# shaderko/velocity-asr

Hardware: NVIDIA B200
Metric: rtfx (higher is better)
Workload: dtype f32

## Files before the change

velocity-asr_b200/csrc/engine.cu:

```cuda
#include <cmath>
#include <cstdio>
#include <cstdlib>
#include <cstring>
#include <string>
#include <unordered_map>
#include <vector>

#include "../../include/vasr.h"
#include "common.cuh"
#include "kernels.cuh"

using namespace vasr;

namespace {

thread_local std::string g_err;

int fail(int code, const std::string& msg) {
  g_err = msg;
  return code;
}

#define CK(expr)                                                                               \
  do {                                                                                         \
    cudaError_t e_ = (expr);                                                                   \
    if (e_ != cudaSuccess)                                                                     \
      return fail(VASR_ERR_CUDA, std::string(#expr) + ": " + cudaGetErrorString(e_) + " (" +   \
                                     __FILE__ + ":" + std::to_string(__LINE__) + ")");         \
  } while (0)

#define RET(expr)            \
  do {                       \
    int r_ = (expr);         \
    if (r_ != VASR_OK) return r_; \
  } while (0)

constexpr int N_FFT = 400, HOP = 160, N_FREQ = 201, PAD = 200;

struct BlockW {
  float *ln1_g, *ln1_b, *ln2_g, *ln2_b, *conv_w, *conv_b, *A, *D;
  float *w_in, *w_xdt, *b_xdt, *w_out, *w_f1, *b_f1, *w_f2, *b_f2;
  float* s_f1;
  int N = 0;
  int di = 0, ks = 0;
  int structured = 0;
};

struct QSite {
  float *qs = nullptr, *qz = nullptr;
  int N = 0;
  int nmod = 0;
  const char* name[3] = {nullptr, nullptr, nullptr};
  int c0[3] = {0, 0, 0}, nc[3] = {0, 0, 0};
};
enum { Q_TB = 0, Q_P1, Q_P2, Q_Q, Q_KV, Q_O, Q_F3, Q_FO, Q_CTC, Q_SITES };

struct Arena {
  char* base = nullptr;
  size_t bytes = 0;
  size_t used = 0;
  void reset() { used = 0; }
  template <typename T>
  T* take(int64_t n) {
    size_t off = (used + 255) & ~size_t(255);
    used = off + (size_t)(n > 0 ? n : 0) * sizeof(T);
    return reinterpret_cast<T*>(base + off);
  }
};

}

struct vasr_handle {
  vasr_config cfg{};
  int device = 0;
  std::unordered_map<std::string, std::vector<float>> staged;
  bool committed = false;
  std::vector<void*> weight_allocs;
  std::vector<void*> frontend_allocs;
  std::vector<void*>* alloc_list = &weight_allocs;
  int quant = 0;
  int quant_active = 0;
  int calibrating = 0;
  QSite qsite[Q_SITES];
  static constexpr int RAG_RING = 4;
  int32_t* rag_pin[RAG_RING] = {};
  cudaEvent_t rag_ev[RAG_RING] = {};
  int64_t rag_pin_cap = 0;
  int rag_next = 0;
  float* q_mm = nullptr;
  std::unordered_map<const float*, float*> w_split;

  std::vector<BlockW> local, global;
  float *tb_w = nullptr, *tb_b = nullptr, *pe_time = nullptr, *pe_freq = nullptr, *tb_g = nullptr, *tb_bt = nullptr;
  int64_t pe_rows = 0;
  float *loc_g = nullptr, *loc_b = nullptr, *glo_g = nullptr, *glo_b = nullptr;
  float *p1_w = nullptr, *p1_b = nullptr, *p2_w = nullptr, *p2_b = nullptr;
  float *n1_g = nullptr, *n1_b = nullptr, *n2_g = nullptr, *n2_b = nullptr;
  float *w_q = nullptr, *b_q = nullptr, *w_kv = nullptr, *b_kv = nullptr, *w_o = nullptr, *b_o = nullptr;
  float *w_f3 = nullptr, *b_f3 = nullptr, *w_fo = nullptr, *b_fo = nullptr;
  float *ctc_g = nullptr, *ctc_b = nullptr, *w_ctc = nullptr, *b_ctc = nullptr;
  float *w_q_ln = nullptr, *b_q_ln = nullptr, *s_q = nullptr, *w_kv_ln = nullptr, *b_kv_ln = nullptr, *s_kv = nullptr;
  float *w_ctc_ln = nullptr, *b_ctc_ln = nullptr, *s_ctc = nullptr, *w_f3p = nullptr, *b_f3p = nullptr;
  float* win = nullptr;
  float* tw400 = nullptr;
  int *fb_lo = nullptr, *fb_off = nullptr;
  float* fb_w = nullptr;

  int num_sms = 148;
  int64_t tc_launches = 0;

  Arena ws;
  cudaStream_t own_stream = nullptr;
  static constexpr int HOST_SLICES = 8;
  cudaStream_t copy_stream = nullptr;
  cudaEvent_t slice_ev[HOST_SLICES] = {};
  cudaEvent_t copy_gate = nullptr;
  int64_t launches = 0;
  cudaEvent_t call_done = nullptr;
  cudaStream_t call_stream = nullptr;
  bool call_pending = false;

  int prof = 0;
  struct ProfEntry { std::string tag; cudaEvent_t e0, e1; };
  std::vector<ProfEntry> prof_ev;
  bool timing = false;
  std::vector<cudaEvent_t> ev;
  int ev_used = 0;
  cudaEvent_t ev_t0 = nullptr, ev_t1 = nullptr;
  bool ev_total = false;
};

namespace {

struct Dims {
  int64_t B, S, T, L, M, K1, K2, Mg, M2, Tp;
  int d, di, n_mels, V, att;
};

constexpr int GLOBAL_EXPAND = 2, GLOBAL_KS = 4;

Dims make_dims(const vasr_handle* h, int64_t B, int64_t S, int64_t T) {
  Dims q{};
  q.B = B;
  q.S = S;
  q.T = T;
  q.L = (T + 1) / 2;
  q.M = B * q.L;
  int64_t k1 = q.L / 8 > 64 ? q.L / 8 : 64;
  q.K1 = k1 < q.L ? k1 : q.L;
  int64_t k2 = q.K1 / 4 > 16 ? q.K1 / 4 : 16;
  k2 = k2 < 64 ? k2 : 64;
  q.K2 = k2 < q.K1 ? k2 : q.K1;
  q.Mg = B * q.K1;
  q.M2 = B * q.K2;
  q.Tp = T + 2 + ((T + 2) & 1);
  q.d = h->cfg.d_model;
  q.di = h->cfg.d_model * (h->cfg.ssm_expand_ratio > GLOBAL_EXPAND ? h->cfg.ssm_expand_ratio : GLOBAL_EXPAND);
  q.n_mels = h->cfg.mel_bins;
  q.V = h->cfg.vocab_size;
  q.att = h->cfg.attention_dim;
  return q;
}

struct Work {
  float *raw, *melpad;
  double* part;
  float* qscratch;
  float *xa, *xb, *u, *xz, *bcdt, *yg, *hbuf, *cat, *f3, *fm, *fused, *qb, *ob;
  float *ga, *gb, *g2, *g2n, *kv;
  float* logits;
  float* lnstat;
  float* amax_val;
  int32_t* amax_idx;
  int32_t* pred;
  float* pcm_stage;
  int32_t *tok_stage, *len_stage;
  int32_t* ragbuf;
  const int32_t* rag;
};

size_t carve(vasr_handle* h, const Dims& q, bool need_mel, bool need_logits, Work* w, bool need_stage = false) {
  Arena a = h->ws;
  a.reset();
  Work t{};
  const int nmax = h->cfg.ssm_state_dim > h->cfg.global_ssm_state_dim ? h->cfg.ssm_state_dim
                                                                      : h->cfg.global_ssm_state_dim;
  if (need_mel) {
    t.part = a.take<double>(q.B * mel_fft_blocks(q.T) * q.n_mels * 2);
    t.raw = a.take<float>(q.B * q.T * q.n_mels);
  }
  t.melpad = a.take<float>(q.B * q.Tp * q.n_mels);
  t.xa = a.take<float>(q.M * q.d);
  t.xb = a.take<float>(q.M * q.d);
  t.u = a.take<float>(q.M * q.d);
  t.xz = a.take<float>(q.M * 2 * q.di);
  t.bcdt = a.take<float>(q.M * (2 * nmax + q.di));
  t.yg = a.take<float>(q.M * q.di);
  t.hbuf = a.take<float>(q.M * q.di);
  t.cat = a.take<float>(q.M * 2 * q.d);
  if (!h->w_f3p) t.f3 = a.take<float>(q.M * 3 * q.d);
  t.fm = a.take<float>(q.M * q.d);
  t.fused = a.take<float>(q.M * q.d);
  t.qb = a.take<float>(q.M * q.att);
  t.ob = a.take<float>(q.M * q.att);
  t.ga = a.take<float>(q.Mg * q.d);
  t.gb = a.take<float>(q.Mg * q.d);
  t.g2 = a.take<float>(q.M2 * q.d);
  t.g2n = a.take<float>(q.M2 * q.d);
  t.kv = a.take<float>(q.M2 * 2 * q.att);
  if (need_logits) t.logits = a.take<float>(q.M * q.V);
  t.lnstat = a.take<float>(q.M * 2);
  t.amax_val = a.take<float>(q.M * argmax_slots(q.V));
  t.amax_idx = a.take<int32_t>(q.M * argmax_slots(q.V));
  if (h->quant_active) t.qscratch = a.take<float>(q.M * (q.V > 3 * q.d ? q.V : 3 * q.d));
  t.pred = a.take<int32_t>(q.M);
  t.ragbuf = a.take<int32_t>(q.B * RAG_STRIDE);
  if (need_stage) {
    t.pcm_stage = a.take<float>(q.B * q.S);
    t.tok_stage = a.take<int32_t>(q.M);
    t.len_stage = a.take<int32_t>(q.B);
  }
  if (w) *w = t;
  return a.used + 256;
}

int ensure_workspace(vasr_handle* h, const Dims& q, bool need_mel, bool need_logits, Work* w,
                     bool need_stage = false) {
  const size_t need = carve(h, q, need_mel, need_logits, nullptr, need_stage);
  if (need > h->ws.bytes) {
    CK(cudaDeviceSynchronize());
    if (h->ws.base) CK(cudaFree(h->ws.base));
    h->ws.base = nullptr;
    h->ws.bytes = 0;
    void* p = nullptr;
    CK(cudaMalloc(&p, need));
    h->ws.base = static_cast<char*>(p);
    h->ws.bytes = need;
  }
  carve(h, q, need_mel, need_logits, w, need_stage);
  return VASR_OK;
}

const std::vector<float>* find(vasr_handle* h, const std::string& k) {
  auto it = h->staged.find(k);
  return it == h->staged.end() ? nullptr : &it->second;
}

int need(vasr_handle* h, const std::string& k, int64_t numel, const std::vector<float>** out) {
  const std::vector<float>* v = find(h, k);
  if (!v) return fail(VASR_ERR_STATE, "missing weight: " + k);
  if (numel >= 0 && (int64_t)v->size() != numel)
    return fail(VASR_ERR_SHAPE, "weight " + k + " has " + std::to_string(v->size()) + " elements, expected " +
                                    std::to_string(numel));
  *out = v;
  return VASR_OK;
}

template <typename T>
int upload(vasr_handle* h, const T* src, size_t n, T** dst) {
  void* p = nullptr;
  CK(cudaMalloc(&p, (n ? n : 1) * sizeof(T)));
  h->alloc_list->push_back(p);
  if (n) CK(cudaMemcpy(p, src, n * sizeof(T), cudaMemcpyHostToDevice));
  *dst = static_cast<T*>(p);
  return VASR_OK;
}

int up(vasr_handle* h, const std::string& k, int64_t numel, float** dst) {
  const std::vector<float>* v;
  RET(need(h, k, numel, &v));
  return upload(h, v->data(), v->size(), dst);
}

void fake_quant_rows(std::vector<float>& w, int64_t rows) {
  const int64_t cols = rows > 0 ? (int64_t)w.size() / rows : 0;
  for (int64_t r = 0; r < rows; ++r) {
    float* x = w.data() + r * cols;
    float lo = x[0], hi = x[0];
    for (int64_t c = 1; c < cols; ++c) { lo = fminf(lo, x[c]); hi = fmaxf(hi, x[c]); }
    float scale = fmaxf(fabsf(lo), fabsf(hi)) / 127.0f;
    if (scale < 1e-10f) scale = 1e-10f;
    for (int64_t c = 0; c < cols; ++c) {
      volatile float t = x[c] / scale;
      float q = nearbyintf(t + 0.0f);
      q = fminf(fmaxf(q, -128.f), 127.f);
      volatile float dq = (q - 0.0f) * scale;
      volatile float diff = dq - x[c];
      x[c] = x[c] + diff;
    }
  }
}

int get_w(vasr_handle* h, const std::string& k, int64_t numel, int64_t rows, std::vector<float>* out) {
  const std::vector<float>* v;
  RET(need(h, k, numel, &v));
  *out = *v;
  if (h->quant) fake_quant_rows(*out, rows);
  return VASR_OK;
}
int up_w(vasr_handle* h, const std::string& k, int64_t numel, int64_t rows, float** dst) {
  std::vector<float> w;
  RET(get_w(h, k, numel, rows, &w));
  return upload(h, w.data(), w.size(), dst);
}

void fold_ln(const std::vector<float>& W, int64_t N, int64_t K, const float* bias, const float* gamma,
             const float* beta, std::vector<float>* Wf, std::vector<float>* bf, std::vector<float>* sf) {
  Wf->resize((size_t)N * K);
  bf->resize((size_t)N);
  sf->resize((size_t)N);
  for (int64_t n = 0; n < N; ++n) {
    double sb = bias ? (double)bias[n] : 0.0, ss = 0.0;
    for (int64_t k = 0; k < K; ++k) {
      const float w = W[(size_t)n * K + k];
      const float wf = w * gamma[k];
      (*Wf)[(size_t)n * K + k] = wf;
      sb += (double)w * (double)beta[k];
      ss += (double)wf;
    }
    (*bf)[(size_t)n] = (float)sb;
    (*sf)[(size_t)n] = (float)ss;
  }
}
bool can_fold_ln(int d) { return d % 32 == 0 && d / 32 > 4; }
int upload_folded(vasr_handle* h, const std::vector<float>& W, int64_t N, int64_t K, const float* bias,
                  const std::string& gk, const std::string& bk, float** Wd, float** bd, float** sd) {
  const std::vector<float>*g, *b;
  RET(need(h, gk, K, &g));
  RET(need(h, bk, K, &b));
  std::vector<float> Wf, bf, sf;
  fold_ln(W, N, K, bias, g->data(), b->data(), &Wf, &bf, &sf);
  RET(upload(h, Wf.data(), Wf.size(), Wd));
  RET(upload(h, bf.data(), bf.size(), bd));
  return upload(h, sf.data(), sf.size(), sd);
}

int gate_perm_row(int rp, int C) {
  const int t = rp / 192, a = (rp % 192) / 96, j = (rp % 96) / 32, i = rp % 32;
  return j * C + 64 * t + 32 * a + i;
}

int pack_block(vasr_handle* h, const std::string& p, int N, int expand, int ks, BlockW* w) {
  const int d = h->cfg.d_model, di = d * expand;
  w->N = N;
  w->di = di;
  w->ks = ks;
  RET(up(h, p + "norm1.weight", d, &w->ln1_g));
  RET(up(h, p + "norm1.bias", d, &w->ln1_b));
  RET(up(h, p + "norm2.weight", d, &w->ln2_g));
  RET(up(h, p + "norm2.bias", d, &w->ln2_b));
  RET(up(h, p + "conv.weight", (int64_t)d * ks, &w->conv_w));
  RET(up(h, p + "conv.bias", d, &w->conv_b));
  const std::vector<float>*alog, *xw, *dw, *db;
  RET(need(h, p + "ssm.A_log", N, &alog));
  std::vector<float> A(N);
  int structured = 1;
  for (int n = 0; n < N; ++n) {
    A[n] = -expf((*alog)[n]);
    if (fabsf((*alog)[n] - logf((float)(n + 1))) > 1e-6f) structured = 0;
  }
  w->structured = structured;
  RET(upload(h, A.data(), A.size(), &w->A));
  RET(up(h, p + "ssm.D", di, &w->D));
  RET(up(h, p + "ssm.in_proj.weight", (int64_t)2 * di * d, &w->w_in));
  RET(need(h, p + "ssm.x_proj.weight", (int64_t)2 * N * di, &xw));
  RET(need(h, p + "ssm.dt_proj.weight", (int64_t)di * di, &dw));
  RET(need(h, p + "ssm.dt_proj.bias", di, &db));
  std::vector<float> wx((size_t)(2 * N + di) * di), bx((size_t)2 * N + di, 0.f);
  memcpy(wx.data(), xw->data(), xw->size() * sizeof(float));
  memcpy(wx.data() + xw->size(), dw->data(), dw->size() * sizeof(float));
  memcpy(bx.data() + 2 * N, db->data(), db->size() * sizeof(float));
  RET(upload(h, wx.data(), wx.size(), &w->w_xdt));
  RET(upload(h, bx.data(), bx.size(), &w->b_xdt));
  RET(up(h, p + "ssm.out_proj.weight", (int64_t)d * di, &w->w_out));
  const std::vector<float>*f1w, *f1b;
  RET(need(h, p + "ffn.0.weight", (int64_t)di * d, &f1w));
  RET(need(h, p + "ffn.0.bias", di, &f1b));
  w->s_f1 = nullptr;
  if (can_fold_ln(d) && (di % 192 == 0 || di % 192 >= 128)) {
    RET(upload_folded(h, *f1w, di, d, f1b->data(), p + "norm2.weight", p + "norm2.bias", &w->w_f1, &w->b_f1, &w->s_f1));
  } else {
    RET(upload(h, f1w->data(), f1w->size(), &w->w_f1));
    RET(upload(h, f1b->data(), f1b->size(), &w->b_f1));
  }
  RET(up(h, p + "ffn.3.weight", (int64_t)d * di, &w->w_f2));
  RET(up(h, p + "ffn.3.bias", d, &w->b_f2));
  return VASR_OK;
}

void default_window(std::vector<float>& w) {
  w.resize(N_FFT);
  for (int i = 0; i < N_FFT; ++i) w[i] = (float)(0.5 - 0.5 * cos(2.0 * M_PI * i / N_FFT));
}
void default_filterbank(int n_mels, std::vector<float>& fb) {
  fb.assign((size_t)n_mels * N_FREQ, 0.f);
  auto lin = [](float a, float b, int steps, int i) {
    float step = (b - a) / (float)(steps - 1);
    return i < steps / 2 ? a + step * (float)i : b - step * (float)(steps - 1 - i);
  };
  const float mel_max = 2595.f * log10f(1.f + 8000.f / 700.f);
  std::vector<float> hz(n_mels + 2);
  for (int i = 0; i < n_mels + 2; ++i) hz[i] = 700.f * (powf(10.f, lin(0.f, mel_max, n_mels + 2, i) / 2595.f) - 1.f);
  for (int j = 0; j < n_mels; ++j)
    for (int k = 0; k < N_FREQ; ++k) {
      const float f = lin(0.f, 8000.f, N_FREQ, k);
      const float up_ = (f - hz[j]) / (hz[j + 1] - hz[j] + 1e-10f);
      const float dn = (hz[j + 2] - f) / (hz[j + 2] - hz[j + 1] + 1e-10f);
      const float v = up_ < dn ? up_ : dn;
      fb[(size_t)j * N_FREQ + k] = v > 0.f ? v : 0.f;
    }
}

int pack_frontend_impl(vasr_handle* h);
int setup_qsites(vasr_handle* h);
void free_splits(vasr_handle* h);
int pack_frontend(vasr_handle* h) {
  CK(cudaDeviceSynchronize());
  free_splits(h);
  for (void* p : h->frontend_allocs) cudaFree(p);
  h->frontend_allocs.clear();
  h->alloc_list = &h->frontend_allocs;
  const int r = pack_frontend_impl(h);
  h->alloc_list = &h->weight_allocs;
  return r;
}
int pack_frontend_impl(vasr_handle* h) {
  const int n_mels = h->cfg.mel_bins;
  std::vector<float> win, fb;
  if (const std::vector<float>* v = find(h, "frontend.window")) {
    if ((int)v->size() != N_FFT) return fail(VASR_ERR_SHAPE, "frontend.window must have 400 elements");
    win = *v;
  } else {
    default_window(win);
  }
  if (const std::vector<float>* v = find(h, "frontend.mel_filterbank")) {
    if ((int64_t)v->size() != (int64_t)n_mels * N_FREQ)
      return fail(VASR_ERR_SHAPE, "frontend.mel_filterbank must be n_mels x 201");
    fb = *v;
  } else {
    default_filterbank(n_mels, fb);
  }
  RET(upload(h, win.data(), win.size(), &h->win));
  std::vector<float> tw((size_t)2 * N_FFT);
  for (int m = 0; m < N_FFT; ++m) {
    const double ang = 2.0 * M_PI * (double)m / (double)N_FFT;
    tw[2 * m] = (float)cos(ang);
    tw[2 * m + 1] = (float)(-sin(ang));
  }
  RET(upload(h, tw.data(), tw.size(), &h->tw400));
  std::vector<int> lo(n_mels), off(n_mels + 1, 0);
  std::vector<float> wts;
  for (int j = 0; j < n_mels; ++j) {
    int a = -1, b = -1;
    for (int k = 0; k < N_FREQ; ++k)
      if (fb[(size_t)j * N_FREQ + k] != 0.f) {
        if (a < 0) a = k;
        b = k;
      }
    lo[j] = a < 0 ? 0 : a;
    if (a >= 0)
      for (int k = a; k <= b; ++k) wts.push_back(fb[(size_t)j * N_FREQ + k]);
    off[j + 1] = (int)wts.size();
  }
  RET(upload(h, lo.data(), lo.size(), &h->fb_lo));
  RET(upload(h, off.data(), off.size(), &h->fb_off));
  RET(upload(h, wts.data(), wts.size(), &h->fb_w));
  return VASR_OK;
}

void free_splits(vasr_handle* h) {
  for (auto& kv : h->w_split) cudaFree(kv.second);
  h->w_split.clear();
}

void free_weights(vasr_handle* h) {
  free_splits(h);
  for (void* p : h->weight_allocs) cudaFree(p);
  h->weight_allocs.clear();
  h->local.clear();
  h->global.clear();
  h->committed = false;
}

#define KL(expr)                                                                            \
  do {                                                                                      \
    cudaError_t e_ = (expr);                                                                \
    if (e_ != cudaSuccess)                                                                  \
      return fail(e_ == cudaErrorInvalidValue ? VASR_ERR_UNSUPPORTED : VASR_ERR_CUDA,       \
                  std::string(#expr) + ": " + cudaGetErrorString(e_));                      \
  } while (0)

int split_of(vasr_handle* h, const float* W, int64_t numel, cudaStream_t s, const float** out) {
  auto it = h->w_split.find(W);
  if (it == h->w_split.end()) {
    void* p = nullptr;
    CK(cudaMalloc(&p, (size_t)2 * numel * sizeof(float)));
    KL(launch_split_tf32(W, static_cast<float*>(p), numel, s));
    it = h->w_split.emplace(W, static_cast<float*>(p)).first;
  }
  *out = it->second;
  return VASR_OK;
}

int gemm(vasr_handle* h, GemmArgs& g, cudaStream_t s);
int calibrate_site(vasr_handle* h, const GemmArgs& g, const QSite& q, float* scratch, cudaStream_t s) {
  GemmArgs p = g;
  p.C = scratch; p.ldc = g.N;
  p.q_scale = p.q_zp = nullptr;
  p.act = ACT_NONE; p.act_from = 0;
  p.resid = nullptr; p.pe_time = p.pe_freq = nullptr;
  RET(gemm(h, p, s));
  for (int i = 0; i < q.nmod; ++i) {
    KL(launch_minmax(scratch, g.N, g.M, q.c0[i], q.nc[i], h->q_mm, s, &h->launches));
    KL(launch_set_qparams(h->q_mm, q.qs, q.qz, q.c0[i], q.nc[i], s, &h->launches));
  }
  return VASR_OK;
}

int gemm_impl(vasr_handle* h, GemmArgs& g, cudaStream_t s);
int gemm(vasr_handle* h, GemmArgs& g, cudaStream_t s) {
  if (!h->prof) return gemm_impl(h, g, s);
  vasr_handle::ProfEntry pe;
  pe.tag = "M" + std::to_string(g.M) + " K" + std::to_string(g.K) + " N" + std::to_string(g.N) + " act" +
           std::to_string(g.act) + (g.resid ? " resid" : "") + (g.pe_time ? " pe" : "") + (g.q_scale ? " quant" : "");
  CK(cudaEventCreate(&pe.e0));
  CK(cudaEventCreate(&pe.e1));
  CK(cudaEventRecord(pe.e0, s));
  const int r = gemm_impl(h, g, s);
  CK(cudaEventRecord(pe.e1, s));
  h->prof_ev.push_back(pe);
  return r;
}

int gemm_impl(vasr_handle* h, GemmArgs& g, cudaStream_t s) {
  RET(split_of(h, g.W, g.N * g.K, s, &g.W_split));
  const cudaError_t e = launch_gemm_tc(g, h->num_sms, s, &h->launches);
  if (e == cudaErrorNotSupported) {
    (void)cudaGetLastError();
    return fail(VASR_ERR_UNSUPPORTED, "projection " + std::to_string(g.M) + " x " + std::to_string(g.K) + " -> " +
                                          std::to_string(g.N) + ": view not supported by the tensor-core kernel "
                                          "(16-byte alignment of rows, K % 4, N % 4)");
  }
  if (e != cudaSuccess) return fail(VASR_ERR_CUDA, std::string("launch_gemm_tc: ") + cudaGetErrorString(e));
  ++h->tc_launches;
  return VASR_OK;
}

int gemm_q(vasr_handle* h, GemmArgs& g, int site, float* qscratch, cudaStream_t s) {
  if (site >= 0 && h->quant_active) {
    const QSite& q = h->qsite[site];
    g.q_scale = q.qs;
    g.q_zp = q.qz;
    if (h->calibrating) RET(calibrate_site(h, g, q, qscratch, s));
  }
  return gemm(h, g, s);
}

int linear(vasr_handle* h, const float* A, int64_t lda, const float* W, const float* bias, float* C, int64_t ldc,
           int64_t M, int64_t K, int64_t N, int act, int act_from, const float* resid, int64_t ldr,
           cudaStream_t s, int site = -1, float* qscratch = nullptr) {
  GemmArgs g;
  g.A = A; g.lda = lda; g.W = W; g.bias = bias; g.C = C; g.ldc = ldc;
  g.M = M; g.N = N; g.K = K; g.act = act; g.act_from = act_from; g.resid = resid; g.ldr = ldr;
  return gemm_q(h, g, site, qscratch, s);
}
int linear_ln(vasr_handle* h, const Work& k, const float* A, int64_t lda, const float* W, const float* bias,
              const float* colsum, float* C, int64_t ldc, int64_t M, int64_t K, int64_t N, int act, cudaStream_t s) {
  GemmArgs g;
  g.A = A; g.lda = lda; g.W = W; g.bias = bias; g.C = C; g.ldc = ldc;
  g.M = M; g.N = N; g.K = K; g.act = act; g.act_from = 0;
  g.ln_s = colsum; g.ln_stats = k.lnstat;
  return gemm(h, g, s);
}


int run_scan(vasr_handle* h, const BlockW& w, const Work& k, int64_t B, int64_t L, int quirk, cudaStream_t s) {
  const int di = w.di;
  const int64_t ld = 2 * w.N + di;
  ScanArgs a;
  a.x = k.xz; a.ldx = 2 * di;
  a.z = k.xz + di; a.ldz = 2 * di;
  a.Bm = k.bcdt; a.ldb = ld;
  a.Cm = k.bcdt + w.N; a.ldc = ld;
  a.dt = k.bcdt + 2 * w.N; a.lddt = ld;
  a.A = w.A; a.D = w.D;
  a.y = k.yg; a.ldy = di;
  a.B = B; a.L = L; a.Di = di; a.N = w.N;
  a.parallel_quirk = quirk;
  a.structured_a = w.structured;
  a.num_sms = h->num_sms;
  const bool t = h->timing && h->ev_used + 2 <= (int)h->ev.size();
  if (t) cudaEventRecord(h->ev[h->ev_used], s);
  KL(launch_selective_scan(a, s, &h->launches));
  if (t) {
    cudaEventRecord(h->ev[h->ev_used + 1], s);
    h->ev_used += 2;
  }
  return VASR_OK;
}

int run_block(vasr_handle* h, const BlockW& w, const Work& k, float* x, float* x1, int64_t B, int64_t L, int quirk,
              cudaStream_t s) {
  const int d = h->cfg.d_model, di = w.di;
  const int64_t M = B * L;
  KL(launch_ln_dwconv(x, k.u, w.ln1_g, w.ln1_b, w.conv_w, w.conv_b, B, L, d, w.ks, s, &h->launches));
  RET(linear(h, k.u, d, w.w_in, nullptr, k.xz, 2 * di, M, d, 2 * di, ACT_NONE, 0, nullptr, 0, s));
  RET(linear(h, k.xz, 2 * di, w.w_xdt, w.b_xdt, k.bcdt, 2 * w.N + di, M, di, 2 * w.N + di, ACT_SOFTPLUS, 2 * w.N,
             nullptr, 0, s));
  RET(run_scan(h, w, k, B, L, quirk, s));
  RET(linear(h, k.yg, di, w.w_out, nullptr, x1, d, M, di, d, ACT_NONE, 0, x, d, s));
  if (w.s_f1) {
    RET(linear_ln(h, k, x1, d, w.w_f1, w.b_f1, w.s_f1, k.hbuf, di, M, d, di, ACT_GELU, s));
  } else {
    KL(launch_layer_norm(x1, d, k.u, d, w.ln2_g, w.ln2_b, M, d, s, &h->launches));
    RET(linear(h, k.u, d, w.w_f1, w.b_f1, k.hbuf, di, M, d, di, ACT_GELU, 0, nullptr, 0, s));
  }
  RET(linear(h, k.hbuf, di, w.w_f2, w.b_f2, x, d, M, di, d, ACT_NONE, 0, x1, d, s));
  return VASR_OK;
}

int quirk_for(const vasr_handle* h, int stack, int scan_mode) {
  if (scan_mode < 0) scan_mode = stack == 0 ? h->cfg.scan_mode : VASR_SCAN_PARALLEL;
  return scan_mode == VASR_SCAN_PARALLEL ? 1 : 0;
}

int run_global_context(vasr_handle* h, const Dims& q, const Work& k, cudaStream_t s) {
  const int d = q.d, att = q.att;
  KL(launch_adaptive_pool(k.cat, 2 * d, k.gb, q.B, q.L, q.K1, d, s, &h->launches, k.rag, RAG_L, RAG_K1));
  RET(linear(h, k.gb, d, h->p1_w, h->p1_b, k.ga, d, q.Mg, d, d, ACT_NONE, 0, nullptr, 0, s, Q_P1, k.qscratch));
  for (size_t i = 0; i < h->global.size(); ++i)
    RET(run_block(h, h->global[i], k, k.ga, k.gb, q.B, q.K1, quirk_for(h, 1, -1), s));
  KL(launch_layer_norm(k.ga, d, k.ga, d, h->glo_g, h->glo_b, q.Mg, d, s, &h->launches));
  KL(launch_adaptive_pool(k.ga, d, k.g2, q.B, q.K1, q.K2, d, s, &h->launches, k.rag, RAG_K1, RAG_K2));
  RET(linear(h, k.g2, d, h->p2_w, h->p2_b, k.g2n, d, q.M2, d, d, ACT_NONE, 0, nullptr, 0, s, Q_P2, k.qscratch));
  if (h->w_kv_ln) {
    RET(linear_ln(h, k, k.g2n, d, h->w_kv_ln, h->b_kv_ln, h->s_kv, k.kv, 2 * att, q.M2, d, 2 * att, ACT_NONE, s));
    RET(linear_ln(h, k, k.cat, 2 * d, h->w_q_ln, h->b_q_ln, h->s_q, k.qb, att, q.M, d, att, ACT_NONE, s));
  } else {
    KL(launch_layer_norm(k.g2n, d, k.g2n, d, h->n1_g, h->n1_b, q.M2, d, s, &h->launches));
    RET(linear(h, k.g2n, d, h->w_kv, h->b_kv, k.kv, 2 * att, q.M2, d, 2 * att, ACT_NONE, 0, nullptr, 0, s, Q_KV, k.qscratch));
    KL(launch_layer_norm(k.cat, 2 * d, k.u, d, h->n2_g, h->n2_b, q.M, d, s, &h->launches));
    RET(linear(h, k.u, d, h->w_q, h->b_q, k.qb, att, q.M, d, att, ACT_NONE, 0, nullptr, 0, s, Q_Q, k.qscratch));
  }
  KL(launch_attention(k.qb, att, k.kv, k.ob, att, q.B, q.L, q.K2, h->cfg.attention_heads,
                      att / h->cfg.attention_heads, s, &h->launches, k.rag));
  RET(linear(h, k.ob, att, h->w_o, h->b_o, k.cat + d, 2 * d, q.M, att, d, ACT_NONE, 0, nullptr, 0, s, Q_O, k.qscratch));
  if (h->w_f3p) {
    GemmArgs g;
    g.A = k.cat; g.lda = 2 * d; g.W = h->w_f3p; g.bias = h->b_f3p; g.C = k.fm; g.ldc = d;
    g.M = q.M; g.N = 3 * d; g.K = 2 * d; g.gate = 1;
    RET(gemm(h, g, s));
  } else {
    RET(linear(h, k.cat, 2 * d, h->w_f3, h->b_f3, k.f3, 3 * d, q.M, 2 * d, 3 * d, ACT_NONE, 0, nullptr, 0, s, Q_F3, k.qscratch));
    KL(launch_gate_mix(k.f3, k.fm, q.M, d, s, &h->launches));
  }
  RET(linear(h, k.fm, d, h->w_fo, h->b_fo, k.fused, d, q.M, d, d, ACT_NONE, 0, nullptr, 0, s, Q_FO, k.qscratch));
  return VASR_OK;
}

int run_ctc_head(vasr_handle* h, const Dims& q, const Work& k, const float* x, float* logits, cudaStream_t s) {
  if (h->w_ctc_ln) {
    GemmArgs g;
    g.A = x; g.lda = q.d; g.W = h->w_ctc_ln; g.bias = h->b_ctc_ln; g.C = logits; g.ldc = q.V;
    g.M = q.M; g.N = q.V; g.K = q.d;
    g.ln_s = h->s_ctc; g.ln_stats = k.lnstat;
    if (!logits) { g.amax_val = k.amax_val; g.amax_idx = k.amax_idx; }
    return gemm(h, g, s);
  }
  if (!logits) return fail(VASR_ERR_STATE, "the FakeQuantize model decodes from its logits");
  KL(launch_layer_norm(x, q.d, k.u, q.d, h->ctc_g, h->ctc_b, q.M, q.d, s, &h->launches));
  RET(linear(h, k.u, q.d, h->w_ctc, h->b_ctc, logits, q.V, q.M, q.d, q.V, ACT_NONE, 0, nullptr, 0, s, Q_CTC, k.qscratch));
  return VASR_OK;
}

int run_model(vasr_handle* h, const Dims& q, const Work& k, float* logits, float* f_tb, float* f_local,
              float* f_fused, cudaStream_t s) {
  const int d = q.d;
  if (q.L > h->pe_rows)
    return fail(VASR_ERR_SHAPE, "sequence of " + std::to_string(q.L) + " tokens exceeds the positional table (" +
                                    std::to_string(h->pe_rows) + " rows, model.py:87,125)");
  GemmArgs g;
  g.A = k.melpad; g.lda = 2 * q.n_mels; g.rows_per_batch = q.L; g.batch_stride = q.Tp * q.n_mels;
  g.W = h->tb_w; g.bias = h->tb_b; g.C = k.xa; g.ldc = d;
  g.M = q.M; g.N = d; g.K = 3 * q.n_mels;
  g.act = ACT_GELU; g.act_from = 0;
  g.pe_time = h->pe_time; g.pe_freq = h->pe_freq; g.pe_half = d / 2; g.pe_rows = q.L;
  RET(gemm_q(h, g, Q_TB, k.qscratch, s));
  KL(launch_layer_norm(k.xa, d, k.xa, d, h->tb_g, h->tb_bt, q.M, d, s, &h->launches));
  if (f_tb) CK(cudaMemcpyAsync(f_tb, k.xa, (size_t)q.M * d * sizeof(float), cudaMemcpyDeviceToDevice, s));
  for (size_t i = 0; i < h->local.size(); ++i)
    RET(run_block(h, h->local[i], k, k.xa, k.xb, q.B, q.L, quirk_for(h, 0, -1), s));
  KL(launch_layer_norm(k.xa, d, k.cat, 2 * d, h->loc_g, h->loc_b, q.M, d, s, &h->launches));
  if (f_local)
    CK(cudaMemcpy2DAsync(f_local, (size_t)d * sizeof(float), k.cat, (size_t)2 * d * sizeof(float),
                         (size_t)d * sizeof(float), (size_t)q.M, cudaMemcpyDeviceToDevice, s));
  RET(run_global_context(h, q, k, s));
  if (f_fused) CK(cudaMemcpyAsync(f_fused, k.fused, (size_t)q.M * d * sizeof(float), cudaMemcpyDeviceToDevice, s));
  RET(run_ctc_head(h, q, k, k.fused, logits, s));
  return VASR_OK;
}

int run_mel(vasr_handle* h, const Dims& q, const Work& k, const float* pcm, int normalize, cudaStream_t s) {
  KL(launch_mel_fft(pcm, k.raw, normalize ? k.part : nullptr, q.B, q.S, q.T, q.n_mels, h->fb_lo, h->fb_off, h->fb_w,
                    h->win, h->tw400, s, &h->launches, k.rag));
  return VASR_OK;
}

int run_mel_from_host(vasr_handle* h, const Dims& q, const Work& k, const float* pcm_host, cudaStream_t s) {
  const int64_t per = (q.B + vasr_handle::HOST_SLICES - 1) / vasr_handle::HOST_SLICES;
  const int64_t nblk = mel_fft_blocks(q.T);
  CK(cudaEventRecord(h->copy_gate, s));
  CK(cudaStreamWaitEvent(h->copy_stream, h->copy_gate, 0));
  int i = 0;
  for (int64_t b0 = 0; b0 < q.B; b0 += per, ++i) {
    const int64_t nb = q.B - b0 < per ? q.B - b0 : per;
    CK(cudaMemcpyAsync(k.pcm_stage + b0 * q.S, pcm_host + b0 * q.S, (size_t)nb * q.S * sizeof(float),
                       cudaMemcpyHostToDevice, h->copy_stream));
    CK(cudaEventRecord(h->slice_ev[i], h->copy_stream));
    CK(cudaStreamWaitEvent(s, h->slice_ev[i], 0));
    KL(launch_mel_fft(k.pcm_stage + b0 * q.S, k.raw + b0 * q.T * q.n_mels, k.part + b0 * nblk * q.n_mels * 2, nb, q.S,
                      q.T, q.n_mels, h->fb_lo, h->fb_off, h->fb_w, h->win, h->tw400, s, &h->launches,
                      k.rag ? k.rag + b0 * RAG_STRIDE : nullptr));
  }
  return VASR_OK;
}

int check_ready(const vasr_handle* h) {
  if (!h) return fail(VASR_ERR_INVALID, "null handle");
  if (!h->committed) return fail(VASR_ERR_STATE, "weights not committed (call vasr_commit_weights)");
  return VASR_OK;
}

struct DeviceGuard {
  int prev = -1;
  explicit DeviceGuard(int dev) {
    if (cudaGetDevice(&prev) != cudaSuccess || prev == dev) prev = -1;
    cudaSetDevice(dev);
  }
  ~DeviceGuard() {
    if (prev >= 0) cudaSetDevice(prev);
  }
  DeviceGuard(const DeviceGuard&) = delete;
  DeviceGuard& operator=(const DeviceGuard&) = delete;
};

struct CallOrder {
  vasr_handle* h;
  cudaStream_t s;
  CallOrder(vasr_handle* h_, cudaStream_t s_) : h(h_), s(s_) {
    if (h->call_pending && h->call_stream != s) cudaStreamWaitEvent(s, h->call_done, 0);
  }
  ~CallOrder() {
    if (cudaEventRecord(h->call_done, s) == cudaSuccess) {
      h->call_stream = s;
      h->call_pending = true;
    }
  }
  CallOrder(const CallOrder&) = delete;
  CallOrder& operator=(const CallOrder&) = delete;
};

void timing_begin(vasr_handle* h, cudaStream_t s) {
  h->ev_used = 0;
  h->ev_total = false;
  if (h->timing) {
    cudaEventRecord(h->ev_t0, s);
    h->ev_total = true;
  }
}
void timing_end(vasr_handle* h, cudaStream_t s) {
  if (h->timing) cudaEventRecord(h->ev_t1, s);
}

int setup_qsites(vasr_handle* h) {
  const int d = h->cfg.d_model, att = h->cfg.attention_dim, V = h->cfg.vocab_size;
  auto site = [&](int id, int N, std::initializer_list<const char*> names, std::initializer_list<int> widths) {
    QSite& q = h->qsite[id];
    q.N = N;
    q.nmod = 0;
    int c = 0;
    auto w = widths.begin();
    for (const char* nm : names) {
      q.name[q.nmod] = nm; q.c0[q.nmod] = c; q.nc[q.nmod] = *w;
      c += *w; ++w; ++q.nmod;
    }
  };
  site(Q_TB, d, {"temporal_binding.conv"}, {d});
  site(Q_P1, d, {"global_context.pool1.pool_proj"}, {d});
  site(Q_P2, d, {"global_context.pool2.pool_proj"}, {d});
  site(Q_Q, att, {"global_context.cross_attention.q_proj"}, {att});
  site(Q_KV, 2 * att, {"global_context.cross_attention.k_proj", "global_context.cross_attention.v_proj"}, {att, att});
  site(Q_O, d, {"global_context.cross_attention.out_proj"}, {d});
  site(Q_F3, 3 * d, {"global_context.fusion.gate_proj.0", "global_context.fusion.local_proj",
                     "global_context.fusion.global_proj"}, {d, d, d});
  site(Q_FO, d, {"global_context.fusion.out_proj"}, {d});
  site(Q_CTC, V, {"ctc_head.proj.2"}, {V});
  for (int i = 0; i < Q_SITES; ++i) {
    QSite& q = h->qsite[i];
    std::vector<float> zeros((size_t)q.N, 0.f);
    RET(upload(h, zeros.data(), zeros.size(), &q.qs));
    RET(upload(h, zeros.data(), zeros.size(), &q.qz));
  }
  if (!h->q_mm) {
    void* p = nullptr;
    CK(cudaMalloc(&p, 2 * sizeof(float)));
    h->q_mm = static_cast<float*>(p);
  }
  return VASR_OK;
}

QSite* find_module(vasr_handle* h, const char* module, int* idx) {
  for (int i = 0; i < Q_SITES; ++i)
    for (int j = 0; j < h->qsite[i].nmod; ++j)
      if (strcmp(h->qsite[i].name[j], module) == 0) {
        *idx = j;
        return &h->qsite[i];
      }
  return nullptr;
}

}

extern "C" {

const char* vasr_last_error(void) { return g_err.c_str(); }
const char* vasr_version(void) { return "libvasr 0.1 (sm_100a)"; }

int64_t vasr_num_frames(int64_t samples) { return 1 + samples / HOP; }
int64_t vasr_num_tokens(int64_t frames) { return (frames + 1) / 2; }

int vasr_create(const vasr_config* cfg, int device, vasr_handle** out) {
  if (!cfg || !out) return fail(VASR_ERR_INVALID, "null argument");
  *out = nullptr;
  const vasr_config& c = *cfg;
  if (c.scan_mode < 0 || c.scan_mode > 2) return fail(VASR_ERR_INVALID, "Unknown scan_mode");
  if (c.d_model <= 0 || c.d_model > 192 || (c.d_model % 16) != 0)
    return fail(VASR_ERR_UNSUPPORTED, "d_model must be a multiple of 16, at most 192");
  if ((c.mel_bins * 3) % 16 != 0 || c.mel_bins * 8 > 1024)
    return fail(VASR_ERR_UNSUPPORTED, "mel_bins must make 3*mel_bins a multiple of 16 (and be <= 128)");
  auto n_ok = [](int n) { return n == 16 || n == 32 || n == 64; };
  if (!n_ok(c.ssm_state_dim) || !n_ok(c.global_ssm_state_dim))
    return fail(VASR_ERR_UNSUPPORTED, "ssm state_dim must be 16, 32 or 64");
  const int di = c.d_model * c.ssm_expand_ratio;
  if (c.ssm_expand_ratio < 1 || (di % 64) != 0 || (c.d_model * GLOBAL_EXPAND) % 64 != 0)
    return fail(VASR_ERR_UNSUPPORTED, "d_model*expand_ratio (and 2*d_model for the global stack) must be multiples of 64");
  if (c.ssm_kernel_size < 1 || c.ssm_kernel_size > 8) return fail(VASR_ERR_UNSUPPORTED, "ssm_kernel_size must be in [1, 8]");
  if (c.attention_heads < 1 || c.attention_dim % c.attention_heads != 0 || c.attention_dim / c.attention_heads > 16 ||
      c.attention_dim % 16 != 0 || c.attention_heads > 4)
    return fail(VASR_ERR_UNSUPPORTED, "attention_dim must be a multiple of 16 with head_dim <= 16 and at most 4 heads "
                                      "(the attention kernel runs 64 threads per head in a 256-thread CTA)");
  if (c.vocab_size < 1 || c.ssm_layers < 0 || c.global_ssm_layers < 0) return fail(VASR_ERR_INVALID, "bad sizes");
  int ndev = 0;
  if (cudaGetDeviceCount(&ndev) != cudaSuccess || ndev <= 0)
    return fail(VASR_ERR_CUDA, "no CUDA device: libvasr has no CPU path");
  if (device < 0 || device >= ndev) return fail(VASR_ERR_INVALID, "bad device index");
  cudaDeviceProp prop;
  CK(cudaGetDeviceProperties(&prop, device));
  if (prop.major != 10) return fail(VASR_ERR_CUDA, std::string("libvasr is built for sm_100a only; device is ") + prop.name);
  DeviceGuard dev_guard(device);
  vasr_handle* h = new vasr_handle();
  h->cfg = c;
  h->device = device;
  h->num_sms = prop.multiProcessorCount;
  h->prof = debug_env_int("VASR_PROF", 0);
  CK(cudaStreamCreateWithFlags(&h->own_stream, cudaStreamNonBlocking));
  CK(cudaStreamCreateWithFlags(&h->copy_stream, cudaStreamNonBlocking));
  for (auto& e : h->slice_ev) CK(cudaEventCreateWithFlags(&e, cudaEventDisableTiming));
  CK(cudaEventCreateWithFlags(&h->copy_gate, cudaEventDisableTiming));
  CK(cudaEventCreateWithFlags(&h->call_done, cudaEventDisableTiming));
  h->ev.resize(64);
  for (auto& e : h->ev) CK(cudaEventCreate(&e));
  CK(cudaEventCreate(&h->ev_t0));
  CK(cudaEventCreate(&h->ev_t1));
  RET(pack_frontend(h));
  *out = h;
  return VASR_OK;
}

void vasr_destroy(vasr_handle* h) {
  if (!h) return;
  DeviceGuard dev_guard(h->device);
  cudaDeviceSynchronize();
  free_weights(h);
  for (void* p : h->frontend_allocs) cudaFree(p);
  if (h->ws.base) cudaFree(h->ws.base);
  if (h->q_mm) cudaFree(h->q_mm);
  for (auto& e : h->ev) cudaEventDestroy(e);
  if (h->ev_t0) cudaEventDestroy(h->ev_t0);
  if (h->ev_t1) cudaEventDestroy(h->ev_t1);
  if (h->own_stream) cudaStreamDestroy(h->own_stream);
  if (h->copy_stream) cudaStreamDestroy(h->copy_stream);
  for (auto& e : h->slice_ev)
    if (e) cudaEventDestroy(e);
  if (h->copy_gate) cudaEventDestroy(h->copy_gate);
  if (h->call_done) cudaEventDestroy(h->call_done);
  for (int i = 0; i < vasr_handle::RAG_RING; ++i) {
    if (h->rag_pin[i]) cudaFreeHost(h->rag_pin[i]);
    if (h->rag_ev[i]) cudaEventDestroy(h->rag_ev[i]);
  }
  delete h;
}

int vasr_set_weight(vasr_handle* h, const char* name, const float* host, int64_t numel) {
  if (!h || !name || (!host && numel > 0) || numel < 0) return fail(VASR_ERR_INVALID, "null argument");
  const std::string k(name);
  static const char* prefixes[] = {"temporal_binding.", "local_ssm.", "global_context.", "ctc_head.", "frontend."};
  bool ok = false;
  for (const char* p : prefixes) ok = ok || k.rfind(p, 0) == 0;
  if (!ok) return fail(VASR_ERR_INVALID, "unknown weight name: " + k);
  h->staged[k].assign(host, host + numel);
  if (k.rfind("frontend.", 0) == 0) {
    DeviceGuard dev_guard(h->device);
    return pack_frontend(h);
  }
  h->committed = false;
  return VASR_OK;
}

int vasr_commit_weights(vasr_handle* h) {
  if (!h) return fail(VASR_ERR_INVALID, "null handle");
  DeviceGuard dev_guard(h->device);
  CK(cudaDeviceSynchronize());
  free_weights(h);
  h->w_q_ln = h->b_q_ln = h->s_q = h->w_kv_ln = h->b_kv_ln = h->s_kv = nullptr;
  h->w_ctc_ln = h->b_ctc_ln = h->s_ctc = h->w_f3p = h->b_f3p = nullptr;
  const vasr_config& c = h->cfg;
  const int d = c.d_model, nm = c.mel_bins, att = c.attention_dim;
  std::vector<float> cwv;
  RET(get_w(h, "temporal_binding.conv.weight", (int64_t)d * nm * 3, d, &cwv));
  const std::vector<float>* cw = &cwv;
  std::vector<float> tbw((size_t)d * 3 * nm);
  for (int o = 0; o < d; ++o)
    for (int ch = 0; ch < nm; ++ch)
      for (int j = 0; j < 3; ++j) tbw[(size_t)o * 3 * nm + j * nm + ch] = (*cw)[((size_t)o * nm + ch) * 3 + j];
  RET(upload(h, tbw.data(), tbw.size(), &h->tb_w));
  RET(up(h, "temporal_binding.conv.bias", d, &h->tb_b));
  const std::vector<float>* pt;
  RET(need(h, "temporal_binding.pos_encoding.pe_time", -1, &pt));
  if (pt->size() % (size_t)(d / 2) != 0) return fail(VASR_ERR_SHAPE, "pe_time must be (rows, d_model/2)");
  h->pe_rows = (int64_t)pt->size() / (d / 2);
  RET(upload(h, pt->data(), pt->size(), &h->pe_time));
  RET(up(h, "temporal_binding.pos_encoding.pe_freq", d - d / 2, &h->pe_freq));
  RET(up(h, "temporal_binding.norm.weight", d, &h->tb_g));
  RET(up(h, "temporal_binding.norm.bias", d, &h->tb_bt));
  h->local.resize(c.ssm_layers);
  for (int i = 0; i < c.ssm_layers; ++i)
    RET(pack_block(h, "local_ssm.layers." + std::to_string(i) + ".", c.ssm_state_dim, c.ssm_expand_ratio,
                   c.ssm_kernel_size, &h->local[i]));
  RET(up(h, "local_ssm.norm.weight", d, &h->loc_g));
  RET(up(h, "local_ssm.norm.bias", d, &h->loc_b));
  const std::string gc = "global_context.";
  h->global.resize(c.global_ssm_layers);
  for (int i = 0; i < c.global_ssm_layers; ++i)
    RET(pack_block(h, gc + "global_ssm.layers." + std::to_string(i) + ".", c.global_ssm_state_dim, GLOBAL_EXPAND,
                   GLOBAL_KS, &h->global[i]));
  RET(up(h, gc + "global_ssm.norm.weight", d, &h->glo_g));
  RET(up(h, gc + "global_ssm.norm.bias", d, &h->glo_b));
  RET(up_w(h, gc + "pool1.pool_proj.weight", (int64_t)d * d, d, &h->p1_w));
  RET(up(h, gc + "pool1.pool_proj.bias", d, &h->p1_b));
  RET(up_w(h, gc + "pool2.pool_proj.weight", (int64_t)d * d, d, &h->p2_w));
  RET(up(h, gc + "pool2.pool_proj.bias", d, &h->p2_b));
  RET(up(h, gc + "norm1.weight", d, &h->n1_g));
  RET(up(h, gc + "norm1.bias", d, &h->n1_b));
  RET(up(h, gc + "norm2.weight", d, &h->n2_g));
  RET(up(h, gc + "norm2.bias", d, &h->n2_b));
  RET(up_w(h, gc + "cross_attention.q_proj.weight", (int64_t)att * d, att, &h->w_q));
  RET(up(h, gc + "cross_attention.q_proj.bias", att, &h->b_q));
  const std::vector<float>*kb, *vb;
  std::vector<float> kwv, vwv;
  RET(get_w(h, gc + "cross_attention.k_proj.weight", (int64_t)att * d, att, &kwv));
  RET(need(h, gc + "cross_attention.k_proj.bias", att, &kb));
  RET(get_w(h, gc + "cross_attention.v_proj.weight", (int64_t)att * d, att, &vwv));
  RET(need(h, gc + "cross_attention.v_proj.bias", att, &vb));
  const std::vector<float>*kw = &kwv, *vw = &vwv;
  std::vector<float> wkv(*kw), bkv(*kb);
  wkv.insert(wkv.end(), vw->begin(), vw->end());
  bkv.insert(bkv.end(), vb->begin(), vb->end());
  RET(upload(h, wkv.data(), wkv.size(), &h->w_kv));
  RET(upload(h, bkv.data(), bkv.size(), &h->b_kv));
  if (!h->quant && can_fold_ln(d)) {
    const std::vector<float>*qw, *qb;
    RET(need(h, gc + "cross_attention.q_proj.weight", (int64_t)att * d, &qw));
    RET(need(h, gc + "cross_attention.q_proj.bias", att, &qb));
    RET(upload_folded(h, *qw, att, d, qb->data(), gc + "norm2.weight", gc + "norm2.bias", &h->w_q_ln, &h->b_q_ln, &h->s_q));
    RET(upload_folded(h, wkv, 2 * att, d, bkv.data(), gc + "norm1.weight", gc + "norm1.bias", &h->w_kv_ln, &h->b_kv_ln,
                      &h->s_kv));
  }
  RET(up_w(h, gc + "cross_attention.out_proj.weight", (int64_t)d * att, d, &h->w_o));
  RET(up(h, gc + "cross_attention.out_proj.bias", d, &h->b_o));
  const std::vector<float>*gb, *lb, *cb2;
  std::vector<float> gwv, lwv, cwv2;
  RET(get_w(h, gc + "fusion.gate_proj.0.weight", (int64_t)d * 2 * d, d, &gwv));
  RET(need(h, gc + "fusion.gate_proj.0.bias", d, &gb));
  RET(get_w(h, gc + "fusion.local_proj.weight", (int64_t)d * d, d, &lwv));
  RET(need(h, gc + "fusion.local_proj.bias", d, &lb));
  RET(get_w(h, gc + "fusion.global_proj.weight", (int64_t)d * d, d, &cwv2));
  RET(need(h, gc + "fusion.global_proj.bias", d, &cb2));
  const std::vector<float>*gw = &gwv, *lw = &lwv, *cw2 = &cwv2;
  std::vector<float> wf3((size_t)3 * d * 2 * d, 0.f), bf3;
  memcpy(wf3.data(), gw->data(), gw->size() * sizeof(float));
  for (int o = 0; o < d; ++o) {
    memcpy(&wf3[(size_t)(d + o) * 2 * d], &(*lw)[(size_t)o * d], d * sizeof(float));
    memcpy(&wf3[(size_t)(2 * d + o) * 2 * d + d], &(*cw2)[(size_t)o * d], d * sizeof(float));
  }
  bf3 = *gb;
  bf3.insert(bf3.end(), lb->begin(), lb->end());
  bf3.insert(bf3.end(), cb2->begin(), cb2->end());
  RET(upload(h, wf3.data(), wf3.size(), &h->w_f3));
  RET(upload(h, bf3.data(), bf3.size(), &h->b_f3));
  h->w_f3p = h->b_f3p = nullptr;
  if (!h->quant && d % 64 == 0) {
    std::vector<float> wp(wf3.size()), bp(bf3.size());
    for (int rp = 0; rp < 3 * d; ++rp) {
      const int r = gate_perm_row(rp, d);
      memcpy(&wp[(size_t)rp * 2 * d], &wf3[(size_t)r * 2 * d], (size_t)2 * d * sizeof(float));
      bp[(size_t)rp] = bf3[(size_t)r];
    }
    RET(upload(h, wp.data(), wp.size(), &h->w_f3p));
    RET(upload(h, bp.data(), bp.size(), &h->b_f3p));
  }
  RET(up_w(h, gc + "fusion.out_proj.weight", (int64_t)d * d, d, &h->w_fo));
  RET(up(h, gc + "fusion.out_proj.bias", d, &h->b_fo));
  RET(up(h, "ctc_head.proj.0.weight", d, &h->ctc_g));
  RET(up(h, "ctc_head.proj.0.bias", d, &h->ctc_b));
  RET(up_w(h, "ctc_head.proj.2.weight", (int64_t)c.vocab_size * d, c.vocab_size, &h->w_ctc));
  RET(up(h, "ctc_head.proj.2.bias", c.vocab_size, &h->b_ctc));
  if (!h->quant && can_fold_ln(d)) {
    const std::vector<float>*hw, *hb;
    RET(need(h, "ctc_head.proj.2.weight", (int64_t)c.vocab_size * d, &hw));
    RET(need(h, "ctc_head.proj.2.bias", c.vocab_size, &hb));
    RET(upload_folded(h, *hw, c.vocab_size, d, hb->data(), "ctc_head.proj.0.weight", "ctc_head.proj.0.bias", &h->w_ctc_ln,
                      &h->b_ctc_ln, &h->s_ctc));
  }
  h->quant_active = h->quant;
  if (h->quant_active) RET(setup_qsites(h));
  h->committed = true;
  return VASR_OK;
}

int vasr_log_mel(vasr_handle* h, const float* pcm_dev, int64_t B, int64_t S, int normalize, float* mel_dev,
                 void* stream) {
  if (!h) return fail(VASR_ERR_INVALID, "null handle");
  if (B < 0 || !pcm_dev || !mel_dev) return fail(VASR_ERR_INVALID, "null argument");
  if (S <= PAD) return fail(VASR_ERR_SHAPE, "reflect padding needs more than 200 samples (audio.py:100-101)");
  DeviceGuard dev_guard(h->device);
  cudaStream_t s = static_cast<cudaStream_t>(stream);
  CallOrder call_order(h, s);
  const Dims q = make_dims(h, B, S, vasr_num_frames(S));
  Work k;
  RET(ensure_workspace(h, q, true, false, &k));
  RET(run_mel(h, q, k, pcm_dev, normalize, s));
  KL(launch_mel_finish(k.raw, nullptr, nullptr, mel_dev, q.B, q.T, q.n_mels, q.T, 0, s, &h->launches, nullptr,
                       normalize ? k.part : nullptr));
  return VASR_OK;
}

int vasr_forward(vasr_handle* h, const float* mel_dev, int64_t B, int64_t T, float* logits_dev, float* feat_tb_dev,
                 float* feat_local_dev, float* feat_fused_dev, void* stream) {
  RET(check_ready(h));
  if (B < 0 || T < 1 || !mel_dev || !logits_dev) return fail(VASR_ERR_INVALID, "null argument");
  DeviceGuard dev_guard(h->device);
  cudaStream_t s = static_cast<cudaStream_t>(stream);
  CallOrder call_order(h, s);
  const Dims q = make_dims(h, B, 0, T);
  Work k;
  RET(ensure_workspace(h, q, false, false, &k));
  timing_begin(h, s);
  KL(launch_mel_finish(mel_dev, nullptr, nullptr, k.melpad, q.B, q.T, q.n_mels, q.Tp, 1, s, &h->launches));
  RET(run_model(h, q, k, logits_dev, feat_tb_dev, feat_local_dev, feat_fused_dev, s));
  timing_end(h, s);
  return VASR_OK;
}

int vasr_ssm_block(vasr_handle* h, int stack, int layer, int scan_mode, const float* x_dev, int64_t B, int64_t L,
                   float* out_dev, void* stream) {
  RET(check_ready(h));
  if (stack < 0 || stack > 1) return fail(VASR_ERR_INVALID, "stack must be 0 (local) or 1 (global)");
  const std::vector<BlockW>& blocks = stack == 0 ? h->local : h->global;
  if (layer < 0 || layer >= (int)blocks.size()) return fail(VASR_ERR_INVALID, "layer out of range");
  if (scan_mode > 2) return fail(VASR_ERR_INVALID, "Unknown scan_mode");
  DeviceGuard dev_guard(h->device);
  cudaStream_t s = static_cast<cudaStream_t>(stream);
  CallOrder call_order(h, s);
  Dims q = make_dims(h, B, 0, 2 * L - 1);
  Work k;
  RET(ensure_workspace(h, q, false, false, &k));
  const size_t bytes = (size_t)B * L * q.d * sizeof(float);
  CK(cudaMemcpyAsync(k.xa, x_dev, bytes, cudaMemcpyDeviceToDevice, s));
  RET(run_block(h, blocks[layer], k, k.xa, k.xb, B, L, quirk_for(h, stack, scan_mode), s));
  CK(cudaMemcpyAsync(out_dev, k.xa, bytes, cudaMemcpyDeviceToDevice, s));
  return VASR_OK;
}

int vasr_global_context(vasr_handle* h, const float* local_dev, int64_t B, int64_t L, float* out_dev, void* stream) {
  RET(check_ready(h));
  DeviceGuard dev_guard(h->device);
  cudaStream_t s = static_cast<cudaStream_t>(stream);
  CallOrder call_order(h, s);
  Dims q = make_dims(h, B, 0, 2 * L - 1);
  Work k;
  RET(ensure_workspace(h, q, false, false, &k));
  const size_t row = (size_t)q.d * sizeof(float);
  CK(cudaMemcpy2DAsync(k.cat, 2 * row, local_dev, row, row, (size_t)q.M, cudaMemcpyDeviceToDevice, s));
  RET(run_global_context(h, q, k, s));
  CK(cudaMemcpyAsync(out_dev, k.fused, (size_t)q.M * row, cudaMemcpyDeviceToDevice, s));
  return VASR_OK;
}

int vasr_ctc_head(vasr_handle* h, const float* x_dev, int64_t B, int64_t L, float* logits_dev, void* stream) {
  RET(check_ready(h));
  DeviceGuard dev_guard(h->device);
  cudaStream_t s = static_cast<cudaStream_t>(stream);
  CallOrder call_order(h, s);
  Dims q = make_dims(h, B, 0, 2 * L - 1);
  Work k;
  RET(ensure_workspace(h, q, false, false, &k));
  RET(run_ctc_head(h, q, k, x_dev, logits_dev, s));
  return VASR_OK;
}

int vasr_selective_scan(const float* x, int64_t ldx, const float* dt, int64_t lddt, const float* A, const float* Bm,
                        int64_t ldb, const float* Cm, int64_t ldc, const float* D, const float* z, int64_t ldz,
                        float* y, int64_t ldy, int64_t B, int64_t L, int64_t Di, int64_t N, int scan_mode,
                        void* stream) {
  if (!x || !dt || !A || !Bm || !Cm || !y) return fail(VASR_ERR_INVALID, "null argument");
  if (scan_mode < 0 || scan_mode > 2) return fail(VASR_ERR_INVALID, "Unknown scan_mode");
  if (N != 16 && N != 32 && N != 64) return fail(VASR_ERR_UNSUPPORTED, "state_dim must be 16, 32 or 64");
  float ah[64];
  CK(cudaMemcpy(ah, A, (size_t)N * sizeof(float), cudaMemcpyDeviceToHost));
  int structured = 1;
  for (int n = 0; n < N; ++n)
    if (fabsf(ah[n] + (float)(n + 1)) > 2e-6f * (float)(n + 1)) structured = 0;
  ScanArgs a;
  a.x = x; a.ldx = ldx; a.dt = dt; a.lddt = lddt; a.z = z; a.ldz = ldz;
  a.Bm = Bm; a.ldb = ldb; a.Cm = Cm; a.ldc = ldc; a.A = A; a.D = D; a.y = y; a.ldy = ldy;
  a.B = B; a.L = L; a.Di = (int)Di; a.N = (int)N;
  a.parallel_quirk = scan_mode == VASR_SCAN_PARALLEL;
  a.structured_a = structured;
  cudaStream_t s = static_cast<cudaStream_t>(stream);
  int dev = 0;
  CK(cudaGetDevice(&dev));
  CK(cudaDeviceGetAttribute(&a.num_sms, cudaDevAttrMultiProcessorCount, dev));
  KL(launch_selective_scan(a, s, nullptr));
  return VASR_OK;
}

int vasr_ctc_greedy(const float* logits_dev, int64_t B, int64_t L, int64_t V, int blank, int collapse,
                    int32_t* tokens_dev, int32_t* lens_dev, void* stream) {
  if (!tokens_dev || !lens_dev || (!logits_dev && B * L > 0)) return fail(VASR_ERR_INVALID, "null argument");
  if (B <= 0) return VASR_OK;
  cudaStream_t s = static_cast<cudaStream_t>(stream);
  int32_t* pred = nullptr;
  CK(cudaMallocAsync(reinterpret_cast<void**>(&pred), (size_t)(B * L > 0 ? B * L : 1) * sizeof(int32_t), s));
  KL(launch_argmax(logits_dev, pred, B * L, (int)V, s, nullptr));
  KL(launch_ctc_collapse(pred, tokens_dev, lens_dev, B, L, blank, collapse, s, nullptr));
  CK(cudaFreeAsync(pred, s));
  return VASR_OK;
}

int vasr_ctc_greedy_timestamps(const float* logits_dev, int64_t B, int64_t L, int64_t V, int blank,
                               int32_t* tokens_dev, int32_t* starts_dev, int32_t* ends_dev, int32_t* lens_dev,
                               void* stream) {
  if (!tokens_dev || !starts_dev || !ends_dev || !lens_dev || (!logits_dev && B * L > 0))
    return fail(VASR_ERR_INVALID, "null argument");
  if (B <= 0) return VASR_OK;
  cudaStream_t s = static_cast<cudaStream_t>(stream);
  int32_t* pred = nullptr;
  CK(cudaMallocAsync(reinterpret_cast<void**>(&pred), (size_t)(B * L > 0 ? B * L : 1) * sizeof(int32_t), s));
  KL(launch_argmax(logits_dev, pred, B * L, (int)V, s, nullptr));
  KL(launch_ctc_runs(pred, tokens_dev, starts_dev, ends_dev, lens_dev, B, L, blank, s, nullptr));
  CK(cudaFreeAsync(pred, s));
  return VASR_OK;
}

int vasr_ctc_beam_search(const float* logits_dev, int64_t B, int64_t L, int64_t V, int beam_width, int blank,
                         int32_t* tokens_dev, int32_t* lens_dev, double* scores_dev, void* stream) {
  if (!tokens_dev && B * beam_width * L > 0) return fail(VASR_ERR_INVALID, "null argument");
  if (!lens_dev || !scores_dev || (!logits_dev && B * L > 0)) return fail(VASR_ERR_INVALID, "null argument");
  if (beam_width < 1 || beam_width > 32) return fail(VASR_ERR_INVALID, "beam_width must be in [1, 32]");
  if (V < 1 || blank < 0 || blank >= V) return fail(VASR_ERR_INVALID, "blank token outside the vocabulary");
  if (B <= 0) return VASR_OK;
  cudaStream_t s = static_cast<cudaStream_t>(stream);
  const int W = beam_width;
  const int K = (int)(V - 1 < W + 1 ? V - 1 : W + 1) > 0 ? (int)(V - 1 < W + 1 ? V - 1 : W + 1) : 1;
  const int64_t M = B * L, cap = 1 + L * W;
  float2* stats = nullptr;
  int32_t *top = nullptr, *trie = nullptr;
  CK(cudaMallocAsync(reinterpret_cast<void**>(&stats), (size_t)(M > 0 ? M : 1) * sizeof(float2), s));
  CK(cudaMallocAsync(reinterpret_cast<void**>(&top), (size_t)(M > 0 ? M : 1) * K * sizeof(int32_t), s));
  CK(cudaMallocAsync(reinterpret_cast<void**>(&trie), (size_t)3 * B * cap * sizeof(int32_t), s));
  KL(launch_beam_rows(logits_dev, stats, top, M, (int)V, K, blank, s, nullptr));
  KL(launch_beam_search(logits_dev, stats, top, K, B, L, (int)V, W, blank, trie, cap, tokens_dev, lens_dev,
                        scores_dev, s, nullptr));
  CK(cudaFreeAsync(stats, s));
  CK(cudaFreeAsync(top, s));
  CK(cudaFreeAsync(trie, s));
  return VASR_OK;
}

static int upload_ragged(vasr_handle* h, const Dims& q, Work& k, const int32_t* lens, bool from_samples,
                         cudaStream_t s) {
  const int64_t count = q.B * RAG_STRIDE;
  if (count > h->rag_pin_cap) {
    CK(cudaDeviceSynchronize());
    for (int i = 0; i < vasr_handle::RAG_RING; ++i) {
      if (h->rag_pin[i]) CK(cudaFreeHost(h->rag_pin[i]));
      h->rag_pin[i] = nullptr;
      CK(cudaHostAlloc(reinterpret_cast<void**>(&h->rag_pin[i]), (size_t)count * sizeof(int32_t), cudaHostAllocDefault));
      if (!h->rag_ev[i]) CK(cudaEventCreateWithFlags(&h->rag_ev[i], cudaEventDisableTiming));
    }
    h->rag_pin_cap = count;
  }
  const int slot = h->rag_next;
  h->rag_next = (slot + 1) % vasr_handle::RAG_RING;
  CK(cudaEventSynchronize(h->rag_ev[slot]));
  int32_t* host = h->rag_pin[slot];
  for (int64_t i = 0; i < count; ++i) host[i] = 0;
  for (int64_t b = 0; b < q.B; ++b) {
    const int64_t n = lens[b];
    if (from_samples) {
      if (n <= PAD || n > q.S)
        return fail(VASR_ERR_SHAPE, "ragged batch: every utterance needs more than 200 and at most S samples");
    } else if (n < 1 || n > q.T) {
      return fail(VASR_ERR_SHAPE, "ragged batch: every utterance needs between 1 and T frames");
    }
    const Dims u = make_dims(h, 1, from_samples ? n : 0, from_samples ? vasr_num_frames(n) : n);
    int32_t* r = host + b * RAG_STRIDE;
    r[RAG_S] = (int32_t)(from_samples ? n : 0);
    r[RAG_T] = (int32_t)u.T;
    r[RAG_L] = (int32_t)u.L;
    r[RAG_K1] = (int32_t)u.K1;
    r[RAG_K2] = (int32_t)u.K2;
  }
  CK(cudaMemcpyAsync(k.ragbuf, host, (size_t)count * sizeof(int32_t), cudaMemcpyHostToDevice, s));
  CK(cudaEventRecord(h->rag_ev[slot], s));
  k.rag = k.ragbuf;
  return VASR_OK;
}

static int transcribe_impl(vasr_handle* h, const float* pcm_dev, const float* pcm_host, int64_t B, int64_t S,
                           int32_t* tokens_dev, int32_t* lens_dev, int32_t* tokens_host, int32_t* lens_host,
                           cudaStream_t s, const int32_t* sample_lens = nullptr) {
  const bool host = pcm_host != nullptr;
  CallOrder call_order(h, s);
  const Dims q = make_dims(h, B, S, vasr_num_frames(S));
  Work k;
  const bool from_parts = h->w_ctc_ln != nullptr;
  RET(ensure_workspace(h, q, true, !from_parts, &k, host));
  if (sample_lens) RET(upload_ragged(h, q, k, sample_lens, true, s));
  if (host) {
    tokens_dev = k.tok_stage;
    lens_dev = k.len_stage;
  }
  timing_begin(h, s);
  if (host) RET(run_mel_from_host(h, q, k, pcm_host, s));
  else RET(run_mel(h, q, k, pcm_dev, 1, s));
  KL(launch_mel_finish(k.raw, nullptr, nullptr, k.melpad, q.B, q.T, q.n_mels, q.Tp, 1, s, &h->launches, k.rag, k.part));
  RET(run_model(h, q, k, from_parts ? nullptr : k.logits, nullptr, nullptr, nullptr, s));
  if (from_parts) {
    KL(launch_ctc_collapse(k.pred, tokens_dev, lens_dev, q.B, q.L, 0, 1, s, &h->launches, k.rag, k.amax_val, k.amax_idx,
                           argmax_slots(q.V)));
  } else {
    KL(launch_argmax(k.logits, k.pred, q.M, q.V, s, &h->launches));
    KL(launch_ctc_collapse(k.pred, tokens_dev, lens_dev, q.B, q.L, 0, 1, s, &h->launches, k.rag));
  }
  timing_end(h, s);
  if (host) {
    CK(cudaMemcpyAsync(tokens_host, tokens_dev, (size_t)q.M * sizeof(int32_t), cudaMemcpyDeviceToHost, s));
    CK(cudaMemcpyAsync(lens_host, lens_dev, (size_t)B * sizeof(int32_t), cudaMemcpyDeviceToHost, s));
    CK(cudaStreamSynchronize(s));
  }
  return VASR_OK;
}

int vasr_transcribe(vasr_handle* h, const float* pcm_dev, int64_t B, int64_t S, int32_t* tokens_dev,
                    int32_t* lens_dev, void* stream) {
  RET(check_ready(h));
  if (B < 0 || !pcm_dev || !tokens_dev || !lens_dev) return fail(VASR_ERR_INVALID, "null argument");
  if (S <= PAD) return fail(VASR_ERR_SHAPE, "reflect padding needs more than 200 samples (audio.py:100-101)");
  DeviceGuard dev_guard(h->device);
  return transcribe_impl(h, pcm_dev, nullptr, B, S, tokens_dev, lens_dev, nullptr, nullptr,
                         static_cast<cudaStream_t>(stream));
}

int vasr_transcribe_host(vasr_handle* h, const float* pcm_host, int64_t B, int64_t S, int32_t* tokens_host,
                         int32_t* lens_host) {
  RET(check_ready(h));
  if (B <= 0 || !pcm_host || !tokens_host || !lens_host) return fail(VASR_ERR_INVALID, "null argument");
  if (S <= PAD) return fail(VASR_ERR_SHAPE, "reflect padding needs more than 200 samples (audio.py:100-101)");
  DeviceGuard dev_guard(h->device);
  return transcribe_impl(h, nullptr, pcm_host, B, S, nullptr, nullptr, tokens_host, lens_host, h->own_stream);
}

int vasr_transcribe_ragged(vasr_handle* h, const float* pcm_dev, const int32_t* sample_lens_host, int64_t B,
                           int64_t S, int32_t* tokens_dev, int32_t* lens_dev, void* stream) {
  RET(check_ready(h));
  if (B < 0 || !pcm_dev || !tokens_dev || !lens_dev || !sample_lens_host)
    return fail(VASR_ERR_INVALID, "null argument");
  if (S <= PAD) return fail(VASR_ERR_SHAPE, "reflect padding needs more than 200 samples (audio.py:100-101)");
  DeviceGuard dev_guard(h->device);
  return transcribe_impl(h, pcm_dev, nullptr, B, S, tokens_dev, lens_dev, nullptr, nullptr,
                         static_cast<cudaStream_t>(stream), sample_lens_host);
}

int vasr_transcribe_ragged_host(vasr_handle* h, const float* pcm_host, const int32_t* sample_lens_host, int64_t B,
                                int64_t S, int32_t* tokens_host, int32_t* lens_host) {
  RET(check_ready(h));
  if (B <= 0 || !pcm_host || !tokens_host || !lens_host || !sample_lens_host)
    return fail(VASR_ERR_INVALID, "null argument");
  if (S <= PAD) return fail(VASR_ERR_SHAPE, "reflect padding needs more than 200 samples (audio.py:100-101)");
  DeviceGuard dev_guard(h->device);
  return transcribe_impl(h, nullptr, pcm_host, B, S, nullptr, nullptr, tokens_host, lens_host, h->own_stream,
                         sample_lens_host);
}

int vasr_forward_ragged(vasr_handle* h, const float* mel_dev, const int32_t* frame_lens_host, int64_t B, int64_t T,
                        float* logits_dev, void* stream) {
  RET(check_ready(h));
  if (B < 0 || T < 1 || !mel_dev || !logits_dev || !frame_lens_host) return fail(VASR_ERR_INVALID, "null argument");
  DeviceGuard dev_guard(h->device);
  cudaStream_t s = static_cast<cudaStream_t>(stream);
  CallOrder call_order(h, s);
  const Dims q = make_dims(h, B, 0, T);
  Work k;
  RET(ensure_workspace(h, q, false, false, &k));
  RET(upload_ragged(h, q, k, frame_lens_host, false, s));
  timing_begin(h, s);
  KL(launch_mel_finish(mel_dev, nullptr, nullptr, k.melpad, q.B, q.T, q.n_mels, q.Tp, 1, s, &h->launches, k.rag));
  RET(run_model(h, q, k, logits_dev, nullptr, nullptr, nullptr, s));
  timing_end(h, s);
  return VASR_OK;
}

int vasr_linear(const float* x_dev, int64_t ldx, const float* w_dev, const float* bias_dev, float* out_dev,
                int64_t ldo, int64_t M, int64_t K, int64_t N, int act, void* stream) {
  if (!x_dev || !w_dev || !out_dev) return fail(VASR_ERR_INVALID, "null argument");
  if (act < 0 || act > 3) return fail(VASR_ERR_INVALID, "unknown activation");
  GemmArgs g;
  g.A = x_dev; g.lda = ldx; g.W = w_dev; g.bias = bias_dev; g.C = out_dev; g.ldc = ldo;
  g.M = M; g.N = N; g.K = K; g.act = act; g.act_from = 0;
  KL(launch_gemm(g, static_cast<cudaStream_t>(stream), nullptr));
  return VASR_OK;
}

int vasr_set_quantization(vasr_handle* h, int enabled) {
  if (!h) return fail(VASR_ERR_INVALID, "null handle");
  if ((enabled != 0) != (h->quant != 0)) {
    h->quant = enabled != 0;
    h->committed = false;
  }
  return VASR_OK;
}

int vasr_calibrate(vasr_handle* h, const float* mel_dev, int64_t B, int64_t T, void* stream) {
  RET(check_ready(h));
  if (!h->quant_active) return fail(VASR_ERR_STATE, "quantisation is not enabled (vasr_set_quantization + commit)");
  if (B <= 0 || T < 1 || !mel_dev) return fail(VASR_ERR_INVALID, "null argument");
  DeviceGuard dev_guard(h->device);
  cudaStream_t s = static_cast<cudaStream_t>(stream);
  CallOrder call_order(h, s);
  const Dims q = make_dims(h, B, 0, T);
  Work k;
  RET(ensure_workspace(h, q, false, true, &k));
  KL(launch_mel_finish(mel_dev, nullptr, nullptr, k.melpad, q.B, q.T, q.n_mels, q.Tp, 1, s, &h->launches));
  h->calibrating = 1;
  const int r = run_model(h, q, k, k.logits, nullptr, nullptr, nullptr, s);
  h->calibrating = 0;
  return r;
}

int vasr_get_quant_params(vasr_handle* h, const char* module, float* scale, float* zero_point) {
  if (!h || !module || !scale || !zero_point) return fail(VASR_ERR_INVALID, "null argument");
  if (!h->quant_active) return fail(VASR_ERR_STATE, "quantisation is not enabled");
  int j = 0;
  QSite* q = find_module(h, module, &j);
  if (!q) return fail(VASR_ERR_INVALID, std::string("not a quantised module: ") + module);
  DeviceGuard dev_guard(h->device);
  CK(cudaDeviceSynchronize());
  CK(cudaMemcpy(scale, q->qs + q->c0[j], sizeof(float), cudaMemcpyDeviceToHost));
  CK(cudaMemcpy(zero_point, q->qz + q->c0[j], sizeof(float), cudaMemcpyDeviceToHost));
  return VASR_OK;
}

int vasr_set_quant_params(vasr_handle* h, const char* module, float scale, float zero_point) {
  if (!h || !module) return fail(VASR_ERR_INVALID, "null argument");
  if (!h->quant_active) return fail(VASR_ERR_STATE, "quantisation is not enabled");
  int j = 0;
  QSite* q = find_module(h, module, &j);
  if (!q) return fail(VASR_ERR_INVALID, std::string("not a quantised module: ") + module);
  DeviceGuard dev_guard(h->device);
  CK(cudaDeviceSynchronize());
  std::vector<float> sv((size_t)q->nc[j], scale), zv((size_t)q->nc[j], zero_point);
  CK(cudaMemcpy(q->qs + q->c0[j], sv.data(), sv.size() * sizeof(float), cudaMemcpyHostToDevice));
  CK(cudaMemcpy(q->qz + q->c0[j], zv.data(), zv.size() * sizeof(float), cudaMemcpyHostToDevice));
  return VASR_OK;
}

int vasr_quant_site(vasr_handle* h, const char* module, const float* x_dev, int64_t B, int64_t R, float* out_dev,
                    int32_t* n_out, int32_t* col0, int32_t* ncol, void* stream) {
  RET(check_ready(h));
  if (!module) return fail(VASR_ERR_INVALID, "null argument");
  if (!h->quant_active) return fail(VASR_ERR_STATE, "quantisation is not enabled (vasr_set_quantization + commit)");
  int j = 0;
  QSite* q = find_module(h, module, &j);
  if (!q) return fail(VASR_ERR_INVALID, std::string("not a quantised module: ") + module);
  const int site = (int)(q - h->qsite);
  if (n_out) *n_out = q->N;
  if (col0) *col0 = q->c0[j];
  if (ncol) *ncol = q->nc[j];
  if (!x_dev || !out_dev) return B * R > 0 ? fail(VASR_ERR_INVALID, "null argument") : VASR_OK;
  if (B <= 0 || R <= 0) return VASR_OK;
  DeviceGuard dev_guard(h->device);
  cudaStream_t s = static_cast<cudaStream_t>(stream);
  CallOrder call_order(h, s);
  const int d = h->cfg.d_model, att = h->cfg.attention_dim;
  GemmArgs g;
  g.act = ACT_NONE;
  g.C = out_dev; g.ldc = q->N; g.N = q->N;
  if (site == Q_TB) {
    const Dims dm = make_dims(h, B, 0, R);
    Work k;
    RET(ensure_workspace(h, dm, false, false, &k));
    KL(launch_mel_finish(x_dev, nullptr, nullptr, k.melpad, dm.B, dm.T, dm.n_mels, dm.Tp, 1, s, &h->launches));
    g.A = k.melpad; g.lda = 2 * dm.n_mels; g.rows_per_batch = dm.L; g.batch_stride = dm.Tp * dm.n_mels;
    g.W = h->tb_w; g.bias = h->tb_b; g.M = dm.M; g.K = 3 * dm.n_mels;
  } else {
    struct { const float* w; const float* b; int K; } tab[Q_SITES] = {
        {nullptr, nullptr, 0}, {h->p1_w, h->p1_b, d}, {h->p2_w, h->p2_b, d}, {h->w_q, h->b_q, d},
        {h->w_kv, h->b_kv, d}, {h->w_o, h->b_o, att}, {h->w_f3, h->b_f3, 2 * d}, {h->w_fo, h->b_fo, d},
        {h->w_ctc, h->b_ctc, d}};
    g.A = x_dev; g.lda = tab[site].K; g.W = tab[site].w; g.bias = tab[site].b; g.M = B * R; g.K = tab[site].K;
  }
  g.q_scale = q->qs;
  g.q_zp = q->qz;
  return gemm(h, g, s);
}

int vasr_split_tf32(const float* w_dev, float* split_dev, int64_t numel, void* stream) {
  if (!w_dev || !split_dev || numel < 0) return fail(VASR_ERR_INVALID, "null argument");
  KL(launch_split_tf32(w_dev, split_dev, numel, static_cast<cudaStream_t>(stream)));
  return VASR_OK;
}

int vasr_linear_tc(const float* x_dev, int64_t ldx, const float* w_dev, const float* w_split_dev,
                   const float* bias_dev, const float* resid_dev, int64_t ldr, float* out_dev, int64_t ldo, int64_t M,
                   int64_t K, int64_t N, int act, void* stream) {
  if (!x_dev || (!w_dev && !w_split_dev) || !out_dev) return fail(VASR_ERR_INVALID, "null argument");
  if (act < 0 || act > 3) return fail(VASR_ERR_INVALID, "unknown activation");
  cudaStream_t s = static_cast<cudaStream_t>(stream);
  int dev = 0, sms = 148;
  CK(cudaGetDevice(&dev));
  CK(cudaDeviceGetAttribute(&sms, cudaDevAttrMultiProcessorCount, dev));
  GemmArgs g;
  g.A = x_dev; g.lda = ldx; g.W = w_dev; g.bias = bias_dev; g.C = out_dev; g.ldc = ldo;
  g.M = M; g.N = N; g.K = K; g.act = act; g.act_from = 0;
  g.resid = resid_dev; g.ldr = ldr;
  float* hl = nullptr;
  if (!w_split_dev) {
    CK(cudaMallocAsync(reinterpret_cast<void**>(&hl), (size_t)2 * N * K * sizeof(float), s));
    KL(launch_split_tf32(w_dev, hl, N * K, s));
    w_split_dev = hl;
  }
  g.W_split = w_split_dev;
  cudaError_t e = launch_gemm_tc(g, sms, s, nullptr);
  if (hl) CK(cudaFreeAsync(hl, s));
  if (e == cudaErrorNotSupported) return fail(VASR_ERR_UNSUPPORTED, "tensor map could not be encoded for this view");
  if (e != cudaSuccess) return fail(VASR_ERR_CUDA, std::string("launch_gemm_tc: ") + cudaGetErrorString(e));
  return VASR_OK;
}

int vasr_debug_gemm_trace(long long* dev_buf) {
  g_trace = dev_buf;
  return VASR_OK;
}

int vasr_debug_dump_profile(vasr_handle* h) {
  if (!h) return fail(VASR_ERR_INVALID, "null handle");
  CK(cudaDeviceSynchronize());
  std::unordered_map<std::string, std::pair<int, float>> agg;
  float total = 0.f;
  for (auto& pe : h->prof_ev) {
    float ms = 0.f;
    cudaEventElapsedTime(&ms, pe.e0, pe.e1);
    auto& a = agg[pe.tag];
    a.first += 1;
    a.second += ms;
    total += ms;
    cudaEventDestroy(pe.e0);
    cudaEventDestroy(pe.e1);
  }
  h->prof_ev.clear();
  for (auto& kv : agg)
    printf("%-44s x%3d  total %8.3f ms  avg %7.1f us\n", kv.first.c_str(), kv.second.first, kv.second.second,
           1e3f * kv.second.second / kv.second.first);
  printf("projections total %.3f ms\n", total);
  fflush(stdout);
  return VASR_OK;
}

int64_t vasr_tc_launches(const vasr_handle* h) { return h ? h->tc_launches : 0; }
int64_t vasr_kernel_launches(const vasr_handle* h) { return h ? h->launches : 0; }
int64_t vasr_workspace_bytes(const vasr_handle* h) { return h ? (int64_t)h->ws.bytes : 0; }

int vasr_set_timing(vasr_handle* h, int enabled) {
  if (!h) return fail(VASR_ERR_INVALID, "null handle");
  h->timing = enabled != 0;
  return VASR_OK;
}

int vasr_last_timing(const vasr_handle* h, float* scan_ms, int32_t* scan_launches, float* total_ms) {
  if (!h) return fail(VASR_ERR_INVALID, "null handle");
  if (!h->ev_total) return fail(VASR_ERR_STATE, "timing was not enabled for the last call");
  CK(cudaEventSynchronize(h->ev_t1));
  float tot = 0.f, sc = 0.f;
  CK(cudaEventElapsedTime(&tot, h->ev_t0, h->ev_t1));
  for (int i = 0; i + 1 < h->ev_used; i += 2) {
    float ms = 0.f;
    CK(cudaEventElapsedTime(&ms, h->ev[i], h->ev[i + 1]));
    sc += ms;
  }
  if (scan_ms) *scan_ms = sc;
  if (scan_launches) *scan_launches = h->ev_used / 2;
  if (total_ms) *total_ms = tot;
  return VASR_OK;
}

}
```

velocity-asr_b200/csrc/gemm_tc.cu:

```cuda
#include <cuda.h>

#include <cstdlib>
#include <cstring>

#include "common.cuh"
#include "kernels.cuh"

namespace vasr {

namespace {

constexpr int TBM = 128, TBN = 128, TBK = 32, STAGES = 4;
constexpr int TILE_BYTES = TBM * TBK * 4;
constexpr int STAGE_BYTES = 3 * TILE_BYTES;
constexpr int EPI_WARPS = 8;
constexpr int EPI_STAGE_BYTES = 32 * 128;
constexpr int BAR_OFFSET = STAGES * STAGE_BYTES + EPI_WARPS * EPI_STAGE_BYTES;
constexpr int SMEM_BYTES = BAR_OFFSET + 256 + 1024;
constexpr int TC_THREADS = 448;
constexpr uint32_t TMEM_COLS = 512;
constexpr uint32_t TMEM_A0 = 256;
static_assert(SMEM_BYTES <= 232448, "exceeds the 227 KB of dynamic shared memory per CTA");

constexpr int B_FULL = 0, B_CONV = STAGES, B_EMPTY = 2 * STAGES, B_TFULL = 3 * STAGES, B_TEMPTY = 3 * STAGES + 2;
constexpr int N_BARS = 3 * STAGES + 4;

__device__ __forceinline__ uint32_t make_idesc(uint32_t n) {
  return (1u << 4) | (2u << 7) | (2u << 10) | ((n >> 3) << 17) | ((uint32_t)(TBM >> 4) << 24);
}

__device__ __forceinline__ uint32_t smem_u32(const void* p) { return (uint32_t)__cvta_generic_to_shared(p); }

__device__ __forceinline__ void mbar_init(uint32_t bar, uint32_t count) {
  asm volatile("mbarrier.init.shared::cta.b64 [%0], %1;" ::"r"(bar), "r"(count));
}
__device__ __forceinline__ void mbar_arrive(uint32_t bar) {
  asm volatile("mbarrier.arrive.shared::cta.b64 _, [%0];" ::"r"(bar) : "memory");
}
__device__ __forceinline__ void mbar_expect_tx(uint32_t bar, uint32_t bytes) {
  asm volatile("mbarrier.arrive.expect_tx.shared::cta.b64 _, [%0], %1;" ::"r"(bar), "r"(bytes) : "memory");
}
__device__ __forceinline__ bool mbar_try(uint32_t bar, uint32_t parity) {
  uint32_t done;
  asm volatile(
      "{\n\t.reg .pred p;\n\t"
      "mbarrier.try_wait.parity.shared::cta.b64 p, [%1], %2;\n\t"
      "selp.u32 %0, 1, 0, p;\n\t}"
      : "=r"(done)
      : "r"(bar), "r"(parity)
      : "memory");
  return done != 0;
}
__device__ __noinline__ void mbar_wait_slow(uint32_t bar, uint32_t parity) {
  const long long t0 = clock64();
  while (!mbar_try(bar, parity))
    if (clock64() - t0 > 4000000000LL) __trap();
}
__device__ __forceinline__ void mbar_wait(uint32_t bar, uint32_t parity) {
  if (!mbar_try(bar, parity)) mbar_wait_slow(bar, parity);
}

__device__ __forceinline__ void tma_load_3d(uint32_t dst, const CUtensorMap* map, int c0, int c1, int c2,
                                            uint32_t bar) {
  asm volatile(
      "cp.async.bulk.tensor.3d.shared::cluster.global.mbarrier::complete_tx::bytes [%0], [%1, {%3, %4, %5}], [%2];"
      ::"r"(dst), "l"(map), "r"(bar), "r"(c0), "r"(c1), "r"(c2)
      : "memory");
}
__device__ __forceinline__ void tma_prefetch_3d(const CUtensorMap* map, int c0, int c1, int c2) {
  asm volatile("cp.async.bulk.prefetch.tensor.3d.L2.global [%0, {%1, %2, %3}];" ::"l"(map), "r"(c0), "r"(c1), "r"(c2)
               : "memory");
}
__device__ __forceinline__ void tma_load_2d(uint32_t dst, const CUtensorMap* map, int c0, int c1, uint32_t bar) {
  asm volatile(
      "cp.async.bulk.tensor.2d.shared::cluster.global.mbarrier::complete_tx::bytes [%0], [%1, {%3, %4}], [%2];"
      ::"r"(dst), "l"(map), "r"(bar), "r"(c0), "r"(c1)
      : "memory");
}

__device__ __forceinline__ uint64_t umma_desc(uint32_t smem_addr) {
  return (uint64_t)((smem_addr & 0x3FFFF) >> 4) | (1ull << 16) | (64ull << 32) | (1ull << 46) | (2ull << 61);
}
__device__ __forceinline__ void umma_tf32_ts(uint32_t tmem_d, uint32_t tmem_a, uint64_t db, uint32_t idesc,
                                             uint32_t accumulate) {
  asm volatile(
      "{\n\t.reg .pred p;\n\t"
      "setp.ne.b32 p, %4, 0;\n\t"
      "tcgen05.mma.cta_group::1.kind::tf32 [%0], [%1], %2, %3, p;\n\t}"
      ::"r"(tmem_d), "r"(tmem_a), "l"(db), "r"(idesc), "r"(accumulate)
      : "memory");
}
__device__ __forceinline__ void umma_commit(uint32_t bar) {
  asm volatile("tcgen05.commit.cta_group::1.mbarrier::arrive::one.shared::cluster.b64 [%0];" ::"r"(bar) : "memory");
}
__device__ __forceinline__ bool elect_one() {
  uint32_t pred;
  asm volatile("{\n\t.reg .pred p;\n\telect.sync _|p, 0xffffffff;\n\tselp.u32 %0, 1, 0, p;\n\t}" : "=r"(pred));
  return pred != 0;
}
__device__ __forceinline__ void tc_fence_before() { asm volatile("tcgen05.fence::before_thread_sync;" ::: "memory"); }
__device__ __forceinline__ void tc_fence_after() { asm volatile("tcgen05.fence::after_thread_sync;" ::: "memory"); }

__device__ __forceinline__ void tmem_ld32(uint32_t taddr, uint32_t (&v)[32]) {
  asm volatile(
      "tcgen05.ld.sync.aligned.32x32b.x32.b32 "
      "{%0, %1, %2, %3, %4, %5, %6, %7, %8, %9, %10, %11, %12, %13, %14, %15, "
      "%16, %17, %18, %19, %20, %21, %22, %23, %24, %25, %26, %27, %28, %29, %30, %31}, [%32];"
      : "=r"(v[0]), "=r"(v[1]), "=r"(v[2]), "=r"(v[3]), "=r"(v[4]), "=r"(v[5]), "=r"(v[6]), "=r"(v[7]),
        "=r"(v[8]), "=r"(v[9]), "=r"(v[10]), "=r"(v[11]), "=r"(v[12]), "=r"(v[13]), "=r"(v[14]), "=r"(v[15]),
        "=r"(v[16]), "=r"(v[17]), "=r"(v[18]), "=r"(v[19]), "=r"(v[20]), "=r"(v[21]), "=r"(v[22]), "=r"(v[23]),
        "=r"(v[24]), "=r"(v[25]), "=r"(v[26]), "=r"(v[27]), "=r"(v[28]), "=r"(v[29]), "=r"(v[30]), "=r"(v[31])
      : "r"(taddr));
  asm volatile("tcgen05.wait::ld.sync.aligned;" ::: "memory");
}
__device__ __forceinline__ void tmem_ld32_issue(uint32_t taddr, uint32_t (&v)[32]) {
  asm volatile(
      "tcgen05.ld.sync.aligned.32x32b.x32.b32 "
      "{%0, %1, %2, %3, %4, %5, %6, %7, %8, %9, %10, %11, %12, %13, %14, %15, "
      "%16, %17, %18, %19, %20, %21, %22, %23, %24, %25, %26, %27, %28, %29, %30, %31}, [%32];"
      : "=r"(v[0]), "=r"(v[1]), "=r"(v[2]), "=r"(v[3]), "=r"(v[4]), "=r"(v[5]), "=r"(v[6]), "=r"(v[7]),
        "=r"(v[8]), "=r"(v[9]), "=r"(v[10]), "=r"(v[11]), "=r"(v[12]), "=r"(v[13]), "=r"(v[14]), "=r"(v[15]),
        "=r"(v[16]), "=r"(v[17]), "=r"(v[18]), "=r"(v[19]), "=r"(v[20]), "=r"(v[21]), "=r"(v[22]), "=r"(v[23]),
        "=r"(v[24]), "=r"(v[25]), "=r"(v[26]), "=r"(v[27]), "=r"(v[28]), "=r"(v[29]), "=r"(v[30]), "=r"(v[31])
      : "r"(taddr));
}
__device__ __forceinline__ void tmem_ld_wait() { asm volatile("tcgen05.wait::ld.sync.aligned;" ::: "memory"); }
__device__ __forceinline__ void tmem_st32(uint32_t taddr, const uint32_t (&v)[32]) {
  asm volatile(
      "tcgen05.st.sync.aligned.32x32b.x32.b32 [%0], "
      "{%1, %2, %3, %4, %5, %6, %7, %8, %9, %10, %11, %12, %13, %14, %15, %16, "
      "%17, %18, %19, %20, %21, %22, %23, %24, %25, %26, %27, %28, %29, %30, %31, %32};"
      ::"r"(taddr), "r"(v[0]), "r"(v[1]), "r"(v[2]), "r"(v[3]), "r"(v[4]), "r"(v[5]), "r"(v[6]), "r"(v[7]),
        "r"(v[8]), "r"(v[9]), "r"(v[10]), "r"(v[11]), "r"(v[12]), "r"(v[13]), "r"(v[14]), "r"(v[15]),
        "r"(v[16]), "r"(v[17]), "r"(v[18]), "r"(v[19]), "r"(v[20]), "r"(v[21]), "r"(v[22]), "r"(v[23]),
        "r"(v[24]), "r"(v[25]), "r"(v[26]), "r"(v[27]), "r"(v[28]), "r"(v[29]), "r"(v[30]), "r"(v[31])
      : "memory");
}

__device__ __forceinline__ uint32_t rna_tf32(float x) {
  uint32_t r;
  asm("cvt.rna.tf32.f32 %0, %1;" : "=r"(r) : "f"(x));
  return r;
}

template <int ACT>
__device__ __forceinline__ float apply_act_t(float v) {
  if (ACT == ACT_GELU) return gelu_poly(v);
  if (ACT == ACT_SOFTPLUS) return softplus_t20(v);
  if (ACT == ACT_SIGMOID) return sigmoid_f(v);
  return v;
}

struct TcArgs {
  int64_t M, N, K;
  int64_t rows_per_batch;
  int64_t n_batches;
  int m_tiles_per_batch;
  int n_tiles;
  float* C;
  int64_t ldc;
  const float* bias;
  const float* q_scale;
  const float* q_zp;
  int act_from;
  const float* resid;
  int64_t ldr;
  const float* pe_time;
  const float* pe_freq;
  int pe_half;
  int prefetch;
  int dbg;
  int rotate_n;
  int wres;
  long long* trace;
  const float* ln_s;
  float2* ln_stats;
  float ln_eps;
  float* amax_val;
  int32_t* amax_idx;
};
constexpr int EPI_LNA = 1, EPI_AMAX = 2, EPI_GATE = 4;
__device__ __forceinline__ void tile_coords(const TcArgs& g, int64_t tile64, int64_t units, int64_t* mt, int* nt) {
  const uint32_t tile = (uint32_t)tile64, n_tiles = (uint32_t)g.n_tiles;
  const uint32_t m = tile / n_tiles;
  const uint32_t per = (uint32_t)units / n_tiles > 0 ? (uint32_t)units / n_tiles : 1u;
  *mt = m;
  *nt = (int)((tile - m * n_tiles + (g.rotate_n ? m / per : 0u)) % n_tiles);
}
#ifdef VASR_TC_TRACE_MMA
#define MMA_TRACE(x) x
#else
#define MMA_TRACE(x)
#endif
constexpr int TRACE_SLOTS = 128;
constexpr int TRACE_ROLES = 16;
constexpr int TRACE_CTA = 8;
__device__ __forceinline__ void trace_cta(const TcArgs& g, int slot) {
  if (g.trace) {
    unsigned long long t;
    asm volatile("mov.u64 %0, %%globaltimer;" : "=l"(t));
    g.trace[TRACE_ROLES * TRACE_SLOTS + TRACE_CTA * blockIdx.x + slot] = (long long)t;
  }
}
__device__ __forceinline__ void trace_ev(const TcArgs& g, int role, int idx) {
  if (g.trace && blockIdx.x == 0 && idx < TRACE_SLOTS) g.trace[role * TRACE_SLOTS + idx] = clock64();
}

template <int ACT, bool PE, bool RESID, bool QUANT, bool PAIR, int EPI = 0>
__device__ __forceinline__ void epilogue_loop(const TcArgs& g, uint8_t* stg, int warp, int lane, uint32_t first_tile,
                                              uint32_t tile_stride, uint32_t total_tiles32, uint32_t units, uint32_t rank,
                                              uint32_t bar_tfull0, uint32_t bar_tempty0_local,
                                              const float2* sstats = nullptr) {
  constexpr uint32_t tmem_base = 0u;
  constexpr uint32_t TM = PAIR ? 2 * TBM : TBM;
  auto BARF = [&](uint32_t acc) { return bar_tfull0 + 8u * acc; };
  auto arrive_empty = [&](uint32_t acc) {
    if (PAIR) {
      __syncwarp();
      if (lane == 0) {
        uint32_t r;
        asm volatile("mapa.shared::cluster.u32 %0, %1, %2;" : "=r"(r) : "r"(bar_tempty0_local + 8u * acc), "r"(0u));
        asm volatile("mbarrier.arrive.shared::cluster.b64 _, [%0];" ::"r"(r) : "memory");
      }
    } else {
      mbar_arrive(bar_tempty0_local + 8u * acc);
    }
  };
  const int q = warp & 3;
  const int chalf = (warp - 6) >> 2;
    const int cc = lane & 7, rsub = lane >> 3;
  const uint32_t n_tiles = (uint32_t)g.n_tiles, mtpb = (uint32_t)g.m_tiles_per_batch;
  const uint32_t per = units / n_tiles > 0 ? units / n_tiles : 1u;
  const uint32_t rpb = (uint32_t)g.rows_per_batch;
  uint32_t it = 0;
  for (uint32_t tile = first_tile; tile < total_tiles32; tile += tile_stride, ++it) {
    if (tile + tile_stride >= total_tiles32) pdl_trigger();
    const uint32_t mt = tile / n_tiles;
    const uint32_t nt = (tile % n_tiles + (g.rotate_n ? mt / per : 0u)) % n_tiles;
    const uint32_t batch = mt / mtpb;
    const uint32_t mi0 = (mt % mtpb) * TM + rank * TBM + q * 32;
    const uint32_t ncol0 = nt * TBN;
    const uint32_t nrem = (uint32_t)g.N - ncol0;
    const int nchunks = nrem >= (uint32_t)TBN ? 4 : (int)((nrem + 31) >> 5);
    const uint32_t acc = it & 1u;
    const int c_begin = 2 * chalf, c_end = (2 * chalf + 2 < nchunks) ? 2 * chalf + 2 : nchunks;
    const uint32_t n0 = ncol0 + c_begin * 32 + 4 * cc;
    const int64_t mrow0 = (int64_t)batch * rpb + mi0;
    float* crow = g.C + mrow0 * g.ldc + n0;
    const float* rrow = RESID ? g.resid + mrow0 * g.ldr + n0 : nullptr;
    if constexpr ((EPI & EPI_AMAX) != 0) {
      static_assert(!PE && !RESID && !QUANT && ACT == ACT_NONE, "argmax epilogue: plain projection only");
      const uint32_t r = mi0 + lane;
      const int64_t grow = (int64_t)batch * rpb + r;
      const int64_t slot = ((int64_t)nt * 2 + chalf) * g.M + grow;
      mbar_wait(BARF(acc), (it >> 1) & 1u);
      tc_fence_after();
      if (c_begin >= c_end) {
        tc_fence_before();
        arrive_empty(acc);
        if (r < rpb) { g.amax_val[slot] = -INFINITY; g.amax_idx[slot] = -1; }
        continue;
      }
      uint32_t v0[32], v1[32];
      const uint32_t taddr = tmem_base + ((uint32_t)(q * 32) << 16) + acc * TBN + c_begin * 32;
      tmem_ld32_issue(taddr, v0);
      if (c_begin + 1 < c_end) tmem_ld32_issue(taddr + 32, v1);
      float rs = 1.f, ms = 0.f;
      if (EPI & EPI_LNA) {
        const float2 t = sstats[(it & 1u) * TBM + q * 32 + lane];
        rs = t.x; ms = t.y;
      }
      tmem_ld_wait();
      tc_fence_before();
      arrive_empty(acc);
      float best = -INFINITY;
      int bi = -1;
#pragma unroll
      for (int j = 0; j < 2; ++j) {
        if (c_begin + j >= c_end) break;
        const uint32_t nb = ncol0 + (c_begin + j) * 32;
#pragma unroll
        for (int k4 = 0; k4 < 8; ++k4) {
          const uint32_t n = nb + 4 * k4;
          if (n >= (uint32_t)g.N) break;
          const float4 b = g.bias ? __ldg(reinterpret_cast<const float4*>(g.bias + n)) : make_float4(0.f, 0.f, 0.f, 0.f);
          float4 t = b;
          if (EPI & EPI_LNA) {
            const float4 sc = __ldg(reinterpret_cast<const float4*>(g.ln_s + n));
            t.x = fmaf(ms, sc.x, b.x); t.y = fmaf(ms, sc.y, b.y); t.z = fmaf(ms, sc.z, b.z); t.w = fmaf(ms, sc.w, b.w);
          }
          const float a0 = __uint_as_float(j == 0 ? v0[4 * k4] : v1[4 * k4]);
          const float a1 = __uint_as_float(j == 0 ? v0[4 * k4 + 1] : v1[4 * k4 + 1]);
          const float a2 = __uint_as_float(j == 0 ? v0[4 * k4 + 2] : v1[4 * k4 + 2]);
          const float a3 = __uint_as_float(j == 0 ? v0[4 * k4 + 3] : v1[4 * k4 + 3]);
          const float x0 = (EPI & EPI_LNA) ? fmaf(rs, a0, t.x) : a0 + t.x;
          const float x1 = (EPI & EPI_LNA) ? fmaf(rs, a1, t.y) : a1 + t.y;
          const float x2 = (EPI & EPI_LNA) ? fmaf(rs, a2, t.z) : a2 + t.z;
          const float x3 = (EPI & EPI_LNA) ? fmaf(rs, a3, t.w) : a3 + t.w;
          if (x0 > best || bi < 0) { best = x0; bi = (int)n; }
          if (x1 > best) { best = x1; bi = (int)n + 1; }
          if (x2 > best) { best = x2; bi = (int)n + 2; }
          if (x3 > best) { best = x3; bi = (int)n + 3; }
        }
      }
      if (r < rpb) { g.amax_val[slot] = best; g.amax_idx[slot] = bi; }
      continue;
    }
    float4 b4[2], qs4[2], qz4[2], pf4[2];
    bool col_ok[2];
#pragma unroll
    for (int j = 0; j < 2; ++j) {
      const uint32_t n = n0 + 32 * j;
      col_ok[j] = (c_begin + j < c_end) && n < (uint32_t)g.N;
      b4[j] = qs4[j] = qz4[j] = pf4[j] = make_float4(0.f, 0.f, 0.f, 0.f);
      if (!(EPI & EPI_LNA) && col_ok[j] && g.bias) b4[j] = __ldg(reinterpret_cast<const float4*>(g.bias + n));
      if (QUANT && col_ok[j]) {
        qs4[j] = __ldg(reinterpret_cast<const float4*>(g.q_scale + n));
        qz4[j] = __ldg(reinterpret_cast<const float4*>(g.q_zp + n));
      }
      if (PE && col_ok[j] && n >= (uint32_t)g.pe_half)
        pf4[j] = __ldg(reinterpret_cast<const float4*>(g.pe_freq + (n - g.pe_half)));
    }
    float4 r4[8];
    auto load_resid = [&](int j) {
#pragma unroll
      for (int i = 0; i < 8; ++i) {
        const uint32_t rr = 4 * i + rsub;
        r4[i] = make_float4(0.f, 0.f, 0.f, 0.f);
        if (RESID && col_ok[j] && mi0 + rr < rpb)
          r4[i] = __ldg(reinterpret_cast<const float4*>(rrow + (int64_t)rr * g.ldr + 32 * j));
      }
    };
    if (RESID) load_resid(0);
    if (threadIdx.x == 192) trace_ev(g, 5, (int)it);
    mbar_wait(BARF(acc), (it >> 1) & 1u);
    if (threadIdx.x == 192) trace_ev(g, 6, (int)it);
    tc_fence_after();
    if (c_begin >= c_end) {
      tc_fence_before();
      arrive_empty(acc);
      continue;
    }
    uint32_t v0[32], v1[32];
    const uint32_t taddr = tmem_base + ((uint32_t)(q * 32) << 16) + acc * TBN + c_begin * 32;
    if (!(g.dbg & 1)) {
      tmem_ld32_issue(taddr, v0);
      if (c_begin + 1 < c_end) tmem_ld32_issue(taddr + 32, v1);
      float2 own = make_float2(1.f, 0.f);
      if constexpr ((EPI & EPI_LNA) != 0) {
        if (mi0 + lane < rpb) own = __ldcg(g.ln_stats + mrow0 + lane);
      }
      tmem_ld_wait();
      if constexpr ((EPI & EPI_LNA) != 0) {
        const u64 rs2 = pack2(own.x, own.x), ms2 = pack2(own.y, own.y);
#pragma unroll
        for (int j = 0; j < 2; ++j) {
          if (c_begin + j >= c_end) break;
          const uint32_t nb = ncol0 + (c_begin + j) * 32;
#pragma unroll
          for (int k4 = 0; k4 < 8; ++k4) {
            if (nb + 4 * k4 >= (uint32_t)g.N) break;
            const float4 sc = __ldg(reinterpret_cast<const float4*>(g.ln_s + nb + 4 * k4));
            const float4 bc = g.bias ? __ldg(reinterpret_cast<const float4*>(g.bias + nb + 4 * k4)) : make_float4(0.f, 0.f, 0.f, 0.f);
            uint32_t* v = j == 0 ? v0 : v1;
            u64 a = pack2(__uint_as_float(v[4 * k4]), __uint_as_float(v[4 * k4 + 1]));
            u64 b = pack2(__uint_as_float(v[4 * k4 + 2]), __uint_as_float(v[4 * k4 + 3]));
            a = fma2(rs2, a, fma2(ms2, pack2(sc.x, sc.y), pack2(bc.x, bc.y)));
            b = fma2(rs2, b, fma2(ms2, pack2(sc.z, sc.w), pack2(bc.z, bc.w)));
            float f0, f1, f2, f3;
            unpack2(a, f0, f1); unpack2(b, f2, f3);
            v[4 * k4] = __float_as_uint(f0); v[4 * k4 + 1] = __float_as_uint(f1);
            v[4 * k4 + 2] = __float_as_uint(f2); v[4 * k4 + 3] = __float_as_uint(f3);
          }
        }
      }
    } else {
#pragma unroll
      for (int k = 0; k < 32; ++k) v0[k] = v1[k] = 0u;
    }
    tc_fence_before();
    arrive_empty(acc);
    if (threadIdx.x == 192) trace_ev(g, 7, (int)it);
    if (g.dbg & 2) continue;
#pragma unroll
    for (int j = 0; j < 2; ++j) {
      if (c_begin + j >= c_end) break;
      {
        uint8_t* srow = stg + lane * 128;
#pragma unroll
        for (int k = 0; k < 8; ++k)
          *reinterpret_cast<uint4*>(srow + ((k ^ (lane & 7)) << 4)) =
              j == 0 ? make_uint4(v0[4 * k], v0[4 * k + 1], v0[4 * k + 2], v0[4 * k + 3])
                     : make_uint4(v1[4 * k], v1[4 * k + 1], v1[4 * k + 2], v1[4 * k + 3]);
      }
      __syncwarp();
      if (threadIdx.x == 192 && j == 0) trace_ev(g, 8, (int)it);
      const uint32_t n = n0 + 32 * j;
      const bool act_on = ACT != ACT_NONE && n >= (uint32_t)g.act_from;
#pragma unroll
      for (int i = 0; i < 8; ++i) {
        const uint32_t rr = 4 * i + rsub;
        float4 x = *reinterpret_cast<const float4*>(stg + rr * 128 + ((cc ^ (rr & 7)) << 4));
        if constexpr ((EPI & EPI_LNA) == 0) { x.x += b4[j].x; x.y += b4[j].y; x.z += b4[j].z; x.w += b4[j].w; }
        if (QUANT) {
          x.x = fake_quant_u8(x.x, qs4[j].x, qz4[j].x); x.y = fake_quant_u8(x.y, qs4[j].y, qz4[j].y);
          x.z = fake_quant_u8(x.z, qs4[j].z, qz4[j].z); x.w = fake_quant_u8(x.w, qs4[j].w, qz4[j].w);
        }
        if (act_on) {
          if (ACT == ACT_GELU) {
            gelu_poly2(x.x, x.y);
            gelu_poly2(x.z, x.w);
          } else {
            x.x = apply_act_t<ACT>(x.x); x.y = apply_act_t<ACT>(x.y);
            x.z = apply_act_t<ACT>(x.z); x.w = apply_act_t<ACT>(x.w);
          }
        }
        if (PE) {
          float4 p4 = pf4[j];
          if (n < (uint32_t)g.pe_half && col_ok[j] && mi0 + rr < rpb)
            p4 = __ldg(reinterpret_cast<const float4*>(g.pe_time + (int64_t)(mi0 + rr) * g.pe_half + n));
          x.x += p4.x; x.y += p4.y; x.z += p4.z; x.w += p4.w;
        }
        if (RESID) { x.x += r4[i].x; x.y += r4[i].y; x.z += r4[i].z; x.w += r4[i].w; }
        if (col_ok[j] && mi0 + rr < rpb) *reinterpret_cast<float4*>(crow + (int64_t)rr * g.ldc + 32 * j) = x;
      }
      __syncwarp();
      if (RESID && j == 0 && c_begin + 1 < c_end) load_resid(1);
      if (threadIdx.x == 192 && j == 0) trace_ev(g, 9, (int)it);
    }
  }
}

template <int ACT, bool RESID, int EPI = 0>
__device__ __forceinline__ void epilogue_loop192(const TcArgs& g, uint8_t* stg, float2* rowfac, const float2* sstats, int warp, int lane, uint32_t first_tile,
                                                 uint32_t tile_stride, uint32_t total_tiles32, uint32_t rank,
                                                 uint32_t bar_tfull0, uint32_t bar_tempty0_local) {
  constexpr uint32_t tmem_base = 0u;
  constexpr uint32_t TN = 192, TM = 2 * TBM;
  auto arrive_empty = [&](uint32_t acc) {
    __syncwarp();
    if (lane == 0) {
      uint32_t r;
      asm volatile("mapa.shared::cluster.u32 %0, %1, %2;" : "=r"(r) : "r"(bar_tempty0_local + 8u * acc), "r"(0u));
      asm volatile("mbarrier.arrive.shared::cluster.b64 _, [%0];" ::"r"(r) : "memory");
    }
  };
  const int q = warp & 3;
  const int chalf = (warp - 6) >> 2;
  const int cc = lane & 7, rsub = lane >> 3;
  const uint32_t n_tiles = (uint32_t)g.n_tiles, mtpb = (uint32_t)g.m_tiles_per_batch;
  const uint32_t rpb = (uint32_t)g.rows_per_batch;
  uint32_t it = 0;
  for (uint32_t tile = first_tile; tile < total_tiles32; tile += tile_stride, ++it) {
    if (tile + tile_stride >= total_tiles32) pdl_trigger();
    const uint32_t mt = tile / n_tiles, nt = tile - mt * n_tiles;
    const uint32_t batch = mt / mtpb;
    const uint32_t mi0 = (mt % mtpb) * TM + rank * TBM + q * 32;
    const uint32_t ncol0 = nt * TN;
    const uint32_t nrem = (uint32_t)g.N - ncol0;
    const int nchunks = nrem >= TN ? 6 : (int)((nrem + 31) >> 5);
    const uint32_t acc = it & 1u;
    const int c_begin = 3 * chalf, c_end = (c_begin + 3 < nchunks) ? c_begin + 3 : nchunks;
    const uint32_t n0 = ncol0 + c_begin * 32 + 4 * cc;
    const int64_t mrow0 = (int64_t)batch * rpb + mi0;
    float* crow = g.C + mrow0 * g.ldc + n0;
    const float* rrow = RESID ? g.resid + mrow0 * g.ldr + n0 : nullptr;
    float4 b4[3];
    bool col_ok[3];
#pragma unroll
    for (int j = 0; j < 3; ++j) {
      const uint32_t n = n0 + 32 * j;
      col_ok[j] = (c_begin + j < c_end) && n < (uint32_t)g.N;
      b4[j] = make_float4(0.f, 0.f, 0.f, 0.f);
      if (col_ok[j] && g.bias) b4[j] = __ldg(reinterpret_cast<const float4*>(g.bias + n));
    }
    if constexpr ((EPI & EPI_GATE) != 0) {
      static_assert(!RESID && ACT == ACT_NONE && !(EPI & EPI_LNA), "gate epilogue: plain stacked projection");
      float* orow = g.C + mrow0 * g.ldc + nt * 64 + chalf * 32 + 4 * cc;
      mbar_wait(bar_tfull0 + 8u * acc, (it >> 1) & 1u);
      tc_fence_after();
      uint32_t v0[32], v1[32];
      const uint32_t taddr = tmem_base + ((uint32_t)(q * 32) << 16) + acc * TN + c_begin * 32;
      tmem_ld32_issue(taddr, v0);
      tmem_ld32_issue(taddr + 32, v1);
      tmem_ld_wait();
      float4 gx[8], lx[8];
      auto take = [&](const uint32_t (&v)[32], int j, float4 (&o)[8]) {
        uint8_t* srow = stg + lane * 128;
#pragma unroll
        for (int k = 0; k < 8; ++k)
          *reinterpret_cast<uint4*>(srow + ((k ^ (lane & 7)) << 4)) = make_uint4(v[4 * k], v[4 * k + 1], v[4 * k + 2], v[4 * k + 3]);
        __syncwarp();
#pragma unroll
        for (int i = 0; i < 8; ++i) {
          const uint32_t rr = 4 * i + rsub;
          float4 x = *reinterpret_cast<const float4*>(stg + rr * 128 + ((cc ^ (rr & 7)) << 4));
          x.x += b4[j].x; x.y += b4[j].y; x.z += b4[j].z; x.w += b4[j].w;
          o[i] = x;
        }
        __syncwarp();
      };
      take(v0, 0, gx);
      tmem_ld32_issue(taddr + 64, v0);
      tmem_ld_wait();
      tc_fence_before();
      arrive_empty(acc);
      take(v1, 1, lx);
#pragma unroll
      for (int i = 0; i < 8; ++i) {
        gx[i].x = sigmoid_f(gx[i].x); gx[i].y = sigmoid_f(gx[i].y); gx[i].z = sigmoid_f(gx[i].z); gx[i].w = sigmoid_f(gx[i].w);
      }
      {
        uint8_t* srow = stg + lane * 128;
#pragma unroll
        for (int k = 0; k < 8; ++k)
          *reinterpret_cast<uint4*>(srow + ((k ^ (lane & 7)) << 4)) = make_uint4(v0[4 * k], v0[4 * k + 1], v0[4 * k + 2], v0[4 * k + 3]);
        __syncwarp();
#pragma unroll
        for (int i = 0; i < 8; ++i) {
          const uint32_t rr = 4 * i + rsub;
          float4 t = *reinterpret_cast<const float4*>(stg + rr * 128 + ((cc ^ (rr & 7)) << 4));
          t.x += b4[2].x; t.y += b4[2].y; t.z += b4[2].z; t.w += b4[2].w;
          float4 o;
          o.x = gx[i].x * lx[i].x + (1.0f - gx[i].x) * t.x;
          o.y = gx[i].y * lx[i].y + (1.0f - gx[i].y) * t.y;
          o.z = gx[i].z * lx[i].z + (1.0f - gx[i].z) * t.z;
          o.w = gx[i].w * lx[i].w + (1.0f - gx[i].w) * t.w;
          if (mi0 + rr < rpb) *reinterpret_cast<float4*>(orow + (int64_t)rr * g.ldc) = o;
        }
        __syncwarp();
      }
      continue;
    }
    float4 r4[8];
    auto load_resid = [&](int j) {
#pragma unroll
      for (int i = 0; i < 8; ++i) {
        const uint32_t rr = 4 * i + rsub;
        r4[i] = make_float4(0.f, 0.f, 0.f, 0.f);
        if (RESID && col_ok[j] && mi0 + rr < rpb)
          r4[i] = __ldg(reinterpret_cast<const float4*>(rrow + (int64_t)rr * g.ldr + 32 * j));
      }
    };
    if (RESID) {
      load_resid(0);
      if (cc == 0) {
#pragma unroll
        for (int j = 1; j < 3; ++j)
#pragma unroll
          for (int i = 0; i < 8; ++i) {
            const uint32_t rr = 4 * i + rsub;
            if (col_ok[j] && mi0 + rr < rpb)
              asm volatile("prefetch.global.L2 [%0];" ::"l"(rrow + (int64_t)rr * g.ldr + 32 * j));
          }
      }
    }
    mbar_wait(bar_tfull0 + 8u * acc, (it >> 1) & 1u);
    if (warp == 6 && lane == 0) { if (it == 0) trace_cta(g, 2); trace_cta(g, 4); }
    tc_fence_after();
    if (c_begin >= c_end) {
      tc_fence_before();
      arrive_empty(acc);
      continue;
    }
    uint32_t v0[32], v1[32];
    const uint32_t taddr = tmem_base + ((uint32_t)(q * 32) << 16) + acc * TN + c_begin * 32;
    tmem_ld32_issue(taddr, v0);
    if (c_begin + 1 < c_end) tmem_ld32_issue(taddr + 32, v1);
    float4 s4[3];
    if constexpr ((EPI & EPI_LNA) != 0) {
      rowfac[lane] = sstats[(it & 1u) * TBM + q * 32 + lane];
#pragma unroll
      for (int j = 0; j < 3; ++j)
        s4[j] = col_ok[j] ? __ldg(reinterpret_cast<const float4*>(g.ln_s + n0 + 32 * j)) : make_float4(0.f, 0.f, 0.f, 0.f);
    }
    tmem_ld_wait();
    auto emit = [&](const uint32_t (&v)[32], int j) {
      uint8_t* srow = stg + lane * 128;
#pragma unroll
      for (int k = 0; k < 8; ++k)
        *reinterpret_cast<uint4*>(srow + ((k ^ (lane & 7)) << 4)) = make_uint4(v[4 * k], v[4 * k + 1], v[4 * k + 2], v[4 * k + 3]);
      __syncwarp();
#pragma unroll
      for (int i = 0; i < 8; ++i) {
        const uint32_t rr = 4 * i + rsub;
        float4 x = *reinterpret_cast<const float4*>(stg + rr * 128 + ((cc ^ (rr & 7)) << 4));
        if constexpr ((EPI & EPI_LNA) != 0) {
          const float2 f = rowfac[rr];
          const u64 rs2 = pack2(f.x, f.x), ms2 = pack2(f.y, f.y);
          const u64 lo = fma2(rs2, pack2(x.x, x.y), fma2(ms2, pack2(s4[j].x, s4[j].y), pack2(b4[j].x, b4[j].y)));
          const u64 hi = fma2(rs2, pack2(x.z, x.w), fma2(ms2, pack2(s4[j].z, s4[j].w), pack2(b4[j].z, b4[j].w)));
          unpack2(lo, x.x, x.y);
          unpack2(hi, x.z, x.w);
        } else {
          const u64 lo = add2(pack2(x.x, x.y), pack2(b4[j].x, b4[j].y)), hi = add2(pack2(x.z, x.w), pack2(b4[j].z, b4[j].w));
          unpack2(lo, x.x, x.y);
          unpack2(hi, x.z, x.w);
        }
        if (ACT != ACT_NONE && n0 + 32 * j >= (uint32_t)g.act_from) {
          if (ACT == ACT_GELU) {
            gelu_poly2(x.x, x.y);
            gelu_poly2(x.z, x.w);
          } else {
            x.x = apply_act_t<ACT>(x.x); x.y = apply_act_t<ACT>(x.y);
            x.z = apply_act_t<ACT>(x.z); x.w = apply_act_t<ACT>(x.w);
          }
        }
        if (RESID) { x.x += r4[i].x; x.y += r4[i].y; x.z += r4[i].z; x.w += r4[i].w; }
        if (col_ok[j] && mi0 + rr < rpb) *reinterpret_cast<float4*>(crow + (int64_t)rr * g.ldc + 32 * j) = x;
      }
      __syncwarp();
    };
    emit(v0, 0);
    const bool has2 = c_begin + 2 < c_end;
    if (has2) {
      tmem_ld32_issue(taddr + 64, v0);
      tmem_ld_wait();
    }
    tc_fence_before();
    arrive_empty(acc);
    if (c_begin + 1 < c_end) {
      if (RESID) load_resid(1);
      emit(v1, 1);
    }
    if (has2) {
      if (RESID) load_resid(2);
      emit(v0, 2);
    }
    if (warp == 6 && lane == 0 && it == 0) trace_cta(g, 3);
  }
}

template <int ACT, bool PE, bool RESID, bool QUANT>
__global__ void __launch_bounds__(TC_THREADS, 1)
gemm_tc_kernel(const __grid_constant__ CUtensorMap tmA, const __grid_constant__ CUtensorMap tmWh,
               const __grid_constant__ CUtensorMap tmWl, const TcArgs g) {
  extern __shared__ uint8_t smem_raw[];
  uint8_t* smem = smem_raw + ((1024u - (smem_u32(smem_raw) & 1023u)) & 1023u);
  uint64_t* bars = reinterpret_cast<uint64_t*>(smem + BAR_OFFSET);
  uint32_t* tmem_slot = reinterpret_cast<uint32_t*>(bars + N_BARS);

  const int warp = threadIdx.x >> 5, lane = threadIdx.x & 31;
  const uint32_t bar0 = smem_u32(bars);
  auto BAR = [&](int i) { return bar0 + 8u * (uint32_t)i; };
  const uint32_t stage0 = smem_u32(smem);

  if (threadIdx.x == 0) {
    for (int s = 0; s < STAGES; ++s) {
      mbar_init(BAR(B_FULL + s), 1);
      mbar_init(BAR(B_CONV + s), 128);
      mbar_init(BAR(B_EMPTY + s), 1);
    }
    for (int a = 0; a < 2; ++a) {
      mbar_init(BAR(B_TFULL + a), 1);
      mbar_init(BAR(B_TEMPTY + a), EPI_WARPS * 32);
    }
    asm volatile("fence.mbarrier_init.release.cluster;" ::: "memory");
  }
  if (warp == 1) {
    asm volatile("tcgen05.alloc.cta_group::1.sync.aligned.shared::cta.b32 [%0], %1;" ::"r"(smem_u32(tmem_slot)),
                 "r"(TMEM_COLS));
    asm volatile("tcgen05.relinquish_alloc_permit.cta_group::1.sync.aligned;");
  }
  tc_fence_before();
  __syncthreads();
  tc_fence_after();
  if (*tmem_slot != 0u) __trap();
  constexpr uint32_t tmem_base = 0u;
  pdl_wait();

  const int nkb = (int)((g.K + TBK - 1) / TBK);
  const int64_t total_tiles = (int64_t)g.n_tiles * g.m_tiles_per_batch * g.n_batches;
  const int64_t UNITS = gridDim.x;
  if (threadIdx.x == 0) trace_cta(g, 0);

  if (warp == 0) {
    uint32_t stage = 0, phase = 0;
    int tr_i = 0;
    for (int64_t tile = blockIdx.x; tile < total_tiles; tile += gridDim.x) {
      int nt;
      int64_t mt;
      tile_coords(g, tile, UNITS, &mt, &nt);
      const int batch = (int)((uint32_t)mt / (uint32_t)g.m_tiles_per_batch);
      const int mi0 = (int)((uint32_t)mt % (uint32_t)g.m_tiles_per_batch) * TBM;
      if (g.prefetch && tile + gridDim.x < total_tiles) {
        int nnt;
        int64_t nmt;
        tile_coords(g, tile + gridDim.x, UNITS, &nmt, &nnt);
        const int nbatch = (int)((uint32_t)nmt / (uint32_t)g.m_tiles_per_batch);
        const int nmi0 = (int)((uint32_t)nmt % (uint32_t)g.m_tiles_per_batch) * TBM;
        if (elect_one())
          for (int kb = 0; kb < nkb; ++kb) tma_prefetch_3d(&tmA, kb * TBK, nmi0, nbatch);
        __syncwarp();
      }
      for (int kb = 0; kb < nkb; ++kb) {
        mbar_wait(BAR(B_EMPTY + stage), phase ^ 1);
        if (lane == 0) trace_ev(g, 0, tr_i);
        ++tr_i;
        const uint32_t sb = stage0 + stage * STAGE_BYTES;
        if (elect_one()) {
          mbar_expect_tx(BAR(B_FULL + stage), 3 * TILE_BYTES);
          tma_load_3d(sb, &tmA, kb * TBK, mi0, batch, BAR(B_FULL + stage));
          tma_load_2d(sb + TILE_BYTES, &tmWh, kb * TBK, nt * TBN, BAR(B_FULL + stage));
          tma_load_2d(sb + 2 * TILE_BYTES, &tmWl, kb * TBK, nt * TBN, BAR(B_FULL + stage));
        }
        __syncwarp();
        if (++stage == STAGES) { stage = 0; phase ^= 1; }
      }
    }
  } else if (warp == 1) {
    uint32_t stage = 0, phase = 0;
    int64_t it = 0;
    int tr_i = 0;
    for (int64_t tile = blockIdx.x; tile < total_tiles; tile += gridDim.x, ++it) {
      int nt;
      int64_t mt_unused;
      tile_coords(g, tile, UNITS, &mt_unused, &nt);
      int64_t nrem = g.N - (int64_t)nt * TBN;
      const uint32_t n_mma = nrem >= TBN ? (uint32_t)TBN : (uint32_t)((nrem + 15) & ~15LL);
      const uint32_t idesc = make_idesc(n_mma);
      const uint32_t acc = (uint32_t)(it & 1);
      mbar_wait(BAR(B_TEMPTY + acc), (uint32_t)((it >> 1) & 1) ^ 1);
      tc_fence_after();
      const uint32_t tmem_d = tmem_base + acc * TBN;
      for (int kb = 0; kb < nkb; ++kb) {
        mbar_wait(BAR(B_FULL + stage), phase);
        mbar_wait(BAR(B_CONV + stage), phase);
        tc_fence_after();
        if (lane == 0) trace_ev(g, 3, tr_i);
        const uint32_t sb = stage0 + stage * STAGE_BYTES;
        const uint64_t db_hi = umma_desc(sb + TILE_BYTES), db_lo = umma_desc(sb + 2 * TILE_BYTES);
        const uint32_t a_hi = tmem_base + TMEM_A0 + stage * 64, a_lo = a_hi + 32;
        if (elect_one()) {
#pragma unroll
          for (int k4 = 0; k4 < TBK / 8; ++k4) {
            const uint64_t adv = (uint64_t)(k4 * 2);
            umma_tf32_ts(tmem_d, a_lo + 8 * k4, db_hi + adv, idesc, (kb | k4) != 0);
            umma_tf32_ts(tmem_d, a_hi + 8 * k4, db_lo + adv, idesc, 1);
            umma_tf32_ts(tmem_d, a_hi + 8 * k4, db_hi + adv, idesc, 1);
          }
          umma_commit(BAR(B_EMPTY + stage));
          if (kb == nkb - 1) umma_commit(BAR(B_TFULL + acc));
          trace_ev(g, 4, tr_i);
        }
        ++tr_i;
        __syncwarp();
        if (++stage == STAGES) { stage = 0; phase ^= 1; }
      }
    }
  } else if (warp < 6) {
    const int quad = warp & 3;
    const int row = quad * 32 + lane;
    const uint32_t lane_addr = tmem_base + ((uint32_t)(quad * 32) << 16) + TMEM_A0;
    uint32_t stage = 0, phase = 0;
    int tr_i = 0;
    for (int64_t tile = blockIdx.x; tile < total_tiles; tile += gridDim.x) {
      for (int kb = 0; kb < nkb; ++kb) {
        mbar_wait(BAR(B_FULL + stage), phase);
        if (threadIdx.x == 64) trace_ev(g, 1, tr_i);
        const uint8_t* arow = smem + stage * STAGE_BYTES + row * 128;
        uint32_t hi[32], lo[32];
#pragma unroll
        for (int c = 0; c < 8; ++c) {
          const float4 v = *reinterpret_cast<const float4*>(arow + ((c ^ (row & 7)) << 4));
          hi[4 * c + 0] = rna_tf32(v.x); lo[4 * c + 0] = rna_tf32(v.x - __uint_as_float(hi[4 * c + 0]));
          hi[4 * c + 1] = rna_tf32(v.y); lo[4 * c + 1] = rna_tf32(v.y - __uint_as_float(hi[4 * c + 1]));
          hi[4 * c + 2] = rna_tf32(v.z); lo[4 * c + 2] = rna_tf32(v.z - __uint_as_float(hi[4 * c + 2]));
          hi[4 * c + 3] = rna_tf32(v.w); lo[4 * c + 3] = rna_tf32(v.w - __uint_as_float(hi[4 * c + 3]));
        }
        tc_fence_after();
        tmem_st32(lane_addr + stage * 64, hi);
        tmem_st32(lane_addr + stage * 64 + 32, lo);
        asm volatile("tcgen05.wait::st.sync.aligned;" ::: "memory");
        tc_fence_before();
        mbar_arrive(BAR(B_CONV + stage));
        if (threadIdx.x == 64) trace_ev(g, 2, tr_i);
        ++tr_i;
        if (++stage == STAGES) { stage = 0; phase ^= 1; }
      }
    }
  } else {
    epilogue_loop<ACT, PE, RESID, QUANT, false>(g, smem + STAGES * STAGE_BYTES + (warp - 6) * EPI_STAGE_BYTES, warp, lane,
                                                blockIdx.x, gridDim.x, (uint32_t)total_tiles, (uint32_t)UNITS, 0u,
                                                BAR(B_TFULL), BAR(B_TEMPTY));
  }

  tc_fence_before();
  __syncthreads();
  if (threadIdx.x == 0) trace_cta(g, 7);
  if (warp == 1) {
    tc_fence_after();
    asm volatile("tcgen05.dealloc.cta_group::1.sync.aligned.b32 %0, %1;" ::"r"(tmem_base), "r"(TMEM_COLS));
  }
}

constexpr int P_STAGE_BYTES = 2 * TILE_BYTES;
constexpr int P_STAGES = 6;
constexpr int P_ASLOTS = 4;
constexpr int P_BAR_OFFSET = P_STAGES * P_STAGE_BYTES + EPI_WARPS * EPI_STAGE_BYTES;
constexpr int P_SMEM_BYTES = P_BAR_OFFSET + 512 + 1024;
static_assert(P_SMEM_BYTES <= 232448, "exceeds the 227 KB of dynamic shared memory per CTA");
constexpr int PB_AFULL = 0, PB_WFULL = P_STAGES, PB_CONV = 2 * P_STAGES, PB_EMPTY = 3 * P_STAGES,
              PB_TFULL = 4 * P_STAGES, PB_TEMPTY = 4 * P_STAGES + 2, PB_AFREE = 4 * P_STAGES + 4;
constexpr int P_NBARS = 4 * P_STAGES + 4 + P_ASLOTS;

template <int TN>
struct PairCfg {
  static constexpr int W_HALF_BYTES = (TN / 2) * TBK * 4;
  static constexpr int STAGE_BYTES = TILE_BYTES + 2 * W_HALF_BYTES;
  static constexpr int STAGES = TN == 128 ? 6 : 4;
  static constexpr int ASLOTS = TN == 128 ? 4 : 2;
  static constexpr uint32_t A0 = 2 * TN;
  static constexpr int BAR_OFFSET = STAGES * STAGE_BYTES + EPI_WARPS * EPI_STAGE_BYTES;
  static constexpr int ROWFAC_OFFSET = BAR_OFFSET + 512;
  static constexpr int SMEM_BYTES = BAR_OFFSET + 512 + (TN == 192 ? EPI_WARPS * 256 + 2 * TBM * 8 : 0) + 1024;
  static constexpr int AFULL = 0, WFULL = STAGES, CONV = 2 * STAGES, EMPTY = 3 * STAGES, TFULL = 4 * STAGES,
                       TEMPTY = 4 * STAGES + 2, AFREE = 4 * STAGES + 4, NBARS = 4 * STAGES + 4 + ASLOTS;
  static_assert(SMEM_BYTES <= 232448, "exceeds the 227 KB of dynamic shared memory per CTA");
  static_assert(A0 + ASLOTS * 64 <= 512, "tensor memory");
};
static_assert(PairCfg<128>::STAGE_BYTES == P_STAGE_BYTES && PairCfg<128>::SMEM_BYTES == P_SMEM_BYTES, "TN = 128 is the layout above");

__device__ __forceinline__ uint32_t cluster_ctarank() {
  uint32_t r;
  asm volatile("mov.u32 %0, %%cluster_ctarank;" : "=r"(r));
  return r;
}
__device__ __forceinline__ void cluster_sync_all() {
  asm volatile("barrier.cluster.arrive.release.aligned;" ::: "memory");
  asm volatile("barrier.cluster.wait.acquire.aligned;" ::: "memory");
}
__device__ __forceinline__ uint32_t mapa(uint32_t addr, uint32_t rank) {
  uint32_t r;
  asm volatile("mapa.shared::cluster.u32 %0, %1, %2;" : "=r"(r) : "r"(addr), "r"(rank));
  return r;
}
__device__ __forceinline__ void mbar_arrive_cluster(uint32_t cluster_addr) {
  asm volatile("mbarrier.arrive.shared::cluster.b64 _, [%0];" ::"r"(cluster_addr) : "memory");
}
__device__ __forceinline__ bool mbar_try_cluster(uint32_t bar, uint32_t parity) {
  uint32_t done;
  asm volatile(
      "{\n\t.reg .pred p;\n\t"
      "mbarrier.try_wait.parity.shared::cta.b64 p, [%1], %2;\n\t"
      "selp.u32 %0, 1, 0, p;\n\t}"
      : "=r"(done)
      : "r"(bar), "r"(parity)
      : "memory");
  return done != 0;
}
__device__ __noinline__ void mbar_wait_cluster_slow(uint32_t bar, uint32_t parity) {
  const long long t0 = clock64();
  while (!mbar_try_cluster(bar, parity))
    if (clock64() - t0 > 4000000000LL) __trap();
}
__device__ __forceinline__ void mbar_wait_cluster(uint32_t bar, uint32_t parity) {
  if (!mbar_try_cluster(bar, parity)) mbar_wait_cluster_slow(bar, parity);
}
__device__ __forceinline__ void tma_load_2d_pair(uint32_t dst, const CUtensorMap* map, int c0, int c1,
                                                 uint32_t leader_bar) {
  asm volatile(
      "cp.async.bulk.tensor.2d.cta_group::2.shared::cluster.global.mbarrier::complete_tx::bytes [%0], [%1, {%3, %4}], [%2];"
      ::"r"(dst), "l"(map), "r"(leader_bar), "r"(c0), "r"(c1)
      : "memory");
}
__device__ __forceinline__ void umma_tf32_ts_pair(uint32_t tmem_d, uint32_t tmem_a, uint64_t db, uint32_t idesc,
                                                  uint32_t accumulate) {
  asm volatile(
      "{\n\t.reg .pred p;\n\t"
      "setp.ne.b32 p, %4, 0;\n\t"
      "tcgen05.mma.cta_group::2.kind::tf32 [%0], [%1], %2, %3, p;\n\t}"
      ::"r"(tmem_d), "r"(tmem_a), "l"(db), "r"(idesc), "r"(accumulate)
      : "memory");
}
__device__ __forceinline__ void umma_commit_pair(uint32_t bar) {
  asm volatile(
      "tcgen05.commit.cta_group::2.mbarrier::arrive::one.shared::cluster.multicast::cluster.b64 [%0], %1;"
      ::"r"(bar), "h"((uint16_t)3)
      : "memory");
}

template <int ACT, bool PE, bool RESID, bool QUANT, bool WRES = false, int TN = 128, int EPI = 0>
#ifdef VASR_TC_MAXNREG
__global__ void __cluster_dims__(2, 1, 1) __maxnreg__(144)
#else
__global__ void __cluster_dims__(2, 1, 1) __launch_bounds__(TC_THREADS, 1)
#endif
gemm_tc2_kernel(const __grid_constant__ CUtensorMap tmA, const __grid_constant__ CUtensorMap tmWh,
                const __grid_constant__ CUtensorMap tmWl, const TcArgs g) {
  using Cfg = PairCfg<TN>;
  constexpr int TBN = TN;
  constexpr int P_STAGE_BYTES = Cfg::STAGE_BYTES, P_STAGES = Cfg::STAGES, P_ASLOTS = Cfg::ASLOTS;
  constexpr int P_BAR_OFFSET = Cfg::BAR_OFFSET, P_NBARS = Cfg::NBARS;
  constexpr int PB_AFULL = Cfg::AFULL, PB_WFULL = Cfg::WFULL, PB_CONV = Cfg::CONV, PB_EMPTY = Cfg::EMPTY,
                PB_TFULL = Cfg::TFULL, PB_TEMPTY = Cfg::TEMPTY, PB_AFREE = Cfg::AFREE;
  constexpr uint32_t TMEM_A0 = Cfg::A0;
  constexpr int W_HALF_BYTES = Cfg::W_HALF_BYTES;
  static_assert(!(WRES && TN != 128), "the W-resident schedule exists for 128-column tiles only");
  constexpr bool SSTATS = (EPI & EPI_LNA) != 0 && (TN == 192 || (EPI & EPI_AMAX) != 0);
  extern __shared__ uint8_t smem_raw[];
  uint8_t* smem = smem_raw + ((1024u - (smem_u32(smem_raw) & 1023u)) & 1023u);
  uint64_t* bars = reinterpret_cast<uint64_t*>(smem + P_BAR_OFFSET);
  uint32_t* tmem_slot = reinterpret_cast<uint32_t*>(bars + P_NBARS);

  if (threadIdx.x == 0) {
    asm volatile("prefetch.tensormap [%0];" ::"l"(reinterpret_cast<uint64_t>(&tmA)) : "memory");
    asm volatile("prefetch.tensormap [%0];" ::"l"(reinterpret_cast<uint64_t>(&tmWh)) : "memory");
    asm volatile("prefetch.tensormap [%0];" ::"l"(reinterpret_cast<uint64_t>(&tmWl)) : "memory");
  }
  if (threadIdx.x == 0) trace_cta(g, 0);
  const int warp = threadIdx.x >> 5, lane = threadIdx.x & 31;
  const uint32_t rank = cluster_ctarank();
  const bool leader = rank == 0;
  const uint32_t bar0 = smem_u32(bars);
  auto BAR = [&](int i) { return bar0 + 8u * (uint32_t)i; };
  const uint32_t stage0 = smem_u32(smem);
  float2* sstats = reinterpret_cast<float2*>(TN == 192 ? smem + Cfg::ROWFAC_OFFSET + EPI_WARPS * 256
                                                       : smem + P_STAGES * P_STAGE_BYTES);

  if (threadIdx.x == 0) {
    for (int s = 0; s < P_STAGES; ++s) {
      mbar_init(BAR(PB_AFULL + s), 1);
      mbar_init(BAR(PB_WFULL + s), 1);
      mbar_init(BAR(PB_CONV + s), 8);
      mbar_init(BAR(PB_EMPTY + s), 1);
    }
    for (int a = 0; a < 2; ++a) {
      mbar_init(BAR(PB_TFULL + a), 1);
      mbar_init(BAR(PB_TEMPTY + a), 2 * EPI_WARPS);
    }
    for (int a = 0; a < P_ASLOTS; ++a) mbar_init(BAR(PB_AFREE + a), 1);
    asm volatile("fence.mbarrier_init.release.cluster;" ::: "memory");
  }
  if (warp == 1) {
    asm volatile("tcgen05.alloc.cta_group::2.sync.aligned.shared::cta.b32 [%0], %1;" ::"r"(smem_u32(tmem_slot)),
                 "r"(TMEM_COLS));
    asm volatile("tcgen05.relinquish_alloc_permit.cta_group::2.sync.aligned;");
  }
  tc_fence_before();
  __syncthreads();
  cluster_sync_all();
  tc_fence_after();
  if (*tmem_slot != 0u) __trap();
  constexpr uint32_t tmem_base = 0u;
  if (threadIdx.x == 0) trace_cta(g, 6);
  pdl_wait();
  if (threadIdx.x == 0) trace_cta(g, 1);

  const int nkb = (int)((g.K + TBK - 1) / TBK);
  const int64_t total_tiles = (int64_t)g.n_tiles * g.m_tiles_per_batch * g.n_batches;
  const int64_t pair = blockIdx.x >> 1, npairs = gridDim.x >> 1;
  const int64_t UNITS = npairs;
  int64_t first_tile = pair, tile_stride = npairs;
  if (WRES) {
    const int64_t slot = pair / g.n_tiles, nt_own = pair % g.n_tiles;
    first_tile = slot < g.wres ? slot * g.n_tiles + nt_own : total_tiles;
    tile_stride = (int64_t)g.wres * g.n_tiles;
  }

  if (warp == 0) {
    uint32_t stage = 0, phase = 0, cnt = 0;
    int tr_i = 0;
    for (int64_t tile = first_tile; tile < total_tiles; tile += tile_stride) {
      int nt;
      int64_t mt;
      tile_coords(g, tile, UNITS, &mt, &nt);
      const int batch = (int)((uint32_t)mt / (uint32_t)g.m_tiles_per_batch);
      const int mi0 = (int)((uint32_t)mt % (uint32_t)g.m_tiles_per_batch) * 2 * TBM + (int)rank * TBM;
      int64_t nrem = g.N - (int64_t)nt * TBN;
      const int n_mma = nrem >= TBN ? TBN : (int)((nrem + 15) & ~15LL);
      const int wrow = nt * TBN + (int)rank * (n_mma / 2);
      for (int kb = 0; kb < nkb; ++kb) {
        mbar_wait_cluster(BAR(PB_EMPTY + stage), phase ^ 1);
        if (lane == 0) trace_ev(g, 0, tr_i);
        ++tr_i;
        const uint32_t sb = stage0 + stage * P_STAGE_BYTES;
        const uint32_t wbar = mapa(BAR(PB_WFULL + stage), 0);
        const bool load_w = !WRES || cnt < (uint32_t)P_STAGES;
        if (elect_one()) {
          mbar_expect_tx(BAR(PB_AFULL + stage), TILE_BYTES);
          tma_load_3d(sb, &tmA, kb * TBK, mi0, batch, BAR(PB_AFULL + stage));
          if (load_w) {
            if (leader) mbar_expect_tx(BAR(PB_WFULL + stage), 4 * W_HALF_BYTES);
            tma_load_2d_pair(sb + TILE_BYTES, &tmWh, kb * TBK, wrow, wbar);
            tma_load_2d_pair(sb + TILE_BYTES + W_HALF_BYTES, &tmWl, kb * TBK, wrow, wbar);
          }
        }
        __syncwarp();
        ++cnt;
        if (++stage == P_STAGES) { stage = 0; phase ^= 1; }
      }
    }
  } else if (warp == 1) {
    if (leader) {
      uint32_t stage = 0, phase = 0, cnt = 0;
      uint32_t it = 0;
      int tr_i = 0;
      for (int64_t tile = first_tile; tile < total_tiles; tile += tile_stride, ++it) {
        MMA_TRACE(if (lane == 0) trace_ev(g, 10, (int)it);)
        int nt;
        int64_t mt_unused;
        tile_coords(g, tile, UNITS, &mt_unused, &nt);
        const int64_t nrem = g.N - (int64_t)nt * TBN;
        const uint32_t n_mma = nrem >= TBN ? (uint32_t)TBN : (uint32_t)((nrem + 15) & ~15LL);
        const uint32_t idesc = (1u << 4) | (2u << 7) | (2u << 10) | ((n_mma >> 3) << 17) | ((256u >> 4) << 24);
        const uint32_t acc = it & 1u;
        mbar_wait_cluster(BAR(PB_TEMPTY + acc), ((it >> 1) & 1u) ^ 1u);
        tc_fence_after();
        MMA_TRACE(if (lane == 0) trace_ev(g, 11, (int)it);)
        const uint32_t tmem_d = tmem_base + acc * TBN;
#pragma unroll 1
        for (int kb = 0; kb < nkb; ++kb) {
          if (!WRES || cnt < (uint32_t)P_STAGES) mbar_wait_cluster(BAR(PB_WFULL + stage), phase);
          mbar_wait_cluster(BAR(PB_CONV + stage), phase);
          tc_fence_after();
          MMA_TRACE(if (lane == 0) trace_ev(g, 3, tr_i);)
          const uint32_t sb = stage0 + stage * P_STAGE_BYTES;
          const uint64_t db_hi = umma_desc(sb + TILE_BYTES), db_lo = umma_desc(sb + TILE_BYTES + W_HALF_BYTES);
          const uint32_t slot = cnt % P_ASLOTS;
          const uint32_t a_hi = tmem_base + TMEM_A0 + slot * 64, a_lo = a_hi + 32;
          if (elect_one()) {
#pragma unroll
            for (int k4 = 0; k4 < TBK / 8; ++k4) {
              const uint64_t adv = (uint64_t)(k4 * 2);
              umma_tf32_ts_pair(tmem_d, a_lo + 8 * k4, db_hi + adv, idesc, (kb | k4) != 0);
              umma_tf32_ts_pair(tmem_d, a_hi + 8 * k4, db_lo + adv, idesc, 1);
              umma_tf32_ts_pair(tmem_d, a_hi + 8 * k4, db_hi + adv, idesc, 1);
            }
            umma_commit_pair(BAR(PB_EMPTY + stage));
            umma_commit_pair(BAR(PB_AFREE + slot));
            if (kb == nkb - 1) umma_commit_pair(BAR(PB_TFULL + acc));
            MMA_TRACE(trace_ev(g, 4, tr_i);)
          }
          ++tr_i;
          ++cnt;
          __syncwarp();
          if (++stage == P_STAGES) { stage = 0; phase ^= 1; }
        }
      }
    }
  } else if (warp < 6) {
    const int quad = warp & 3;
    const int row = quad * 32 + lane;
    const uint32_t lane_addr = tmem_base + ((uint32_t)(quad * 32) << 16) + TMEM_A0;
    uint32_t stage = 0, phase = 0, cnt = 0, cit = 0;
    int tr_i = 0;
    for (int64_t tile = first_tile; tile < total_tiles; tile += tile_stride, ++cit) {
      u64 sum2[2] = {0ull, 0ull}, sq2[2] = {0ull, 0ull}, shift2 = 0ull;
      for (int kb = 0; kb < nkb; ++kb) {
        mbar_wait(BAR(PB_AFULL + stage), phase);
        if (threadIdx.x == 64) trace_ev(g, 1, tr_i);
        const uint8_t* arow = smem + stage * P_STAGE_BYTES + row * 128;
        if constexpr ((EPI & EPI_LNA) != 0) {
          if (kb == 0) {
            u64 s0 = 0ull, s1 = 0ull;
#pragma unroll
            for (int c = 0; c < 8; ++c) {
              const float4 v = *reinterpret_cast<const float4*>(arow + ((c ^ (row & 7)) << 4));
              s0 = add2(s0, pack2(v.x, v.y)); s1 = add2(s1, pack2(v.z, v.w));
            }
            const float shift = (hsum2(s0) + hsum2(s1)) * (1.0f / 32.0f);
            shift2 = pack2(-shift, -shift);
          }
        }
        uint32_t hi[32], lo[32];
#pragma unroll
        for (int c = 0; c < 8; ++c) {
          float4 v = *reinterpret_cast<const float4*>(arow + ((c ^ (row & 7)) << 4));
          if constexpr ((EPI & EPI_LNA) != 0) {
            const u64 a = add2(pack2(v.x, v.y), shift2), b = add2(pack2(v.z, v.w), shift2);
            sum2[0] = add2(sum2[0], a); sum2[1] = add2(sum2[1], b);
            sq2[0] = fma2(a, a, sq2[0]); sq2[1] = fma2(b, b, sq2[1]);
            unpack2(a, v.x, v.y);
            unpack2(b, v.z, v.w);
          }
          hi[4 * c + 0] = rna_tf32(v.x); lo[4 * c + 0] = rna_tf32(v.x - __uint_as_float(hi[4 * c + 0]));
          hi[4 * c + 1] = rna_tf32(v.y); lo[4 * c + 1] = rna_tf32(v.y - __uint_as_float(hi[4 * c + 1]));
          hi[4 * c + 2] = rna_tf32(v.z); lo[4 * c + 2] = rna_tf32(v.z - __uint_as_float(hi[4 * c + 2]));
          hi[4 * c + 3] = rna_tf32(v.w); lo[4 * c + 3] = rna_tf32(v.w - __uint_as_float(hi[4 * c + 3]));
        }
        if constexpr ((EPI & EPI_LNA) != 0) {
          if (kb == nkb - 1) {
            const float inv = 1.0f / (float)g.K;
            if constexpr (SSTATS) {
              const float dm = (hsum2(sum2[0]) + hsum2(sum2[1])) * inv;
              const float var = fmaxf(fmaf(-dm, dm, (hsum2(sq2[0]) + hsum2(sq2[1])) * inv), 0.f);
              const float rstd = 1.0f / sqrtf(var + g.ln_eps);
              sstats[(cit & 1u) * TBM + row] = make_float2(rstd, -dm * rstd);
            } else {
            int nt_unused;
            int64_t mt;
            tile_coords(g, tile, UNITS, &mt, &nt_unused);
            const uint32_t r = ((uint32_t)mt % (uint32_t)g.m_tiles_per_batch) * 2u * TBM + rank * TBM + (uint32_t)row;
            if (r < (uint32_t)g.rows_per_batch) {
              const float dm = (hsum2(sum2[0]) + hsum2(sum2[1])) * inv;
              const float var = fmaxf(fmaf(-dm, dm, (hsum2(sq2[0]) + hsum2(sq2[1])) * inv), 0.f);
              const float rstd = 1.0f / sqrtf(var + g.ln_eps);
              g.ln_stats[(int64_t)((uint32_t)mt / (uint32_t)g.m_tiles_per_batch) * g.rows_per_batch + r] =
                  make_float2(rstd, -dm * rstd);
            }
            }
          }
        }
        const uint32_t slot = cnt % P_ASLOTS;
        mbar_wait(BAR(PB_AFREE + slot), ((cnt / P_ASLOTS) & 1u) ^ 1u);
        tc_fence_after();
        tmem_st32(lane_addr + slot * 64, hi);
        tmem_st32(lane_addr + slot * 64 + 32, lo);
        asm volatile("tcgen05.wait::st.sync.aligned;" ::: "memory");
        tc_fence_before();
        __syncwarp();
        if (lane == 0) mbar_arrive_cluster(mapa(BAR(PB_CONV + stage), 0));
        if (threadIdx.x == 64) trace_ev(g, 2, tr_i);
        ++tr_i;
        ++cnt;
        if (++stage == P_STAGES) { stage = 0; phase ^= 1; }
      }
    }
  } else {
    if constexpr (TN == 192) {
      static_assert(TN != 192 || (ACT != ACT_SIGMOID && !PE && !QUANT), "192-column tiles: no pos-enc / quantised / sigmoid epilogue");
      epilogue_loop192<ACT, RESID, EPI>(g, smem + P_STAGES * P_STAGE_BYTES + (warp - 6) * EPI_STAGE_BYTES,
                              reinterpret_cast<float2*>(smem + Cfg::ROWFAC_OFFSET) + (warp - 6) * 32, sstats, warp, lane,
                              (uint32_t)first_tile, (uint32_t)tile_stride, (uint32_t)total_tiles, rank, BAR(PB_TFULL),
                              BAR(PB_TEMPTY));
    } else {
      static_assert(!(EPI & EPI_GATE), "the gate epilogue exists for 192-column tiles only");
      epilogue_loop<ACT, PE, RESID, QUANT, true, EPI>(g, smem + P_STAGES * P_STAGE_BYTES + (warp - 6) * EPI_STAGE_BYTES, warp, lane,
                                                 (uint32_t)first_tile, (uint32_t)tile_stride, (uint32_t)total_tiles, (uint32_t)UNITS, rank,
                                                 BAR(PB_TFULL), BAR(PB_TEMPTY), sstats);
    }
  }

  if (threadIdx.x == 6 * 32) trace_cta(g, 5);
  tc_fence_before();
  __syncthreads();
  cluster_sync_all();
  if (threadIdx.x == 0) trace_cta(g, 7);
  if (warp == 1) {
    tc_fence_after();
    asm volatile("tcgen05.dealloc.cta_group::2.sync.aligned.b32 %0, %1;" ::"r"(tmem_base), "r"(TMEM_COLS));
  }
}

__global__ void __launch_bounds__(256) split_tf32_kernel(const float* __restrict__ w, float* __restrict__ hl,
                                                         int64_t n) {
  const int64_t i = (int64_t)blockIdx.x * 256 + threadIdx.x;
  if (i >= n) return;
  const float x = w[i];
  const float h = __uint_as_float(rna_tf32(x));
  hl[i] = h;
  hl[n + i] = __uint_as_float(rna_tf32(x - h));
}

typedef CUresult (*EncodeTiledFn)(CUtensorMap*, CUtensorMapDataType, cuuint32_t, void*, const cuuint64_t*,
                                  const cuuint64_t*, const cuuint32_t*, const cuuint32_t*, CUtensorMapInterleave,
                                  CUtensorMapSwizzle, CUtensorMapL2promotion, CUtensorMapFloatOOBfill);

EncodeTiledFn encode_fn() {
  static EncodeTiledFn fn = nullptr;
  static bool tried = false;
  if (!tried) {
    tried = true;
    void* p = nullptr;
    cudaDriverEntryPointQueryResult qres;
    if (cudaGetDriverEntryPoint("cuTensorMapEncodeTiled", &p, cudaEnableDefault, &qres) == cudaSuccess &&
        qres == cudaDriverEntryPointSuccess)
      fn = reinterpret_cast<EncodeTiledFn>(p);
  }
  return fn;
}

bool make_map(CUtensorMap* map, const float* base, int rank, const uint64_t* dims, const uint64_t* strides_bytes,
              const uint32_t* box) {
  EncodeTiledFn fn = encode_fn();
  if (!fn) return false;
  cuuint64_t gd[3], gs[2];
  cuuint32_t bx[3], es[3] = {1, 1, 1};
  for (int i = 0; i < rank; ++i) { gd[i] = dims[i]; bx[i] = box[i]; }
  for (int i = 0; i + 1 < rank; ++i) gs[i] = strides_bytes[i];
  CUresult r = fn(map, CU_TENSOR_MAP_DATA_TYPE_FLOAT32, (cuuint32_t)rank, const_cast<float*>(base), gd, gs, bx, es,
                  CU_TENSOR_MAP_INTERLEAVE_NONE, CU_TENSOR_MAP_SWIZZLE_128B, CU_TENSOR_MAP_L2_PROMOTION_L2_128B,
                  CU_TENSOR_MAP_FLOAT_OOB_FILL_NONE);
  return r == CUDA_SUCCESS;
}

}

long long* g_trace = nullptr;

bool gemm_tc_supported(const GemmArgs& g) {
  if (!encode_fn()) return false;
  if (g.K % 4 != 0 || g.lda % 4 != 0 || g.batch_stride % 4 != 0) return false;
  auto al16 = [](const void* p) { return (reinterpret_cast<uintptr_t>(p) & 15) == 0; };
  if (!al16(g.A) || !al16(g.W_split)) return false;
  if ((g.N & 3) || (g.ldc & 3) || !al16(g.C) || (g.act_from & 3)) return false;
  if (g.bias && !al16(g.bias)) return false;
  if (g.q_scale && (!g.q_zp || !al16(g.q_scale) || !al16(g.q_zp))) return false;
  if (g.resid && ((g.ldr & 3) || !al16(g.resid))) return false;
  if (g.pe_time && ((g.pe_half & 3) || !al16(g.pe_time) || !al16(g.pe_freq))) return false;
  return true;
}

cudaError_t launch_split_tf32(const float* w, float* hl, int64_t n, cudaStream_t s) {
  if (n <= 0) return cudaSuccess;
  split_tf32_kernel<<<(unsigned)((n + 255) / 256), 256, 0, s>>>(w, hl, n);
  return cudaGetLastError();
}

cudaError_t launch_gemm_tc(const GemmArgs& g, int num_sms, cudaStream_t s, int64_t* launches) {
  if (g.M <= 0 || g.N <= 0) return cudaSuccess;
  if (!g.W_split || !gemm_tc_supported(g)) return cudaErrorNotSupported;
  const int64_t rpb = g.rows_per_batch > 0 ? g.rows_per_batch : g.M;
  const int64_t nb = g.rows_per_batch > 0 ? g.M / g.rows_per_batch : 1;
  if (nb * rpb != g.M) return cudaErrorNotSupported;
  if (g.pe_time && g.pe_rows != rpb) return cudaErrorNotSupported;
  const int64_t bstride = g.rows_per_batch > 0 ? g.batch_stride : rpb * g.lda;

  static const bool use_pair = debug_env_int("VASR_TC_PAIR", 1) != 0;
  const bool pair = use_pair && num_sms >= 2;
  static const int t192_env = debug_env_int("VASR_TC_T192", 1);
  const bool lna = g.ln_s != nullptr, amax = g.amax_val != nullptr, gate = g.gate != 0;
  if (lna && (!pair || !g.ln_stats || g.K % TBK != 0 || g.K / TBK <= 4 || g.pe_time || g.resid || g.q_scale ||
              !(reinterpret_cast<uintptr_t>(g.ln_s) % 16 == 0) || !(g.act == ACT_NONE || (g.act == ACT_GELU && !amax))))
    return cudaErrorNotSupported;
  if (amax && (!pair || !g.amax_idx || g.act != ACT_NONE || g.pe_time || g.resid || g.q_scale || gate)) return cudaErrorNotSupported;
  if (gate && (!pair || lna || g.act != ACT_NONE || g.pe_time || g.resid || g.q_scale || g.N % 192 != 0)) return cudaErrorNotSupported;
  const bool inst192 = !g.pe_time && !g.q_scale && !amax && (!lna || g.act == ACT_GELU) &&
                       (g.act == ACT_NONE || ((g.act == ACT_SOFTPLUS || g.act == ACT_GELU) && !g.resid));
  const int64_t r192 = g.N % 192;
  bool t192 = pair && t192_env && inst192 && (r192 == 0 || r192 >= TBN);
  if (t192_env == 2 && g.N % TBN == 0) t192 = false;
  if (gate && !t192) return cudaErrorNotSupported;
  if (lna && g.act == ACT_GELU && !t192) return cudaErrorNotSupported;
  const int tn = t192 ? 192 : TBN;
  CUtensorMap tmA, tmWh, tmWl;
  {
    const uint64_t dims[3] = {(uint64_t)g.K, (uint64_t)rpb, (uint64_t)nb};
    const uint64_t str[2] = {(uint64_t)g.lda * 4, (uint64_t)(bstride > 0 ? bstride : g.lda) * 4};
    const uint32_t box[3] = {TBK, TBM, 1};
    if (!make_map(&tmA, g.A, 3, dims, str, box)) return cudaErrorNotSupported;
  }
  {
    const uint64_t dims[2] = {(uint64_t)g.K, (uint64_t)g.N};
    const uint64_t str[1] = {(uint64_t)g.K * 4};
    const uint32_t box[2] = {TBK, (uint32_t)(pair ? tn / 2 : tn)};
    if (!make_map(&tmWh, g.W_split, 2, dims, str, box)) return cudaErrorNotSupported;
    if (!make_map(&tmWl, g.W_split + g.N * g.K, 2, dims, str, box)) return cudaErrorNotSupported;
  }
  TcArgs a;
  a.M = g.M; a.N = g.N; a.K = g.K;
  a.rows_per_batch = rpb;
  a.n_batches = nb;
  a.m_tiles_per_batch = (int)((rpb + (pair ? 2 : 1) * TBM - 1) / ((pair ? 2 : 1) * TBM));
  a.n_tiles = (int)((g.N + tn - 1) / tn);
  a.C = g.C; a.ldc = g.ldc; a.bias = g.bias; a.act_from = g.act_from;
  a.q_scale = g.q_scale; a.q_zp = g.q_zp;
  a.resid = g.resid; a.ldr = g.ldr;
  a.pe_time = g.pe_time; a.pe_freq = g.pe_freq; a.pe_half = g.pe_half;
  a.ln_s = g.ln_s; a.ln_stats = reinterpret_cast<float2*>(g.ln_stats); a.ln_eps = g.ln_eps;
  a.amax_val = g.amax_val; a.amax_idx = g.amax_idx;
  a.trace = g_trace;
  static const int rot_env = debug_env_int("VASR_TC_ROT", 1);
  a.rotate_n = rot_env;
  static const int dbg_env = debug_env_int("VASR_TC_DBG", 0);
  a.dbg = dbg_env;
  static const int pf_env = debug_env_int("VASR_TC_PREFETCH", 0);
  a.prefetch = pf_env;

  const int64_t tiles = (int64_t)a.n_tiles * a.m_tiles_per_batch * nb;
  if (tiles >= (1LL << 31) || rpb >= (1LL << 31)) return cudaErrorNotSupported;
  const int64_t units = pair ? num_sms / 2 : num_sms;
  const unsigned grid = (unsigned)((tiles < units ? tiles : units) * (pair ? 2 : 1));
  static const int wres_env = debug_env_int("VASR_TC_WRES", 1);
  a.wres = 0;
  if (pair && wres_env) {
    const int64_t nkb = (g.K + TBK - 1) / TBK, per = units / a.n_tiles, m_tiles = (int64_t)a.m_tiles_per_batch * nb;
    if (nkb <= P_STAGES && P_STAGES % nkb == 0 && per >= 1 && m_tiles >= 4 * per && (int64_t)grid == 2 * units) {
      a.wres = (int)per;
    }
  }
  const bool pe = g.pe_time != nullptr, rs = g.resid != nullptr;
  if (pe || rs || g.q_scale || !(g.act == ACT_NONE || g.act == ACT_GELU) || t192) a.wres = 0;
  if (a.wres) a.rotate_n = 0;
  cudaError_t err = cudaSuccess;
  auto go1 = [&](auto kernel) {
    err = cudaFuncSetAttribute(kernel, cudaFuncAttributeMaxDynamicSharedMemorySize, SMEM_BYTES);
    if (err == cudaSuccess) err = launch_k(kernel, dim3(grid), dim3(TC_THREADS), SMEM_BYTES, s, tmA, tmWh, tmWl, a);
  };
  auto go2 = [&](auto kernel) {
    err = cudaFuncSetAttribute(kernel, cudaFuncAttributeMaxDynamicSharedMemorySize, P_SMEM_BYTES);
    if (err == cudaSuccess) err = launch_k(kernel, dim3(grid), dim3(TC_THREADS), P_SMEM_BYTES, s, tmA, tmWh, tmWl, a);
  };
  auto go192 = [&](auto kernel) {
    err = cudaFuncSetAttribute(kernel, cudaFuncAttributeMaxDynamicSharedMemorySize, PairCfg<192>::SMEM_BYTES);
    if (err == cudaSuccess)
      err = launch_k(kernel, dim3(grid), dim3(TC_THREADS), PairCfg<192>::SMEM_BYTES, s, tmA, tmWh, tmWl, a);
  };
  if (t192) {
    a.rotate_n = 0;
    if (gate) go192(gemm_tc2_kernel<ACT_NONE, false, false, false, false, 192, EPI_GATE>);
    else if (lna) go192(gemm_tc2_kernel<ACT_GELU, false, false, false, false, 192, EPI_LNA>);
    else if (g.act == ACT_SOFTPLUS) go192(gemm_tc2_kernel<ACT_SOFTPLUS, false, false, false, false, 192>);
    else if (g.act == ACT_GELU) go192(gemm_tc2_kernel<ACT_GELU, false, false, false, false, 192>);
    else if (rs) go192(gemm_tc2_kernel<ACT_NONE, false, true, false, false, 192>);
    else go192(gemm_tc2_kernel<ACT_NONE, false, false, false, false, 192>);
    if (err != cudaSuccess) return err;
    if (launches) ++*launches;
    return cudaSuccess;
  }
  if (lna || amax) {
    if (a.wres) {
      if (lna && amax) go2(gemm_tc2_kernel<ACT_NONE, false, false, false, true, 128, EPI_LNA | EPI_AMAX>);
      else if (lna) go2(gemm_tc2_kernel<ACT_NONE, false, false, false, true, 128, EPI_LNA>);
      else go2(gemm_tc2_kernel<ACT_NONE, false, false, false, true, 128, EPI_AMAX>);
    } else {
      if (lna && amax) go2(gemm_tc2_kernel<ACT_NONE, false, false, false, false, 128, EPI_LNA | EPI_AMAX>);
      else if (lna) go2(gemm_tc2_kernel<ACT_NONE, false, false, false, false, 128, EPI_LNA>);
      else go2(gemm_tc2_kernel<ACT_NONE, false, false, false, false, 128, EPI_AMAX>);
    }
    if (err != cudaSuccess) return err;
    if (launches) ++*launches;
    return cudaSuccess;
  }
  const bool quant = g.q_scale != nullptr;
  if (quant) {
    if (rs || !((g.act == ACT_NONE && !pe) || (g.act == ACT_GELU && pe))) return cudaErrorNotSupported;
    if (pair) {
      if (pe) go2(gemm_tc2_kernel<ACT_GELU, true, false, true>);
      else go2(gemm_tc2_kernel<ACT_NONE, false, false, true>);
    } else {
      if (pe) go1(gemm_tc_kernel<ACT_GELU, true, false, true>);
      else go1(gemm_tc_kernel<ACT_NONE, false, false, true>);
    }
  }
#define VASR_TC_CASE(ACTV)                                                                   \
  if (!quant && g.act == ACTV) {                                                             \
    if (pair) {                                                                              \
      if (pe && rs) go2(gemm_tc2_kernel<ACTV, true, true, false>);                           \
      else if (pe) go2(gemm_tc2_kernel<ACTV, true, false, false>);                           \
      else if (rs) go2(gemm_tc2_kernel<ACTV, false, true, false>);                           \
      else if (a.wres && ACTV == ACT_NONE) go2(gemm_tc2_kernel<ACT_NONE, false, false, false, true>);   \
      else if (a.wres && ACTV == ACT_GELU) go2(gemm_tc2_kernel<ACT_GELU, false, false, false, true>);   \
      else go2(gemm_tc2_kernel<ACTV, false, false, false>);                                  \
    } else {                                                                                 \
      if (pe && rs) go1(gemm_tc_kernel<ACTV, true, true, false>);                            \
      else if (pe) go1(gemm_tc_kernel<ACTV, true, false, false>);                            \
      else if (rs) go1(gemm_tc_kernel<ACTV, false, true, false>);                            \
      else go1(gemm_tc_kernel<ACTV, false, false, false>);                                   \
    }                                                                                        \
  }
  VASR_TC_CASE(ACT_NONE)
  VASR_TC_CASE(ACT_GELU)
  VASR_TC_CASE(ACT_SOFTPLUS)
  VASR_TC_CASE(ACT_SIGMOID)
#undef VASR_TC_CASE
  if (err != cudaSuccess) return err;
  if (launches) ++*launches;
  return cudaSuccess;
}

}
```

velocity-asr_b200/csrc/kernels.cuh:

```cuda
#pragma once
#include <cuda_runtime.h>
#include <stdint.h>

namespace vasr {

struct GemmArgs {
  const float* A = nullptr;
  int64_t lda = 0;
  int64_t rows_per_batch = 0;
  int64_t batch_stride = 0;
  const float* W = nullptr;
  const float* W_split = nullptr;
  const float* bias = nullptr;
  const float* q_scale = nullptr;
  const float* q_zp = nullptr;
  float* C = nullptr;
  int64_t ldc = 0;
  int64_t M = 0, N = 0, K = 0;
  int act = 0;
  int act_from = 0;
  const float* resid = nullptr;
  int64_t ldr = 0;
  const float* ln_s = nullptr;
  float* ln_stats = nullptr;
  float ln_eps = 1e-5f;
  float* amax_val = nullptr;
  int32_t* amax_idx = nullptr;
  int gate = 0;
  const float* pe_time = nullptr;
  const float* pe_freq = nullptr;
  int pe_half = 0;
  int64_t pe_rows = 0;
};
cudaError_t launch_gemm(const GemmArgs& g, cudaStream_t s, int64_t* launches);
cudaError_t launch_gemm_tc(const GemmArgs& g, int num_sms, cudaStream_t s, int64_t* launches);
cudaError_t launch_split_tf32(const float* w, float* hl, int64_t n, cudaStream_t s);
extern long long* g_trace;

cudaError_t launch_minmax(const float* x, int64_t ldx, int64_t M, int c0, int nc, float* mm, cudaStream_t s,
                          int64_t* launches);
cudaError_t launch_set_qparams(const float* mm, float* q_scale, float* q_zp, int c0, int nc, cudaStream_t s,
                               int64_t* launches);

cudaError_t launch_layer_norm(const float* x, int64_t ldx, float* y, int64_t ldy, const float* gamma,
                              const float* beta, int64_t M, int C, cudaStream_t s, int64_t* launches);
cudaError_t launch_ln_dwconv(const float* x, float* u, const float* gamma, const float* beta,
                             const float* w, const float* bias, int64_t B, int64_t L, int C, int k,
                             cudaStream_t s, int64_t* launches);

struct ScanArgs {
  const float* x = nullptr;   int64_t ldx = 0;
  const float* dt = nullptr;  int64_t lddt = 0;
  const float* z = nullptr;   int64_t ldz = 0;
  const float* Bm = nullptr;  int64_t ldb = 0;
  const float* Cm = nullptr;  int64_t ldc = 0;
  const float* A = nullptr;
  const float* D = nullptr;
  float* y = nullptr;         int64_t ldy = 0;
  int64_t B = 0, L = 0;
  int Di = 0, N = 0;
  int parallel_quirk = 0;
  int structured_a = 0;
  int num_sms = 0;
};
cudaError_t launch_selective_scan(const ScanArgs& a, cudaStream_t s, int64_t* launches);

enum { RAG_S = 0, RAG_T = 1, RAG_L = 2, RAG_K1 = 3, RAG_K2 = 4, RAG_STRIDE = 8 };

int64_t mel_fft_blocks(int64_t T);
cudaError_t launch_mel_fft(const float* pcm, float* raw, double* part, int64_t B, int64_t S, int64_t T, int n_mels,
                           const int* fb_lo, const int* fb_off, const float* fb_w, const float* win,
                           const float* tw, cudaStream_t s, int64_t* launches, const int32_t* rag = nullptr);
cudaError_t launch_mel_finish(const float* raw, const float* mean, const float* rstd, float* out, int64_t B,
                              int64_t T, int n_mels, int64_t frames_per_utt, int front, cudaStream_t s,
                              int64_t* launches, const int32_t* rag = nullptr, const double* part = nullptr);

cudaError_t launch_adaptive_pool(const float* x, int64_t ldx, float* out, int64_t B, int64_t L, int64_t K,
                                 int C, cudaStream_t s, int64_t* launches, const int32_t* rag = nullptr,
                                 int f_in = 0, int f_out = 0);
cudaError_t launch_attention(const float* q, int64_t ldq, const float* kv, float* o, int64_t ldo, int64_t B,
                             int64_t L, int64_t Kk, int heads, int hd, cudaStream_t s, int64_t* launches,
                             const int32_t* rag = nullptr);
cudaError_t launch_gate_mix(const float* f3, float* out, int64_t M, int C, cudaStream_t s, int64_t* launches);

cudaError_t launch_argmax(const float* logits, int32_t* pred, int64_t M, int V, cudaStream_t s,
                          int64_t* launches);
cudaError_t launch_ctc_runs(const int32_t* pred, int32_t* tokens, int32_t* starts, int32_t* ends, int32_t* lens,
                            int64_t B, int64_t L, int blank, cudaStream_t s, int64_t* launches);
inline int argmax_slots(int64_t N) { return (int)(2 * ((N + 127) / 128)); }
cudaError_t launch_ctc_collapse(int32_t* pred, int32_t* tokens, int32_t* lens, int64_t B, int64_t L,
                                int blank, int collapse, cudaStream_t s, int64_t* launches,
                                const int32_t* rag = nullptr, const float* amax_val = nullptr,
                                const int32_t* amax_idx = nullptr, int slots = 0);

cudaError_t launch_beam_rows(const float* logits, float2* stats, int32_t* top_tok, int64_t M, int V, int K,
                             int blank, cudaStream_t s, int64_t* launches);
cudaError_t launch_beam_search(const float* logits, const float2* stats, const int32_t* top_tok, int K, int64_t B,
                               int64_t L, int V, int W, int blank, int32_t* trie, int64_t trie_cap,
                               int32_t* out_tokens, int32_t* out_lens, double* out_scores, cudaStream_t s,
                               int64_t* launches);

}
```

Baseline: 194,500.

## Stream in-projection and x/dt projection GEMMs in one persistent kernel with row flags

Fuses the Mamba block's input projection and the following x/B/C/dt projection into one persistent tcgen05 GEMM launch. Tiles of the two stages are interleaved with a lag, and the second stage waits on per-row-tile global flags that the first stage's epilogue publishes with release/acquire atomics. This removes a launch boundary and the tail gap between two dependent GEMMs, and lets the second GEMM start while the first is still finishing. The cost is spin-waiting and an extra fence in the epilogue. A wrong lag or the scheduling order could stall CTAs or deadlock, so the wait loop traps after a long timeout.

```diff
diff --git a/velocity-asr_b200/csrc/engine.cu b/velocity-asr_b200/csrc/engine.cu
--- a/velocity-asr_b200/csrc/engine.cu
+++ b/velocity-asr_b200/csrc/engine.cu
@@ -546,6 +546,33 @@
   return VASR_OK;
 }
 
+int gemm_stream(vasr_handle* h, GemmArgs& g0, GemmArgs& g1, cudaStream_t s) {
+  RET(split_of(h, g0.W, g0.N * g0.K, s, &g0.W_split));
+  RET(split_of(h, g1.W, g1.N * g1.K, s, &g1.W_split));
+  vasr_handle::ProfEntry pe;
+  if (h->prof) {
+    pe.tag = "stream M" + std::to_string(g0.M) + " K" + std::to_string(g0.K) + " N" + std::to_string(g0.N) + " -> K" +
+             std::to_string(g1.K) + " N" + std::to_string(g1.N) + " act" + std::to_string(g1.act);
+    CK(cudaEventCreate(&pe.e0));
+    CK(cudaEventCreate(&pe.e1));
+    CK(cudaEventRecord(pe.e0, s));
+  }
+  const cudaError_t e = launch_gemm_tc_stream(g0, g1, h->num_sms, s, &h->launches);
+  if (e == cudaErrorNotSupported) {
+    (void)cudaGetLastError();
+    if (h->prof) { CK(cudaEventDestroy(pe.e0)); CK(cudaEventDestroy(pe.e1)); }
+    RET(gemm(h, g0, s));
+    return gemm(h, g1, s);
+  }
+  if (e != cudaSuccess) return fail(VASR_ERR_CUDA, std::string("launch_gemm_tc_stream: ") + cudaGetErrorString(e));
+  ++h->tc_launches;
+  if (h->prof) {
+    CK(cudaEventRecord(pe.e1, s));
+    h->prof_ev.push_back(pe);
+  }
+  return VASR_OK;
+}
+
 int gemm_q(vasr_handle* h, GemmArgs& g, int site, float* qscratch, cudaStream_t s) {
   if (site >= 0 && h->quant_active) {
     const QSite& q = h->qsite[site];
@@ -604,9 +631,13 @@
   const int d = h->cfg.d_model, di = w.di;
   const int64_t M = B * L;
   KL(launch_ln_dwconv(x, k.u, w.ln1_g, w.ln1_b, w.conv_w, w.conv_b, B, L, d, w.ks, s, &h->launches));
-  RET(linear(h, k.u, d, w.w_in, nullptr, k.xz, 2 * di, M, d, 2 * di, ACT_NONE, 0, nullptr, 0, s));
-  RET(linear(h, k.xz, 2 * di, w.w_xdt, w.b_xdt, k.bcdt, 2 * w.N + di, M, di, 2 * w.N + di, ACT_SOFTPLUS, 2 * w.N,
-             nullptr, 0, s));
+  {
+    GemmArgs gi, gx;
+    gi.A = k.u; gi.lda = d; gi.W = w.w_in; gi.C = k.xz; gi.ldc = 2 * di; gi.M = M; gi.K = d; gi.N = 2 * di;
+    gx.A = k.xz; gx.lda = 2 * di; gx.W = w.w_xdt; gx.bias = w.b_xdt; gx.C = k.bcdt; gx.ldc = 2 * w.N + di;
+    gx.M = M; gx.K = di; gx.N = 2 * w.N + di; gx.act = ACT_SOFTPLUS; gx.act_from = 2 * w.N;
+    RET(gemm_stream(h, gi, gx, s));
+  }
   RET(run_scan(h, w, k, B, L, quirk, s));
   RET(linear(h, k.yg, di, w.w_out, nullptr, x1, d, M, di, d, ACT_NONE, 0, x, d, s));
   if (w.s_f1) {
@@ -1469,6 +1500,23 @@
   return VASR_OK;
 }
 
+int vasr_debug_linear_stream(const float* x_dev, int64_t k0, const float* w0_split, float* out0, int64_t n0,
+                             int64_t k1, const float* w1_split, const float* b1, float* out1, int64_t n1, int act_from1,
+                             int64_t M, void* stream) {
+  if (!x_dev || !w0_split || !out0 || !w1_split || !out1) return fail(VASR_ERR_INVALID, "null argument");
+  int dev = 0, sms = 148;
+  CK(cudaGetDevice(&dev));
+  CK(cudaDeviceGetAttribute(&sms, cudaDevAttrMultiProcessorCount, dev));
+  GemmArgs g0, g1;
+  g0.A = x_dev; g0.lda = k0; g0.W_split = w0_split; g0.C = out0; g0.ldc = n0; g0.M = M; g0.K = k0; g0.N = n0;
+  g1.A = out0; g1.lda = n0; g1.W_split = w1_split; g1.bias = b1; g1.C = out1; g1.ldc = n1; g1.M = M; g1.K = k1;
+  g1.N = n1; g1.act = act_from1 < n1 ? ACT_SOFTPLUS : ACT_NONE; g1.act_from = act_from1 < n1 ? act_from1 : 0;
+  const cudaError_t e = launch_gemm_tc_stream(g0, g1, sms, static_cast<cudaStream_t>(stream), nullptr);
+  if (e == cudaErrorNotSupported) return fail(VASR_ERR_UNSUPPORTED, "shapes not taken by the tile stream");
+  if (e != cudaSuccess) return fail(VASR_ERR_CUDA, std::string("launch_gemm_tc_stream: ") + cudaGetErrorString(e));
+  return VASR_OK;
+}
+
 int vasr_debug_gemm_trace(long long* dev_buf) {
   g_trace = dev_buf;
   return VASR_OK;
diff --git a/velocity-asr_b200/csrc/gemm_tc.cu b/velocity-asr_b200/csrc/gemm_tc.cu
--- a/velocity-asr_b200/csrc/gemm_tc.cu
+++ b/velocity-asr_b200/csrc/gemm_tc.cu
@@ -2,6 +2,10 @@
 
 #include <cstdlib>
 #include <cstring>
+#include <map>
+#include <mutex>
+#include <type_traits>
+#include <utility>
 
 #include "common.cuh"
 #include "kernels.cuh"
@@ -180,6 +184,55 @@
   int32_t* amax_idx;
 };
 constexpr int EPI_LNA = 1, EPI_AMAX = 2, EPI_GATE = 4;
+
+struct TcStream {
+  CUtensorMap tmA, tmWh, tmWl;
+  TcArgs g;
+  unsigned int* flags;
+  unsigned int* count;
+  unsigned int epoch;
+  int lag;
+  int dep_ntiles;
+};
+struct NoStream {};
+
+__device__ __forceinline__ void stream_tile(uint32_t t, uint32_t m, uint32_t n0, uint32_t n1, uint32_t lag,
+                                            uint32_t* stage, uint32_t* mt, uint32_t* nt) {
+  const uint32_t a = n0 * lag, step = n0 + n1, b = a + step * (m - lag);
+  if (t < a) {
+    *stage = 0; *mt = t / n0; *nt = t - *mt * n0;
+  } else if (t < b) {
+    const uint32_t u = t - a, r = u / step, j = u - r * step;
+    if (j < n0) { *stage = 0; *mt = lag + r; *nt = j; }
+    else { *stage = 1; *mt = r; *nt = j - n0; }
+  } else {
+    const uint32_t u = t - b, r = u / n1;
+    *stage = 1; *mt = m - lag + r; *nt = u - r * n1;
+  }
+}
+__device__ __forceinline__ void stream_signal(const TcStream* st, uint32_t mt, int lane) {
+  __threadfence();
+  __syncwarp();
+  if (lane == 0) {
+    unsigned int old;
+    asm volatile("atom.add.acq_rel.gpu.global.u32 %0, [%1], 1;" : "=r"(old) : "l"(st->count + mt) : "memory");
+    if (old + 1 == 2u * EPI_WARPS * (uint32_t)st->dep_ntiles) {
+      st->count[mt] = 0;
+      asm volatile("st.release.gpu.global.u32 [%0], %1;" ::"l"(st->flags + mt), "r"(st->epoch) : "memory");
+    }
+  }
+}
+__device__ __noinline__ void stream_wait(const unsigned int* flag, unsigned int epoch) {
+  const long long t0 = clock64();
+  for (;;) {
+    unsigned int v;
+    asm volatile("ld.acquire.gpu.global.u32 %0, [%1];" : "=r"(v) : "l"(flag) : "memory");
+    if (v == epoch) break;
+    if (clock64() - t0 > 4000000000LL) __trap();
+    __nanosleep(64);
+  }
+  asm volatile("fence.proxy.async.global;" ::: "memory");
+}
 __device__ __forceinline__ void tile_coords(const TcArgs& g, int64_t tile64, int64_t units, int64_t* mt, int* nt) {
   const uint32_t tile = (uint32_t)tile64, n_tiles = (uint32_t)g.n_tiles;
   const uint32_t m = tile / n_tiles;
@@ -431,10 +484,12 @@
   }
 }
 
-template <int ACT, bool RESID, int EPI = 0>
+template <int ACT, bool RESID, int EPI = 0, bool STREAM = false>
 __device__ __forceinline__ void epilogue_loop192(const TcArgs& g, uint8_t* stg, float2* rowfac, const float2* sstats, int warp, int lane, uint32_t first_tile,
                                                  uint32_t tile_stride, uint32_t total_tiles32, uint32_t rank,
-                                                 uint32_t bar_tfull0, uint32_t bar_tempty0_local) {
+                                                 uint32_t bar_tfull0, uint32_t bar_tempty0_local,
+                                                 const TcStream* st = nullptr) {
+  static_assert(!STREAM || (EPI == 0 && !RESID), "tile stream: plain / activation epilogues");
   constexpr uint32_t tmem_base = 0u;
   constexpr uint32_t TN = 192, TM = 2 * TBM;
   auto arrive_empty = [&](uint32_t acc) {
@@ -453,26 +508,30 @@
   uint32_t it = 0;
   for (uint32_t tile = first_tile; tile < total_tiles32; tile += tile_stride, ++it) {
     if (tile + tile_stride >= total_tiles32) pdl_trigger();
-    const uint32_t mt = tile / n_tiles, nt = tile - mt * n_tiles;
+    uint32_t stage = 0, mt, nt;
+    if constexpr (STREAM) stream_tile(tile, mtpb, n_tiles, (uint32_t)st->g.n_tiles, (uint32_t)st->lag, &stage, &mt, &nt);
+    else { mt = tile / n_tiles; nt = tile - mt * n_tiles; }
+#define VASR_TG(f) (STREAM && stage ? st->g.f : g.f)
+    const bool publish = STREAM && stage == 0 && nt < (uint32_t)st->dep_ntiles;
     const uint32_t batch = mt / mtpb;
     const uint32_t mi0 = (mt % mtpb) * TM + rank * TBM + q * 32;
     const uint32_t ncol0 = nt * TN;
-    const uint32_t nrem = (uint32_t)g.N - ncol0;
+    const uint32_t nrem = (uint32_t)VASR_TG(N) - ncol0;
     const int nchunks = nrem >= TN ? 6 : (int)((nrem + 31) >> 5);
     const uint32_t acc = it & 1u;
     const int c_begin = 3 * chalf, c_end = (c_begin + 3 < nchunks) ? c_begin + 3 : nchunks;
     const uint32_t n0 = ncol0 + c_begin * 32 + 4 * cc;
     const int64_t mrow0 = (int64_t)batch * rpb + mi0;
-    float* crow = g.C + mrow0 * g.ldc + n0;
+    float* crow = VASR_TG(C) + mrow0 * VASR_TG(ldc) + n0;
     const float* rrow = RESID ? g.resid + mrow0 * g.ldr + n0 : nullptr;
     float4 b4[3];
     bool col_ok[3];
 #pragma unroll
     for (int j = 0; j < 3; ++j) {
       const uint32_t n = n0 + 32 * j;
-      col_ok[j] = (c_begin + j < c_end) && n < (uint32_t)g.N;
+      col_ok[j] = (c_begin + j < c_end) && n < (uint32_t)VASR_TG(N);
       b4[j] = make_float4(0.f, 0.f, 0.f, 0.f);
-      if (col_ok[j] && g.bias) b4[j] = __ldg(reinterpret_cast<const float4*>(g.bias + n));
+      if (col_ok[j] && VASR_TG(bias)) b4[j] = __ldg(reinterpret_cast<const float4*>(VASR_TG(bias) + n));
     }
     if constexpr ((EPI & EPI_GATE) != 0) {
       static_assert(!RESID && ACT == ACT_NONE && !(EPI & EPI_LNA), "gate epilogue: plain stacked projection");
@@ -561,6 +620,7 @@
     if (c_begin >= c_end) {
       tc_fence_before();
       arrive_empty(acc);
+      if (publish) stream_signal(st, mt, lane);
       continue;
     }
     uint32_t v0[32], v1[32];
@@ -576,6 +636,8 @@
     }
     tmem_ld_wait();
     auto emit = [&](const uint32_t (&v)[32], int j) {
+      const int64_t ldc_j = VASR_TG(ldc);
+      const bool act_j = ACT != ACT_NONE && n0 + 32 * j >= (uint32_t)VASR_TG(act_from);
       uint8_t* srow = stg + lane * 128;
 #pragma unroll
       for (int k = 0; k < 8; ++k)
@@ -597,7 +659,7 @@
           unpack2(lo, x.x, x.y);
           unpack2(hi, x.z, x.w);
         }
-        if (ACT != ACT_NONE && n0 + 32 * j >= (uint32_t)g.act_from) {
+        if (STREAM ? act_j : ACT != ACT_NONE && n0 + 32 * j >= (uint32_t)g.act_from) {
           if (ACT == ACT_GELU) {
             gelu_poly2(x.x, x.y);
             gelu_poly2(x.z, x.w);
@@ -607,7 +669,7 @@
           }
         }
         if (RESID) { x.x += r4[i].x; x.y += r4[i].y; x.z += r4[i].z; x.w += r4[i].w; }
-        if (col_ok[j] && mi0 + rr < rpb) *reinterpret_cast<float4*>(crow + (int64_t)rr * g.ldc + 32 * j) = x;
+        if (col_ok[j] && mi0 + rr < rpb) *reinterpret_cast<float4*>(crow + (int64_t)rr * (STREAM ? ldc_j : g.ldc) + 32 * j) = x;
       }
       __syncwarp();
     };
@@ -627,7 +689,9 @@
       if (RESID) load_resid(2);
       emit(v0, 2);
     }
+    if (publish) stream_signal(st, mt, lane);
     if (warp == 6 && lane == 0 && it == 0) trace_cta(g, 3);
+#undef VASR_TG
   }
 }
 
@@ -880,14 +944,16 @@
       : "memory");
 }
 
-template <int ACT, bool PE, bool RESID, bool QUANT, bool WRES = false, int TN = 128, int EPI = 0>
+template <int ACT, bool PE, bool RESID, bool QUANT, bool WRES = false, int TN = 128, int EPI = 0, bool STREAM = false>
 #ifdef VASR_TC_MAXNREG
 __global__ void __cluster_dims__(2, 1, 1) __maxnreg__(144)
 #else
 __global__ void __cluster_dims__(2, 1, 1) __launch_bounds__(TC_THREADS, 1)
 #endif
 gemm_tc2_kernel(const __grid_constant__ CUtensorMap tmA, const __grid_constant__ CUtensorMap tmWh,
-                const __grid_constant__ CUtensorMap tmWl, const TcArgs g) {
+                const __grid_constant__ CUtensorMap tmWl, const TcArgs g,
+                const __grid_constant__ std::conditional_t<STREAM, TcStream, NoStream> st) {
+  static_assert(!STREAM || (TN == 192 && !WRES && !PE && !QUANT && !RESID && EPI == 0), "tile stream: 192-column plain / activation tiles");
   using Cfg = PairCfg<TN>;
   constexpr int TBN = TN;
   constexpr int P_STAGE_BYTES = Cfg::STAGE_BYTES, P_STAGES = Cfg::STAGES, P_ASLOTS = Cfg::ASLOTS;
@@ -907,6 +973,11 @@
     asm volatile("prefetch.tensormap [%0];" ::"l"(reinterpret_cast<uint64_t>(&tmA)) : "memory");
     asm volatile("prefetch.tensormap [%0];" ::"l"(reinterpret_cast<uint64_t>(&tmWh)) : "memory");
     asm volatile("prefetch.tensormap [%0];" ::"l"(reinterpret_cast<uint64_t>(&tmWl)) : "memory");
+    if constexpr (STREAM) {
+      asm volatile("prefetch.tensormap [%0];" ::"l"(reinterpret_cast<uint64_t>(&st.tmA)) : "memory");
+      asm volatile("prefetch.tensormap [%0];" ::"l"(reinterpret_cast<uint64_t>(&st.tmWh)) : "memory");
+      asm volatile("prefetch.tensormap [%0];" ::"l"(reinterpret_cast<uint64_t>(&st.tmWl)) : "memory");
+    }
   }
   if (threadIdx.x == 0) trace_cta(g, 0);
   const int warp = threadIdx.x >> 5, lane = threadIdx.x & 31;
@@ -948,9 +1019,27 @@
   if (threadIdx.x == 0) trace_cta(g, 1);
 
   const int nkb = (int)((g.K + TBK - 1) / TBK);
-  const int64_t total_tiles = (int64_t)g.n_tiles * g.m_tiles_per_batch * g.n_batches;
+  int64_t total_tiles = (int64_t)g.n_tiles * g.m_tiles_per_batch * g.n_batches;
   const int64_t pair = blockIdx.x >> 1, npairs = gridDim.x >> 1;
   const int64_t UNITS = npairs;
+  int nkb1 = nkb;
+  int64_t N1 = g.N;
+  if constexpr (STREAM) {
+    nkb1 = (int)((st.g.K + TBK - 1) / TBK);
+    N1 = st.g.N;
+    total_tiles += (int64_t)st.g.n_tiles * g.m_tiles_per_batch;
+  }
+  auto coords = [&](int64_t tile, uint32_t* stage, int64_t* mt, int* nt) {
+    if constexpr (STREAM) {
+      uint32_t m, n;
+      stream_tile((uint32_t)tile, (uint32_t)g.m_tiles_per_batch, (uint32_t)g.n_tiles, (uint32_t)st.g.n_tiles,
+                  (uint32_t)st.lag, stage, &m, &n);
+      *mt = m; *nt = (int)n;
+    } else {
+      *stage = 0;
+      tile_coords(g, tile, UNITS, mt, nt);
+    }
+  };
   int64_t first_tile = pair, tile_stride = npairs;
   if (WRES) {
     const int64_t slot = pair / g.n_tiles, nt_own = pair % g.n_tiles;
@@ -962,15 +1051,24 @@
     uint32_t stage = 0, phase = 0, cnt = 0;
     int tr_i = 0;
     for (int64_t tile = first_tile; tile < total_tiles; tile += tile_stride) {
+      uint32_t s;
       int nt;
       int64_t mt;
-      tile_coords(g, tile, UNITS, &mt, &nt);
+      coords(tile, &s, &mt, &nt);
       const int batch = (int)((uint32_t)mt / (uint32_t)g.m_tiles_per_batch);
       const int mi0 = (int)((uint32_t)mt % (uint32_t)g.m_tiles_per_batch) * 2 * TBM + (int)rank * TBM;
-      int64_t nrem = g.N - (int64_t)nt * TBN;
+      int64_t nrem = (s ? N1 : g.N) - (int64_t)nt * TBN;
       const int n_mma = nrem >= TBN ? TBN : (int)((nrem + 15) & ~15LL);
       const int wrow = nt * TBN + (int)rank * (n_mma / 2);
-      for (int kb = 0; kb < nkb; ++kb) {
+      const CUtensorMap *mA = &tmA, *mWh = &tmWh, *mWl = &tmWl;
+      if constexpr (STREAM) {
+        if (s) {
+          mA = &st.tmA; mWh = &st.tmWh; mWl = &st.tmWl;
+          stream_wait(st.flags + mt, st.epoch);
+        }
+      }
+      const int tkb = s ? nkb1 : nkb;
+      for (int kb = 0; kb < tkb; ++kb) {
         mbar_wait_cluster(BAR(PB_EMPTY + stage), phase ^ 1);
         if (lane == 0) trace_ev(g, 0, tr_i);
         ++tr_i;
@@ -979,11 +1077,11 @@
         const bool load_w = !WRES || cnt < (uint32_t)P_STAGES;
         if (elect_one()) {
           mbar_expect_tx(BAR(PB_AFULL + stage), TILE_BYTES);
-          tma_load_3d(sb, &tmA, kb * TBK, mi0, batch, BAR(PB_AFULL + stage));
+          tma_load_3d(sb, mA, kb * TBK, mi0, batch, BAR(PB_AFULL + stage));
           if (load_w) {
             if (leader) mbar_expect_tx(BAR(PB_WFULL + stage), 4 * W_HALF_BYTES);
-            tma_load_2d_pair(sb + TILE_BYTES, &tmWh, kb * TBK, wrow, wbar);
-            tma_load_2d_pair(sb + TILE_BYTES + W_HALF_BYTES, &tmWl, kb * TBK, wrow, wbar);
+            tma_load_2d_pair(sb + TILE_BYTES, mWh, kb * TBK, wrow, wbar);
+            tma_load_2d_pair(sb + TILE_BYTES + W_HALF_BYTES, mWl, kb * TBK, wrow, wbar);
           }
         }
         __syncwarp();
@@ -998,10 +1096,12 @@
       int tr_i = 0;
       for (int64_t tile = first_tile; tile < total_tiles; tile += tile_stride, ++it) {
         MMA_TRACE(if (lane == 0) trace_ev(g, 10, (int)it);)
+        uint32_t s;
         int nt;
         int64_t mt_unused;
-        tile_coords(g, tile, UNITS, &mt_unused, &nt);
-        const int64_t nrem = g.N - (int64_t)nt * TBN;
+        coords(tile, &s, &mt_unused, &nt);
+        const int tkb = s ? nkb1 : nkb;
+        const int64_t nrem = (s ? N1 : g.N) - (int64_t)nt * TBN;
         const uint32_t n_mma = nrem >= TBN ? (uint32_t)TBN : (uint32_t)((nrem + 15) & ~15LL);
         const uint32_t idesc = (1u << 4) | (2u << 7) | (2u << 10) | ((n_mma >> 3) << 17) | ((256u >> 4) << 24);
         const uint32_t acc = it & 1u;
@@ -1010,7 +1110,7 @@
         MMA_TRACE(if (lane == 0) trace_ev(g, 11, (int)it);)
         const uint32_t tmem_d = tmem_base + acc * TBN;
 #pragma unroll 1
-        for (int kb = 0; kb < nkb; ++kb) {
+        for (int kb = 0; kb < tkb; ++kb) {
           if (!WRES || cnt < (uint32_t)P_STAGES) mbar_wait_cluster(BAR(PB_WFULL + stage), phase);
           mbar_wait_cluster(BAR(PB_CONV + stage), phase);
           tc_fence_after();
@@ -1029,7 +1129,7 @@
             }
             umma_commit_pair(BAR(PB_EMPTY + stage));
             umma_commit_pair(BAR(PB_AFREE + slot));
-            if (kb == nkb - 1) umma_commit_pair(BAR(PB_TFULL + acc));
+            if (kb == tkb - 1) umma_commit_pair(BAR(PB_TFULL + acc));
             MMA_TRACE(trace_ev(g, 4, tr_i);)
           }
           ++tr_i;
@@ -1047,7 +1147,15 @@
     int tr_i = 0;
     for (int64_t tile = first_tile; tile < total_tiles; tile += tile_stride, ++cit) {
       u64 sum2[2] = {0ull, 0ull}, sq2[2] = {0ull, 0ull}, shift2 = 0ull;
-      for (int kb = 0; kb < nkb; ++kb) {
+      int tkb = nkb;
+      if constexpr (STREAM) {
+        uint32_t s;
+        int nt_unused;
+        int64_t mt_unused;
+        coords(tile, &s, &mt_unused, &nt_unused);
+        tkb = s ? nkb1 : nkb;
+      }
+      for (int kb = 0; kb < tkb; ++kb) {
         mbar_wait(BAR(PB_AFULL + stage), phase);
         if (threadIdx.x == 64) trace_ev(g, 1, tr_i);
         const uint8_t* arow = smem + stage * P_STAGE_BYTES + row * 128;
@@ -1120,10 +1228,12 @@
   } else {
     if constexpr (TN == 192) {
       static_assert(TN != 192 || (ACT != ACT_SIGMOID && !PE && !QUANT), "192-column tiles: no pos-enc / quantised / sigmoid epilogue");
-      epilogue_loop192<ACT, RESID, EPI>(g, smem + P_STAGES * P_STAGE_BYTES + (warp - 6) * EPI_STAGE_BYTES,
+      const TcStream* stp = nullptr;
+      if constexpr (STREAM) stp = &st;
+      epilogue_loop192<ACT, RESID, EPI, STREAM>(g, smem + P_STAGES * P_STAGE_BYTES + (warp - 6) * EPI_STAGE_BYTES,
                               reinterpret_cast<float2*>(smem + Cfg::ROWFAC_OFFSET) + (warp - 6) * 32, sstats, warp, lane,
                               (uint32_t)first_tile, (uint32_t)tile_stride, (uint32_t)total_tiles, rank, BAR(PB_TFULL),
-                              BAR(PB_TEMPTY));
+                              BAR(PB_TEMPTY), stp);
     } else {
       static_assert(!(EPI & EPI_GATE), "the gate epilogue exists for 192-column tiles only");
       epilogue_loop<ACT, PE, RESID, QUANT, true, EPI>(g, smem + P_STAGES * P_STAGE_BYTES + (warp - 6) * EPI_STAGE_BYTES, warp, lane,
@@ -1188,6 +1298,42 @@
 }
 
 long long* g_trace = nullptr;
+
+bool tc_prepare(const GemmArgs& g, bool pair, int tn, int64_t rpb, int64_t nb, int64_t bstride, CUtensorMap* tmA,
+                CUtensorMap* tmWh, CUtensorMap* tmWl, TcArgs* a) {
+  {
+    const uint64_t dims[3] = {(uint64_t)g.K, (uint64_t)rpb, (uint64_t)nb};
+    const uint64_t str[2] = {(uint64_t)g.lda * 4, (uint64_t)(bstride > 0 ? bstride : g.lda) * 4};
+    const uint32_t box[3] = {TBK, TBM, 1};
+    if (!make_map(tmA, g.A, 3, dims, str, box)) return false;
+  }
+  {
+    const uint64_t dims[2] = {(uint64_t)g.K, (uint64_t)g.N};
+    const uint64_t str[1] = {(uint64_t)g.K * 4};
+    const uint32_t box[2] = {TBK, (uint32_t)(pair ? tn / 2 : tn)};
+    if (!make_map(tmWh, g.W_split, 2, dims, str, box)) return false;
+    if (!make_map(tmWl, g.W_split + g.N * g.K, 2, dims, str, box)) return false;
+  }
+  a->M = g.M; a->N = g.N; a->K = g.K;
+  a->rows_per_batch = rpb;
+  a->n_batches = nb;
+  a->m_tiles_per_batch = (int)((rpb + (pair ? 2 : 1) * TBM - 1) / ((pair ? 2 : 1) * TBM));
+  a->n_tiles = (int)((g.N + tn - 1) / tn);
+  a->C = g.C; a->ldc = g.ldc; a->bias = g.bias; a->act_from = g.act_from;
+  a->q_scale = g.q_scale; a->q_zp = g.q_zp;
+  a->resid = g.resid; a->ldr = g.ldr;
+  a->pe_time = g.pe_time; a->pe_freq = g.pe_freq; a->pe_half = g.pe_half;
+  a->ln_s = g.ln_s; a->ln_stats = reinterpret_cast<float2*>(g.ln_stats); a->ln_eps = g.ln_eps;
+  a->amax_val = g.amax_val; a->amax_idx = g.amax_idx;
+  a->trace = g_trace;
+  static const int rot_env = debug_env_int("VASR_TC_ROT", 1);
+  a->rotate_n = rot_env;
+  static const int dbg_env = debug_env_int("VASR_TC_DBG", 0);
+  a->dbg = dbg_env;
+  static const int pf_env = debug_env_int("VASR_TC_PREFETCH", 0);
+  a->prefetch = pf_env;
+  return true;
+}
 
 bool gemm_tc_supported(const GemmArgs& g) {
   if (!encode_fn()) return false;
@@ -1235,38 +1381,8 @@
   if (lna && g.act == ACT_GELU && !t192) return cudaErrorNotSupported;
   const int tn = t192 ? 192 : TBN;
   CUtensorMap tmA, tmWh, tmWl;
-  {
-    const uint64_t dims[3] = {(uint64_t)g.K, (uint64_t)rpb, (uint64_t)nb};
-    const uint64_t str[2] = {(uint64_t)g.lda * 4, (uint64_t)(bstride > 0 ? bstride : g.lda) * 4};
-    const uint32_t box[3] = {TBK, TBM, 1};
-    if (!make_map(&tmA, g.A, 3, dims, str, box)) return cudaErrorNotSupported;
-  }
-  {
-    const uint64_t dims[2] = {(uint64_t)g.K, (uint64_t)g.N};
-    const uint64_t str[1] = {(uint64_t)g.K * 4};
-    const uint32_t box[2] = {TBK, (uint32_t)(pair ? tn / 2 : tn)};
-    if (!make_map(&tmWh, g.W_split, 2, dims, str, box)) return cudaErrorNotSupported;
-    if (!make_map(&tmWl, g.W_split + g.N * g.K, 2, dims, str, box)) return cudaErrorNotSupported;
-  }
   TcArgs a;
-  a.M = g.M; a.N = g.N; a.K = g.K;
-  a.rows_per_batch = rpb;
-  a.n_batches = nb;
-  a.m_tiles_per_batch = (int)((rpb + (pair ? 2 : 1) * TBM - 1) / ((pair ? 2 : 1) * TBM));
-  a.n_tiles = (int)((g.N + tn - 1) / tn);
-  a.C = g.C; a.ldc = g.ldc; a.bias = g.bias; a.act_from = g.act_from;
-  a.q_scale = g.q_scale; a.q_zp = g.q_zp;
-  a.resid = g.resid; a.ldr = g.ldr;
-  a.pe_time = g.pe_time; a.pe_freq = g.pe_freq; a.pe_half = g.pe_half;
-  a.ln_s = g.ln_s; a.ln_stats = reinterpret_cast<float2*>(g.ln_stats); a.ln_eps = g.ln_eps;
-  a.amax_val = g.amax_val; a.amax_idx = g.amax_idx;
-  a.trace = g_trace;
-  static const int rot_env = debug_env_int("VASR_TC_ROT", 1);
-  a.rotate_n = rot_env;
-  static const int dbg_env = debug_env_int("VASR_TC_DBG", 0);
-  a.dbg = dbg_env;
-  static const int pf_env = debug_env_int("VASR_TC_PREFETCH", 0);
-  a.prefetch = pf_env;
+  if (!tc_prepare(g, pair, tn, rpb, nb, bstride, &tmA, &tmWh, &tmWl, &a)) return cudaErrorNotSupported;
 
   const int64_t tiles = (int64_t)a.n_tiles * a.m_tiles_per_batch * nb;
   if (tiles >= (1LL << 31) || rpb >= (1LL << 31)) return cudaErrorNotSupported;
@@ -1290,12 +1406,12 @@
   };
   auto go2 = [&](auto kernel) {
     err = cudaFuncSetAttribute(kernel, cudaFuncAttributeMaxDynamicSharedMemorySize, P_SMEM_BYTES);
-    if (err == cudaSuccess) err = launch_k(kernel, dim3(grid), dim3(TC_THREADS), P_SMEM_BYTES, s, tmA, tmWh, tmWl, a);
+    if (err == cudaSuccess) err = launch_k(kernel, dim3(grid), dim3(TC_THREADS), P_SMEM_BYTES, s, tmA, tmWh, tmWl, a, NoStream{});
   };
   auto go192 = [&](auto kernel) {
     err = cudaFuncSetAttribute(kernel, cudaFuncAttributeMaxDynamicSharedMemorySize, PairCfg<192>::SMEM_BYTES);
     if (err == cudaSuccess)
-      err = launch_k(kernel, dim3(grid), dim3(TC_THREADS), PairCfg<192>::SMEM_BYTES, s, tmA, tmWh, tmWl, a);
+      err = launch_k(kernel, dim3(grid), dim3(TC_THREADS), PairCfg<192>::SMEM_BYTES, s, tmA, tmWh, tmWl, a, NoStream{});
   };
   if (t192) {
     a.rotate_n = 0;
@@ -1360,4 +1476,79 @@
   return cudaSuccess;
 }
 
-}
+struct StreamScratch {
+  unsigned int* mem = nullptr;
+  int64_t row_tiles = 0;
+  unsigned int epoch = 0;
+};
+cudaError_t stream_scratch(cudaStream_t s, int64_t row_tiles, StreamScratch** out) {
+  static std::mutex mu;
+  static std::map<std::pair<int, cudaStream_t>, StreamScratch> cache;
+  int dev = 0;
+  cudaError_t e = cudaGetDevice(&dev);
+  if (e != cudaSuccess) return e;
+  std::lock_guard<std::mutex> lock(mu);
+  StreamScratch& sc = cache[std::make_pair(dev, s)];
+  if (sc.row_tiles < row_tiles) {
+    if (sc.mem) {
+      e = cudaStreamSynchronize(s);
+      if (e == cudaSuccess) e = cudaFree(sc.mem);
+      if (e != cudaSuccess) return e;
+      sc.mem = nullptr;
+      sc.row_tiles = 0;
+    }
+    const int64_t n = row_tiles > 1024 ? row_tiles : 1024;
+    e = cudaMalloc(reinterpret_cast<void**>(&sc.mem), (size_t)2 * n * sizeof(unsigned int));
+    if (e == cudaSuccess) e = cudaMemsetAsync(sc.mem, 0, (size_t)2 * n * sizeof(unsigned int), s);
+    if (e != cudaSuccess) return e;
+    sc.row_tiles = n;
+  }
+  *out = &sc;
+  return cudaSuccess;
+}
+
+cudaError_t launch_gemm_tc_stream(const GemmArgs& g0, const GemmArgs& g1, int num_sms, cudaStream_t s, int64_t* launches) {
+  if (g0.M <= 0) return cudaSuccess;
+  auto takes = [](const GemmArgs& g) {
+    const int64_t r = g.N % 192;
+    return g.W_split && gemm_tc_supported(g) && g.rows_per_batch == 0 && (r == 0 || r >= TBN) && !g.resid &&
+           !g.pe_time && !g.q_scale && !g.ln_s && !g.amax_val && !g.gate && (g.act == ACT_NONE || g.act == ACT_SOFTPLUS);
+  };
+  if (num_sms < 2 || !takes(g0) || !takes(g1) || g0.act != ACT_NONE) return cudaErrorNotSupported;
+  if (g1.A != g0.C || g1.lda != g0.ldc || g1.K > g0.N || g1.M != g0.M) return cudaErrorNotSupported;
+  CUtensorMap tmA, tmWh, tmWl;
+  TcArgs a;
+  TcStream st;
+  if (!tc_prepare(g0, true, 192, g0.M, 1, 0, &tmA, &tmWh, &tmWl, &a) ||
+      !tc_prepare(g1, true, 192, g1.M, 1, 0, &st.tmA, &st.tmWh, &st.tmWl, &st.g))
+    return cudaErrorNotSupported;
+  a.act_from = (int)g0.N;
+  if (g1.act == ACT_NONE) st.g.act_from = (int)g1.N;
+  a.rotate_n = st.g.rotate_n = 0;
+  a.wres = st.g.wres = 0;
+  const int64_t m_tiles = a.m_tiles_per_batch;
+  const int64_t tiles = m_tiles * (a.n_tiles + st.g.n_tiles);
+  if (tiles >= (1LL << 31) || g0.M >= (1LL << 31)) return cudaErrorNotSupported;
+  const int64_t units = num_sms / 2;
+  const unsigned grid = (unsigned)((tiles < units ? tiles : units) * 2);
+  StreamScratch* sc = nullptr;
+  cudaError_t err = stream_scratch(s, m_tiles, &sc);
+  if (err != cudaSuccess) return err;
+  if (++sc->epoch == 0) ++sc->epoch;
+  st.flags = sc->mem;
+  st.count = sc->mem + sc->row_tiles;
+  st.epoch = sc->epoch;
+  st.dep_ntiles = (int)((g1.K + 191) / 192);
+  static const int lag_env = debug_env_int("VASR_TS_LAG", 0);
+  int64_t lag = lag_env > 0 ? lag_env : (2 * units + a.n_tiles + st.g.n_tiles - 1) / (a.n_tiles + st.g.n_tiles);
+  st.lag = (int)(lag < m_tiles ? lag : m_tiles);
+  auto kernel = gemm_tc2_kernel<ACT_SOFTPLUS, false, false, false, false, 192, 0, true>;
+  err = cudaFuncSetAttribute(kernel, cudaFuncAttributeMaxDynamicSharedMemorySize, PairCfg<192>::SMEM_BYTES);
+  if (err == cudaSuccess)
+    err = launch_k(kernel, dim3(grid), dim3(TC_THREADS), PairCfg<192>::SMEM_BYTES, s, tmA, tmWh, tmWl, a, st);
+  if (err != cudaSuccess) return err;
+  if (launches) ++*launches;
+  return cudaSuccess;
+}
+
+}
diff --git a/velocity-asr_b200/csrc/kernels.cuh b/velocity-asr_b200/csrc/kernels.cuh
--- a/velocity-asr_b200/csrc/kernels.cuh
+++ b/velocity-asr_b200/csrc/kernels.cuh
@@ -34,6 +34,7 @@
 };
 cudaError_t launch_gemm(const GemmArgs& g, cudaStream_t s, int64_t* launches);
 cudaError_t launch_gemm_tc(const GemmArgs& g, int num_sms, cudaStream_t s, int64_t* launches);
+cudaError_t launch_gemm_tc_stream(const GemmArgs& g0, const GemmArgs& g1, int num_sms, cudaStream_t s, int64_t* launches);
 cudaError_t launch_split_tf32(const float* w, float* hl, int64_t n, cudaStream_t s);
 extern long long* g_trace;
 
```

Result: slower. 186,500, median of 6 (-4.1%).
